# zombie-einstein/bourse

Measured on AMD Instinct MI355X. Metric: book-steps/sec, higher is better.
Workload: dtype u32

## Files before the change

bourse_amd/csrc/agent_table.hpp:

```cpp
#pragma once
#include <cmath>
#include <cstdint>
#include <cstring>
#include <string>
#include <vector>

#include "../../include/bourse_amd.h"
#include "host_math.hpp"

namespace bkd {

struct Group {
  uint32_t n;
  uint32_t thr;
  uint32_t tick_lo, tick_rng, tick_zone;
  uint32_t vol_lo, vol_rng, vol_zone;
  uint32_t tick_size;
  uint32_t asset;
  uint32_t pad[2];
};
static_assert(sizeof(Group) == 48, "Group: 48-byte records (the per-unit table is read as three 16-byte loads)");

inline uint64_t groups_hash(const Group* g, size_t n) {
  const unsigned char* c = reinterpret_cast<const unsigned char*>(g);
  uint64_t h = 1469598103934665603ull;
  for (size_t i = 0; i < n * sizeof(Group); ++i) h = (h ^ c[i]) * 1099511628211ull;
  return h;
}

inline int make_groups(const bk_random_agents* rows, uint32_t n_groups, const uint32_t* assets, uint32_t M,
                       const uint32_t* asset_tick, Group* out, uint64_t* total, std::string* msg,
                       const std::string& where = std::string()) {
  *total = 0;
  auto fail = [&](int code, uint32_t g, const char* m) {
    *msg = where.empty() ? std::string(m) : where + "group " + std::to_string(g) + ": " + m;
    return code;
  };
  for (uint32_t g = 0; g < n_groups; ++g) {
    const bk_random_agents& r = rows[g];
    if (r.tick_lo >= r.tick_hi || r.vol_lo >= r.vol_hi)
      return fail(BK_INVALID_ARGUMENT, g, "empty tick/vol range");
    const uint32_t asset = assets ? assets[g] : 0u;
    if (asset >= M) return fail(BK_INVALID_ARGUMENT, g, "group asset index out of range");
    if (r.tick_size % asset_tick[asset] != 0)
      return fail(BK_PRICE_NOT_TICK_MULTIPLE, g, "agent tick_size must be a multiple of the env tick_size");
    if (static_cast<uint64_t>(r.tick_hi - 1) * r.tick_size >= 0xFFFFFFFFull || r.tick_lo == 0)
      return fail(BK_INVALID_ARGUMENT, g, "limit prices must lie in (0, u32::MAX)");
    Group G{};
    G.n = r.n_agents;
    G.thr = activity_threshold(r.activity_rate);
    G.tick_lo = r.tick_lo;
    G.tick_rng = r.tick_hi - r.tick_lo;
    G.tick_zone = sample_zone(G.tick_rng);
    G.vol_lo = r.vol_lo;
    G.vol_rng = r.vol_hi - r.vol_lo;
    G.vol_zone = sample_zone(G.vol_rng);
    G.tick_size = r.tick_size;
    G.asset = asset;
    *total += r.n_agents;
    out[g] = G;
  }
  return BK_OK;
}

constexpr const char* CAPACITY_MSG = "sum of n_agents exceeds max_live_orders (one pool slot per agent)";

inline int make_group_table(const bk_random_agents* rows, uint32_t n_units, uint32_t n_groups, const uint32_t* assets,
                            uint32_t M, const uint32_t* asset_tick, uint32_t max_live_orders, std::vector<Group>& out,
                            uint64_t* total, std::string* msg) {
  std::vector<Group> t(static_cast<size_t>(n_units) * n_groups);
  *total = 0;
  for (uint32_t u = 0; u < n_units; ++u) {
    const std::string where = "unit " + std::to_string(u) + ", ";
    uint64_t tot = 0;
    const size_t row = static_cast<size_t>(u) * n_groups;
    if (int rc = make_groups(rows + row, n_groups, assets, M, asset_tick, t.data() + row, &tot, msg, where)) return rc;
    for (uint32_t g = 0; g < n_groups; ++g)
      if (t[row + g].n != t[g].n) {
        *msg = where + "group " + std::to_string(g) + ": n_agents differs from unit 0's (every unit shares the pool layout)";
        return BK_INVALID_ARGUMENT;
      }
    if (tot > max_live_orders) {
      *msg = where + CAPACITY_MSG;
      return BK_CAPACITY;
    }
    *total = tot;
  }
  out.swap(t);
  return BK_OK;
}

constexpr int MAX_MEMBERS = 4;
constexpr int MAX_ASSETS = 8;

struct MixedDesc {
  uint32_t type;
  uint32_t n;
  uint32_t thr, tick_lo, tick_rng, tick_zone, vol_lo, vol_rng, vol_zone, tick_size;
  uint32_t thr_limit, thr_market;
  int32_t keep_thr;
  uint32_t trade_vol;
  uint32_t slot_base;
  uint32_t pad;
  double mu, sigma, decay, demand, scale, order_ratio, n_f, tick_f;
};
static_assert(sizeof(MixedDesc) == 128, "MixedDesc layout");

inline uint64_t fnv1a_bytes(const void* p, size_t n, uint64_t h = 1469598103934665603ull) {
  const unsigned char* c = static_cast<const unsigned char*>(p);
  for (size_t i = 0; i < n; ++i) h = (h ^ c[i]) * 1099511628211ull;
  return h;
}
inline uint64_t mixed_hash(const uint32_t* member_asset, const MixedDesc* d, size_t n) {
  return fnv1a_bytes(member_asset, MAX_MEMBERS * sizeof(uint32_t), fnv1a_bytes(d, n * sizeof(MixedDesc)));
}

inline int make_mixed_descs(const bk_agent_desc* members, uint32_t n_members, const uint32_t* assets,
                            const uint32_t* asset_tick, MixedDesc* out, uint32_t* fixed_a, std::string* msg,
                            const std::string& where = std::string()) {
  for (int as = 0; as < MAX_ASSETS; ++as) fixed_a[as] = 0;
  auto fail = [&](int code, uint32_t i, const char* m) {
    *msg = where.empty() ? std::string(m) : where + "member " + std::to_string(i) + ": " + m;
    return code;
  };
  for (uint32_t i = 0; i < n_members; ++i) {
    const uint32_t as = assets ? assets[i] : 0u;
    uint32_t& fixed = fixed_a[as];
    const bk_agent_desc& m = members[i];
    MixedDesc D;
    std::memset(&D, 0, sizeof(D));
    D.type = m.type;
    D.n = m.n_agents;
    if (m.tick_size == 0 || m.tick_size % asset_tick[as] != 0)
      return fail(BK_PRICE_NOT_TICK_MULTIPLE, i, "member tick_size must be a non-zero multiple of the env tick_size");
    if (m.type == BK_AGENT_RANDOM) {
      if (m.tick_lo >= m.tick_hi || m.vol_lo >= m.vol_hi || m.tick_lo == 0 ||
          static_cast<uint64_t>(m.tick_hi - 1) * m.tick_size >= 0xFFFFFFFFull)
        return fail(BK_INVALID_ARGUMENT, i, "bad RandomAgents ranges");
      D.thr = activity_threshold(m.activity_rate);
      D.tick_lo = m.tick_lo;
      D.tick_rng = m.tick_hi - m.tick_lo;
      D.tick_zone = sample_zone(D.tick_rng);
      D.vol_lo = m.vol_lo;
      D.vol_rng = m.vol_hi - m.vol_lo;
      D.vol_zone = sample_zone(D.vol_rng);
      D.tick_size = m.tick_size;
      D.slot_base = fixed;
      fixed += m.n_agents;
    } else if (m.type == BK_AGENT_NOISE || m.type == BK_AGENT_MOMENTUM) {
      if (m.n_agents > 0xFFFFu) return fail(BK_INVALID_ARGUMENT, i, "n_agents is a u16 in the reference");
      if (!(m.price_dist_sigma >= 0.0) || !std::isfinite(m.price_dist_sigma) || !std::isfinite(m.price_dist_mu))
        return fail(BK_INVALID_ARGUMENT, i, "LogNormal::new(mu, sigma) needs finite mu and sigma >= 0");
      D.thr_limit = activity_threshold(m.p_limit);
      D.thr_market = activity_threshold(m.p_market);
      D.keep_thr = keep_threshold(m.p_cancel);
      D.trade_vol = m.trade_vol;
      D.mu = m.price_dist_mu;
      D.sigma = m.price_dist_sigma;
      D.decay = m.decay;
      D.demand = m.demand;
      D.scale = m.scale;
      D.order_ratio = m.order_ratio;
      D.n_f = static_cast<double>(m.n_agents);
      D.tick_f = static_cast<double>(m.tick_size);
    } else {
      return fail(BK_INVALID_ARGUMENT, i, "unknown agent type");
    }
    out[i] = D;
  }
  return BK_OK;
}

constexpr const char* MIXED_CAPACITY_MSG = "RandomAgents members leave no pool slots for the other members' orders";
inline bool mixed_capacity_ok(const uint32_t* fixed_a, uint32_t M, uint32_t max_live_orders) {
  for (uint32_t as = 0; as < M; ++as)
    if (fixed_a[as] >= max_live_orders) return false;
  return true;
}

inline int make_mixed_table(const bk_agent_desc* members, uint32_t n_units, uint32_t n_members, const uint32_t* assets,
                            uint32_t M, const uint32_t* asset_tick, uint32_t max_live_orders, std::vector<MixedDesc>& out,
                            uint32_t* fixed_a, std::string* msg) {
  std::vector<MixedDesc> t(static_cast<size_t>(n_units) * n_members);
  for (uint32_t u = 0; u < n_units; ++u) {
    const std::string where = "unit " + std::to_string(u) + ", ";
    const size_t row = static_cast<size_t>(u) * n_members;
    if (int rc = make_mixed_descs(members + row, n_members, assets, asset_tick, t.data() + row, fixed_a, msg, where))
      return rc;
    for (uint32_t i = 0; i < n_members; ++i) {
      const char* what = t[row + i].type != t[i].type ? "type differs from unit 0's"
                         : t[row + i].n != t[i].n   ? "n_agents differs from unit 0's"
                                                    : nullptr;
      if (what) {
        *msg = where + "member " + std::to_string(i) + ": " + what + " (every unit shares the members' kinds and pool layout)";
        return BK_INVALID_ARGUMENT;
      }
    }
  }
  if (!mixed_capacity_ok(fixed_a, M, max_live_orders)) {
    *msg = std::string("unit 0, ") + MIXED_CAPACITY_MSG;
    return BK_CAPACITY;
  }
  out.swap(t);
  return BK_OK;
}

}
```

bourse_amd/csrc/agents_fsm_body.inc:

```
  uint16_t* list = reinterpret_cast<uint16_t*>(fsm_lds);
  const int lane = threadIdx.x;
  __builtin_amdgcn_s_setprio(3);
#if BOURSE_AMD_FSM_TOP_VGPR > 0
  asm volatile("" ::: "v" BK_STR(BOURSE_AMD_FSM_TOP_VGPR));
#endif
  const uint32_t M = a.assets;
  const uint32_t b = a.book_begin + blockIdx.x * 64 + lane;
  if (b >= a.book_end) return;
  uint32_t* st = a.state + (size_t)b * M * a.state_stride;
  uint32_t* bt = a.batch + (size_t)b * M * a.batch_stride;
#if BK_PB
  const Group* row = table + (size_t)b * a.n_groups;
  LaneGroup nxt{};
  if (a.n_groups) nxt = load_lane_group(row);
#endif

  RngLane rng;
  {
    const uint2 x0 = *reinterpret_cast<const uint2*>(st + H_S0_LO);
    const uint2 x1 = *reinterpret_cast<const uint2*>(st + H_S1_LO);
    rng.a0 = x0.x, rng.a1 = x0.y, rng.b0 = x1.x, rng.b1 = x1.y;
  }
  uint64_t live[R];
#pragma unroll
  for (int r = 0; r < R; ++r) {
    uint2 x = *reinterpret_cast<const uint2*>(st + H_LIVE0 + 2 * r);
    for (uint32_t as = 1; as < M; ++as) {
      const uint2 y = *reinterpret_cast<const uint2*>(st + (size_t)as * a.state_stride + H_LIVE0 + 2 * r);
      x.x |= y.x;
      x.y |= y.y;
    }
    live[r] = mk64(x.x, x.y);
  }
  uint2* pv = reinterpret_cast<uint2*>(bt + BT_EV + 32 * R);

  const uint32_t five = RngLane::opaque5();
  uint32_t n = 0, n_ev = 0, gbase = 0;
  for (uint32_t g = 0; g < a.n_groups; ++g) {
    const Group G = a.groups[g];
    const uint32_t gend = gbase + G.n;
    gbase = gend;
#if BK_PB
    LaneGroup L{};
    L = nxt;
    if (g + 1 < a.n_groups) nxt = load_lane_group(row + g + 1);
#endif
    if (G.n == 0) continue;
#if BK_PB
    const uint32_t g_thr = L.a.y, g_tick_lo = L.a.z, g_vol_lo = L.b.y;
    uint32_t g_tick_size = L.tick_size;
    asm volatile("" : "+v"(g_tick_size));
    uint32_t v_trng = L.a.w, v_vrng = L.b.z, v_tzone = L.b.x, v_vzone = L.b.w;
#else
    asm volatile("" ::"s"(G.thr), "s"(G.tick_lo), "s"(G.tick_rng), "s"(G.tick_zone));
    asm volatile("" ::"s"(G.vol_lo), "s"(G.vol_rng), "s"(G.vol_zone), "s"(G.tick_size));
    const uint32_t g_thr = G.thr, g_tick_lo = G.tick_lo, g_vol_lo = G.vol_lo, g_tick_size = G.tick_size;
    uint32_t v_trng = G.tick_rng, v_vrng = G.vol_rng, v_tzone = G.tick_zone, v_vzone = G.vol_zone;
#endif
    asm volatile("" : "+v"(v_trng), "+v"(v_vrng), "+v"(v_tzone), "+v"(v_vzone));
    const uint64_t thr8 = (uint64_t)g_thr << 8;
    uint64_t price0 = (uint64_t)(g_tick_lo * g_tick_size);
    asm volatile("" : "+v"(price0));
    for (uint32_t sbeg = gend - G.n; sbeg < gend;) {
      const uint32_t send = gend < (sbeg | 63u) + 1u ? gend : (sbeg | 63u) + 1u;
      uint64_t w = live[0];
#pragma unroll
      for (int r = 1; r < R; ++r) w = ((sbeg >> 6) == (uint32_t)r) ? live[r] : w;
      uint32_t cur_side = 0, cur_price = 0;
      uint64_t P_ACT = ~0ull, P_SIDE = 0, P_TICK = 0, P_VOL = 0;
      while (n < send) {
        const uint32_t x = rng.output(five);
        const uint32_t range = sel(P_SIDE, 2u, sel(P_TICK, v_trng, v_vrng));
        const uint32_t zone = sel(P_SIDE, 0x7FFFFFFFu, sel(P_TICK, v_tzone, v_vzone));
        const uint64_t m = (uint64_t)x * range;
        const uint32_t val = (uint32_t)(m >> 32);
        uint64_t C_HIT = __builtin_amdgcn_ballot_w64((uint64_t)x < thr8);
        uint64_t C_ACC = __builtin_amdgcn_ballot_w64((uint32_t)m <= zone);
        uint64_t C_LIVE = __builtin_amdgcn_ballot_w64(((w >> (n & 63)) & 1ull) != 0);
        asm volatile("" : "+v"(rng.a0), "+v"(rng.a1), "+v"(rng.b0), "+v"(rng.b1)
                     : "s"(P_ACT), "s"(P_SIDE), "s"(P_TICK), "s"(P_VOL), "s"(C_HIT), "s"(C_ACC), "s"(C_LIVE));
        rng.advance();
        asm volatile("" : "+v"(rng.a0), "+v"(rng.a1), "+v"(rng.b0), "+v"(rng.b1), "+s"(P_ACT), "+s"(P_SIDE), "+s"(P_TICK),
                       "+s"(P_VOL), "+s"(C_HIT), "+s"(C_ACC), "+s"(C_LIVE));
        const uint64_t HIT = P_ACT & C_HIT, CANCEL = HIT & C_LIVE, TO_SIDE = HIT & ~C_LIVE;
        const uint64_t A_SIDE = C_ACC & P_SIDE, A_TICK = C_ACC & P_TICK, A_VOL = C_ACC & P_VOL;
        const uint64_t QUEUE = CANCEL | A_VOL, ADV = (P_ACT & ~C_HIT) | QUEUE;
        cur_side = sel(A_SIDE, val, cur_side);
        {
          uint64_t pr, cy;
#if BK_PB
          asm("v_mad_u64_u32 %0, %1, %2, %3, %4" : "=v"(pr), "=s"(cy) : "v"(val), "v"(g_tick_size), "v"(price0));
#else
          asm("v_mad_u64_u32 %0, %1, %2, %3, %4" : "=v"(pr), "=s"(cy) : "v"(val), "s"(g_tick_size), "v"(price0));
#endif
          cur_price = sel(A_TICK, (uint32_t)pr, cur_price);
        }
        if (lane_bit(QUEUE)) list[n_ev * 64 + lane] = (uint16_t)sel(A_VOL, n | EV_NEW | (cur_side << 14), n);
        asm("v_addc_co_u32_e64 %0, vcc, 0, %0, %1" : "+v"(n_ev) : "s"(QUEUE) : "vcc");
        if (lane_bit(A_VOL)) pv[n] = make_uint2(cur_price, g_vol_lo + val);
        P_SIDE = TO_SIDE | (P_SIDE & ~C_ACC);
        P_TICK = A_SIDE | (P_TICK & ~C_ACC);
        P_VOL = A_TICK | (P_VOL & ~C_ACC);
        P_ACT = ADV;
        asm("v_addc_co_u32_e64 %0, vcc, 0, %0, %1" : "+v"(n) : "s"(ADV) : "vcc");
      }
      sbeg = send;
    }
  }

  {
    uint32_t i = n_ev > 1 ? n_ev - 1 : 0;
    uint32_t rg = i + 1;
    uint32_t zn = (rg << __builtin_clz(rg)) - 1u;
    while (i != 0) {
      const uint32_t x = rng.output(five);
      const uint64_t m = (uint64_t)x * rg;
      uint64_t ACC = __builtin_amdgcn_ballot_w64((uint32_t)m <= zn);
      asm volatile("" : "+v"(rng.a0), "+v"(rng.a1), "+v"(rng.b0), "+v"(rng.b1) : "s"(ACC));
      rng.advance();
      asm volatile("" : "+v"(rng.a0), "+v"(rng.a1), "+v"(rng.b0), "+v"(rng.b1), "+s"(ACC));
      if (lane_bit(ACC)) {
        const uint32_t j = (uint32_t)(m >> 32);
        const uint16_t ai = list[i * 64 + lane], aj = list[j * 64 + lane];
        list[i * 64 + lane] = aj;
        list[j * 64 + lane] = ai;
        --i;
        rg = i + 1;
        zn = (rg << __builtin_clz(rg)) - 1u;
      }
    }
  }

  for (uint32_t as = 0; as < M; ++as) {
    *reinterpret_cast<uint2*>(st + (size_t)as * a.state_stride + H_S0_LO) = make_uint2(rng.a0, rng.a1);
    *reinterpret_cast<uint2*>(st + (size_t)as * a.state_stride + H_S1_LO) = make_uint2(rng.b0, rng.b1);
  }
  bt[BT_NEV] = n_ev;
  for (uint32_t k = 0; k < n_ev; k += 2) {
    const uint32_t lo = list[k * 64 + lane];
    const uint32_t hi = (k + 1 < n_ev) ? list[(k + 1) * 64 + lane] : 0u;
    bt[BT_EV + (k >> 1)] = lo | (hi << 16);
  }
```

bourse_amd/csrc/book_device.hpp:

```cpp
#pragma once
#include <hip/hip_runtime.h>
#include <utility>
#include <stdint.h>

#include "event_asm.hpp"
#include "event_asm_gen.hpp"
#include "agent_table.hpp"

#ifndef BOURSE_AMD_ASM_EVENTS
#define BOURSE_AMD_ASM_EVENTS 1
#endif
#ifndef BOURSE_AMD_ASM_R48
#define BOURSE_AMD_ASM_R48 1
#endif

namespace bkd {

constexpr int HDR_DW = 64;
enum Hdr : int {
  H_T_LO = 0, H_T_HI, H_S0_LO, H_S0_HI, H_S1_LO, H_S1_HI,
  H_NEXT_ID, H_SEQ, H_TRADES_LO, H_TRADES_HI, H_FLAGS, H_TRADING,
  H_STEPS_LO, H_STEPS_HI, H_EVENTS_LO, H_EVENTS_HI, H_TRADE_VOL,
  H_TRADE_BASE_LO, H_TRADE_BASE_HI, H_LAST_NTRADES, H_LAST_NEVENTS,
  H_EV_KEYED,
  H_LIVE0 = 32,
};
constexpr int HDR_SCALARS = 20;
constexpr int POOL_FIELDS = 5;
constexpr int MAX_GROUPS = 8;

constexpr uint32_t FLAG_POOL_OVERFLOW = 1u, FLAG_TRADE_OVERFLOW = 2u, FLAG_STEP_SIZE = 4u,
                   FLAG_ORDER_LOG_FULL = 8u, FLAG_UNKNOWN_ORDER = 16u, FLAG_HIST_OVERFLOW = 32u, FLAG_PRICE_TICK = 64u,
                   FLAG_EVENT_OVERFLOW = 128u;


struct UDiv {
  uint32_t m, sh1, sh2, d;
};
__device__ __forceinline__ uint32_t udiv(uint32_t n, const UDiv& dv) {
  const uint32_t t = __umulhi(dv.m, n);
  return (t + ((n - t) >> dv.sh1)) >> dv.sh2;
}

struct DevTrade {
  uint32_t t_lo, t_hi, price, vol, active, passive, side_is_bid, pad;
};

struct DevOrderLog {
  uint32_t status, vol, price;
  uint32_t key_price;
  uint32_t arr_lo, arr_hi, end_lo, end_hi;
  uint32_t key_lo, key_hi, pad[2];
};

struct DevArgs {
  uint32_t n_books, levels, tick_size, n_groups;
  uint32_t step_lo, step_hi;
  uint32_t state_stride;
  uint32_t l2_width;
  uint32_t trade_cap, hist_cap;
  uint32_t hist_slot0, step_prio;
  uint32_t n_agents_total, log_cap;
  uint32_t* state;
  uint32_t* l2_last;
  uint32_t* hist;
  DevTrade* trades;
  DevOrderLog* order_log;
  const uint32_t* ev_off;
  const uint4* ev;
  const uint32_t* ev_len;
  uint32_t ev_stride;
  uint32_t* batch;
  uint32_t batch_stride;
  uint32_t book_begin, book_end;
  uint32_t assets;
  uint32_t asset_tick[MAX_ASSETS];
  UDiv tick_div, asset_div[MAX_ASSETS];
  Group groups[MAX_GROUPS];
};
constexpr int BT_NEV = 0, BT_EV = 64;
constexpr uint32_t EV_NEW = 0x8000u, EV_BID = 0x4000u, EV_SLOT = 0x1FFu;
constexpr uint32_t EV_MOD = 0x800u, EV_MOD_P = 0x200u, EV_MOD_V = 0x400u;

__device__ __forceinline__ uint32_t rfl(uint32_t v) { return __builtin_amdgcn_readfirstlane(v); }

typedef uint32_t bk_u32x4 __attribute__((ext_vector_type(4)));
typedef uint32_t bk_u32x8 __attribute__((ext_vector_type(8)));
typedef uint32_t bk_u32x16 __attribute__((ext_vector_type(16)));
__device__ __forceinline__ void sload_x16_x4(const uint32_t* p, bk_u32x16& a, bk_u32x4& b) {
  asm volatile("s_load_dwordx16 %0, %2, 0x0\n\ts_load_dwordx4 %1, %2, 0x40\n\ts_waitcnt lgkmcnt(0)"
               : "=&s"(a), "=&s"(b) : "s"(p) : "memory");
}
__device__ __forceinline__ bk_u32x8 sload_x8(const uint32_t* p) {
  bk_u32x8 a;
  asm volatile("s_load_dwordx8 %0, %1, 0x0\n\ts_waitcnt lgkmcnt(0)" : "=&s"(a) : "s"(p) : "memory");
  return a;
}
__device__ __forceinline__ Group sload_group(const Group* p) {
  bk_u32x8 w;
  uint32_t ts;
  asm volatile("s_load_dwordx8 %0, %2, 0x0\n\ts_load_dword %1, %2, 0x20\n\ts_waitcnt lgkmcnt(0)" : "=&s"(w), "=&s"(ts) : "s"(p));
  Group G{};
  G.n = w[0], G.thr = w[1], G.tick_lo = w[2], G.tick_rng = w[3], G.tick_zone = w[4];
  G.vol_lo = w[5], G.vol_rng = w[6], G.vol_zone = w[7], G.tick_size = ts;
  return G;
}
__device__ __forceinline__ uint32_t rdl(uint32_t v, uint32_t lane) { return __builtin_amdgcn_readlane(v, lane); }
extern "C" __device__ uint32_t bk_llvm_writelane(uint32_t val, uint32_t lane, uint32_t old) __asm(
    "llvm.amdgcn.writelane.i32");
__device__ __forceinline__ uint32_t wrl(uint32_t val, uint32_t lane, uint32_t old) {
  return bk_llvm_writelane(val, lane, old);
}

__device__ __forceinline__ uint32_t sel(uint64_t mask, uint32_t if_set, uint32_t if_clear) {
  return __builtin_amdgcn_inverse_ballot_w64(mask) ? if_set : if_clear;
}
__device__ __forceinline__ bool lane_bit(uint64_t mask) { return __builtin_amdgcn_inverse_ballot_w64(mask); }

#define BK_DPP_REDUCE(OP)                                                                      \
  asm("s_nop 1\n\t" OP " %0, %0, %0 quad_perm:[1,0,3,2] row_mask:0xf bank_mask:0xf\n\t"        \
      "s_nop 1\n\t" OP " %0, %0, %0 quad_perm:[2,3,0,1] row_mask:0xf bank_mask:0xf\n\t"        \
      "s_nop 1\n\t" OP " %0, %0, %0 row_half_mirror row_mask:0xf bank_mask:0xf\n\t"            \
      "s_nop 1\n\t" OP " %0, %0, %0 row_mirror row_mask:0xf bank_mask:0xf\n\t"                 \
      "s_nop 1\n\t" OP " %0, %0, %0 row_bcast:15 row_mask:0xa bank_mask:0xf\n\t"               \
      "s_nop 1\n\t" OP " %0, %0, %0 row_bcast:31 row_mask:0xc bank_mask:0xf\n\t"               \
      "s_nop 1"                                                                                \
      : "+v"(x))
__device__ __forceinline__ uint32_t wave_umin(uint32_t x) {
  BK_DPP_REDUCE("v_min_u32_dpp");
  return rdl(x, 63);
}
__device__ __forceinline__ uint32_t wave_umax(uint32_t x) {
  BK_DPP_REDUCE("v_max_u32_dpp");
  return rdl(x, 63);
}
__device__ __forceinline__ int32_t wave_imin(int32_t x) {
  BK_DPP_REDUCE("v_min_i32_dpp");
  return (int32_t)rdl((uint32_t)x, 63);
}
__device__ __forceinline__ int32_t wave_imax(int32_t x) {
  BK_DPP_REDUCE("v_max_i32_dpp");
  return (int32_t)rdl((uint32_t)x, 63);
}
__device__ __forceinline__ uint32_t wave_add(uint32_t x) {
  BK_DPP_REDUCE("v_add_u32_dpp");
  return rdl(x, 63);
}

#define BK_DPP4(CTRL)                                                     \
  "v_max_u32_dpp %0, %0, %0 " CTRL "\n\tv_min_u32_dpp %1, %1, %1 " CTRL "\n\t" \
  "v_add_u32_dpp %2, %2, %2 " CTRL "\n\tv_add_u32_dpp %3, %3, %3 " CTRL "\n\t"
__device__ __forceinline__ void wave_reduce4(uint32_t& mx, uint32_t& mn, uint32_t& s1, uint32_t& s2) {
  asm("s_nop 1\n\t" BK_DPP4("quad_perm:[1,0,3,2] row_mask:0xf bank_mask:0xf") BK_DPP4("quad_perm:[2,3,0,1] row_mask:0xf bank_mask:0xf")
          BK_DPP4("row_half_mirror row_mask:0xf bank_mask:0xf") BK_DPP4("row_mirror row_mask:0xf bank_mask:0xf")
              BK_DPP4("row_bcast:15 row_mask:0xa bank_mask:0xf") BK_DPP4("row_bcast:31 row_mask:0xc bank_mask:0xf") "s_nop 1"
      : "+v"(mx), "+v"(mn), "+v"(s1), "+v"(s2));
  mx = rdl(mx, 63);
  mn = rdl(mn, 63);
  s1 = rdl(s1, 63);
  s2 = rdl(s2, 63);
}

#define BK_DPP3(CTRL) \
  "v_max_u32_dpp %0, %0, %0 " CTRL "\n\tv_min_u32_dpp %1, %1, %1 " CTRL "\n\tv_max_u32_dpp %2, %2, %2 " CTRL "\n\t"
__device__ __forceinline__ void wave_reduce3(uint32_t& mx, uint32_t& mn, uint32_t& m2) {
  asm("s_nop 1\n\t" BK_DPP3("quad_perm:[1,0,3,2] row_mask:0xf bank_mask:0xf") BK_DPP3("quad_perm:[2,3,0,1] row_mask:0xf bank_mask:0xf")
          BK_DPP3("row_half_mirror row_mask:0xf bank_mask:0xf") BK_DPP3("row_mirror row_mask:0xf bank_mask:0xf")
              BK_DPP3("row_bcast:15 row_mask:0xa bank_mask:0xf") BK_DPP3("row_bcast:31 row_mask:0xc bank_mask:0xf") "s_nop 1"
      : "+v"(mx), "+v"(mn), "+v"(m2));
  mx = rdl(mx, 63);
  mn = rdl(mn, 63);
  m2 = rdl(m2, 63);
}

__device__ __forceinline__ uint64_t mk64(uint32_t lo, uint32_t hi) { return ((uint64_t)hi << 32) | lo; }

struct Rng {
  uint64_t s0, s1;
  __device__ __forceinline__ uint32_t next_u32() {
    uint64_t r = s0 * 5ull;
    r = (r << 7) | (r >> 57);
    r *= 9ull;
    uint64_t t1 = s1 ^ s0;
    s0 = ((s0 << 24) | (s0 >> 40)) ^ t1 ^ (t1 << 16);
    s1 = (t1 << 37) | (t1 >> 27);
    return (uint32_t)r;
  }
  __device__ __forceinline__ uint32_t below(uint32_t range, uint32_t zone) {
    for (;;) {
      uint32_t v = next_u32();
      uint64_t m = (uint64_t)v * range;
      if ((uint32_t)m <= zone) return (uint32_t)(m >> 32);
    }
  }
  __device__ __forceinline__ uint32_t below(uint32_t range) {
    uint32_t zone = (range << __builtin_clz(range)) - 1u;
    return below(range, zone);
  }
};

__device__ __forceinline__ uint32_t xor3(uint32_t a, uint32_t b, uint32_t c) {
  return __builtin_amdgcn_bitop3_b32(a, b, c, 0x96);
}
struct RngLane {
  uint32_t a0, a1, b0, b1;
  static __device__ __forceinline__ uint32_t opaque5() {
    uint32_t five = 5u;
    asm("" : "+s"(five));
    return five;
  }
  static __device__ __forceinline__ uint32_t mul5_rotl7_lo(uint32_t a0, uint32_t a1, uint32_t five) {
    const uint64_t p = (uint64_t)a0 * five;
    const uint32_t hi5 = (a1 << 2) + (uint32_t)(p >> 32) + a1;
    return __builtin_amdgcn_alignbit((uint32_t)p, hi5, 25);
  }
  __device__ __forceinline__ uint32_t next_u32() {
    const uint32_t r = mul5_rotl7_lo(a0, a1, opaque5());
    const uint32_t t0 = b0 ^ a0, t1 = b1 ^ a1;
    const uint32_t n0 = xor3(__builtin_amdgcn_alignbit(a0, a1, 8), t0, t0 << 16);
    const uint32_t n1 = xor3(__builtin_amdgcn_alignbit(a1, a0, 8), t1, __builtin_amdgcn_alignbit(t1, t0, 16));
    a0 = n0;
    a1 = n1;
    b0 = __builtin_amdgcn_alignbit(t1, t0, 27);
    b1 = __builtin_amdgcn_alignbit(t0, t1, 27);
    return (r << 3) + r;
  }
  __device__ __forceinline__ uint32_t output(uint32_t five) const {
    const uint32_t r = mul5_rotl7_lo(a0, a1, five);
    return (r << 3) + r;
  }
  __device__ __forceinline__ void advance() {
    uint32_t t0 = b0 ^ a0, t1 = b1 ^ a1;
    uint32_t r0 = __builtin_amdgcn_alignbit(a0, a1, 8), r1 = __builtin_amdgcn_alignbit(a1, a0, 8);
    asm volatile("" : "+v"(t0), "+v"(t1), "+v"(r0), "+v"(r1));
    const uint32_t n0 = xor3(r0, t0, t0 << 16);
    const uint32_t n1 = xor3(r1, t1, __builtin_amdgcn_alignbit(t1, t0, 16));
    a0 = n0;
    a1 = n1;
    b0 = __builtin_amdgcn_alignbit(t1, t0, 27);
    b1 = __builtin_amdgcn_alignbit(t0, t1, 27);
  }
};

template <int R>
struct Book {
  uint32_t price[R], vol[R], id[R], seq[R];
  uint64_t live[R], bid[R], pend[R];
  uint64_t t;
  uint32_t next_id, seq_ctr, trade_vol, flags, trading;
  uint64_t n_trades, n_events, trade_base;
  uint32_t tr_k, tr_price, tr_vol, tr_act, tr_pas;
  uint32_t tr_n;
  uint32_t hdr0;
};

template <int R>
__device__ __forceinline__ uint32_t slot_read(const uint32_t (&v)[R], uint32_t n) {
  uint32_t out = rdl(v[0], n & 63);
#pragma unroll
  for (int r = 1; r < R; ++r) {
    uint32_t x = rdl(v[r], n & 63);
    out = ((n >> 6) == (uint32_t)r) ? x : out;
  }
  return out;
}
template <int R>
__device__ __forceinline__ void slot_write(uint32_t (&v)[R], uint32_t n, uint32_t val) {
#pragma unroll
  for (int r = 0; r < R; ++r)
    if ((n >> 6) == (uint32_t)r) v[r] = wrl(val, n & 63, v[r]);
}
template <int R>
__device__ __forceinline__ bool mask_test(const uint64_t (&m)[R], uint32_t n) {
  uint64_t w = 0;
#pragma unroll
  for (int r = 0; r < R; ++r) w |= m[r] & (((n >> 6) == (uint32_t)r) ? ~0ull : 0ull);
  return (w >> (n & 63)) & 1ull;
}
template <int R>
__device__ __forceinline__ void mask_set(uint64_t (&m)[R], uint32_t n, bool on) {
  const uint64_t bit = 1ull << (n & 63);
#pragma unroll
  for (int r = 0; r < R; ++r) {
    const uint64_t b = ((n >> 6) == (uint32_t)r) ? bit : 0ull;
    m[r] = on ? (m[r] | b) : (m[r] & ~b);
  }
}

template <int R>
__device__ __forceinline__ void flush_trades(Book<R>& B, const DevArgs& a, uint32_t book, uint64_t t0, int lane) {
  if (B.tr_n == 0) return;
  const uint64_t first = B.n_trades;
  B.n_trades += B.tr_n;
  const uint64_t pos0 = first - B.trade_base;
  if ((uint32_t)lane < B.tr_n) {
    const uint64_t pos = pos0 + (uint32_t)lane;
    if (pos < a.trade_cap) {
      const uint64_t t = t0 + (B.tr_k & 0x7FFFFFFFu);
      DevTrade rec;
      rec.t_lo = (uint32_t)t;
      rec.t_hi = (uint32_t)(t >> 32);
      rec.price = B.tr_price;
      rec.vol = B.tr_vol;
      rec.active = B.tr_act;
      rec.passive = B.tr_pas;
      rec.side_is_bid = B.tr_k >> 31;
      rec.pad = 0;
      uint4* dst = reinterpret_cast<uint4*>(a.trades + (size_t)book * a.trade_cap + pos);
      const uint4* src = reinterpret_cast<const uint4*>(&rec);
      dst[0] = src[0];
      dst[1] = src[1];
    }
  }
  if (pos0 + B.tr_n > a.trade_cap) B.flags |= FLAG_TRADE_OVERFLOW;
  B.tr_n = 0;
}

template <int R>
__device__ __forceinline__ void emit_trade(Book<R>& B, const DevArgs& a, uint32_t book, uint64_t t0, int lane,
                                           uint32_t k, bool passive_is_bid, uint32_t price, uint32_t vol,
                                           uint32_t active, uint32_t passive) {
  if (B.tr_n == 64) flush_trades(B, a, book, t0, lane);
  const uint32_t l = B.tr_n;
  B.tr_k = wrl(k | (passive_is_bid ? 0x80000000u : 0u), l, B.tr_k);
  B.tr_price = wrl(price, l, B.tr_price);
  B.tr_vol = wrl(vol, l, B.tr_vol);
  B.tr_act = wrl(active, l, B.tr_act);
  B.tr_pas = wrl(passive, l, B.tr_pas);
  B.tr_n = l + 1;
}

template <int R>
__device__ __forceinline__ uint32_t pool_gather(const uint32_t (&v)[R], uint32_t idx) {
  uint32_t out = (uint32_t)__builtin_amdgcn_ds_bpermute((int)((idx & 63u) << 2), (int)v[0]);
#pragma unroll
  for (int r = 1; r < R; ++r) {
    const uint32_t x = (uint32_t)__builtin_amdgcn_ds_bpermute((int)((idx & 63u) << 2), (int)v[r]);
    out = (idx >> 6) == (uint32_t)r ? x : out;
  }
  return out;
}
template <int R>
__device__ __forceinline__ void flush_trades_compact(Book<R>& B, const DevArgs& a, uint32_t book, uint64_t t0, int lane,
                                                     const uint32_t (&ev)[R]) {
  if (B.tr_n == 0) return;
  const uint32_t k = B.tr_k & 0x7FFFFFFFu, ps = B.tr_pas & (64u * R - 1u);
  const uint32_t as = pool_gather<R>(ev, k < 64u * R ? k : 0u) & EV_SLOT & (64u * R - 1u);
  B.tr_price = pool_gather<R>(B.price, ps);
  B.tr_pas = pool_gather<R>(B.id, ps);
  B.tr_act = pool_gather<R>(B.id, as);
  flush_trades<R>(B, a, book, t0, lane);
}

struct LogCtx {
  DevOrderLog* base;
  uint32_t cap;
};
__device__ __forceinline__ void log_write(const LogCtx& lg, uint32_t& flags, int lane, uint32_t id, uint32_t status,
                                          uint32_t vol, uint32_t price, uint64_t arr, uint64_t end,
                                          bool set_arr, bool set_key = false, uint64_t key_t = 0) {
  if (!lg.base) return;
  if (id >= lg.cap) {
    flags |= FLAG_ORDER_LOG_FULL;
    return;
  }
  if (lane == 0) {
    DevOrderLog* e = lg.base + id;
    e->status = status;
    e->vol = vol;
    e->price = price;
    if (set_arr) {
      e->arr_lo = (uint32_t)arr;
      e->arr_hi = (uint32_t)(arr >> 32);
    }
    e->end_lo = (uint32_t)end;
    e->end_hi = (uint32_t)(end >> 32);
    if (set_key) {
      e->key_price = price;
      e->key_lo = (uint32_t)key_t;
      e->key_hi = (uint32_t)(key_t >> 32);
    }
  }
}
__device__ __forceinline__ void log_fill(const LogCtx& lg, uint32_t& flags, int lane, uint32_t id, uint32_t vol,
                                         uint64_t t) {
  if (!lg.base) return;
  if (id >= lg.cap) {
    flags |= FLAG_ORDER_LOG_FULL;
    return;
  }
  if (lane == 0) {
    DevOrderLog* e = lg.base + id;
    e->vol = vol;
    if (vol == 0) {
      e->status = 2;
      e->end_lo = (uint32_t)t;
      e->end_hi = (uint32_t)(t >> 32);
    }
  }
}

template <int R, bool agg_bid>
__device__ __forceinline__ bool match_side(Book<R>& B, const DevArgs& a, uint32_t book, uint64_t t0, int lane,
                                           uint32_t k, uint32_t p, uint32_t& v, uint32_t agg_id, const LogCtx& lg) {
  const uint32_t v0 = v;
  while (v > 0) {
// ... 39 lines not shown
        pv -= tv;
        B.vol[r] = wrl(pv, l, B.vol[r]);
        if (pv == 0) B.live[r] &= ~eq[r];
      }
    }
    v -= tv;
    emit_trade(B, a, book, t0, lane, k, !agg_bid, best, tv, agg_id, pid);
    B.trade_vol += tv;
    log_fill(lg, B.flags, lane, pid, pv, t0 + k);
  }
  return v0 != 0 && v == 0;
}
template <int R>
__device__ __forceinline__ bool match(Book<R>& B, const DevArgs& a, uint32_t book, uint64_t t0, int lane, uint32_t k,
                                      bool agg_bid, uint32_t p, uint32_t& v, uint32_t agg_id, const LogCtx& lg) {
  return agg_bid ? match_side<R, true>(B, a, book, t0, lane, k, p, v, agg_id, lg)
                 : match_side<R, false>(B, a, book, t0, lane, k, p, v, agg_id, lg);
}

template <int R, int RS, bool CLS = false, bool LOG = false, class... Lg>
__device__ __forceinline__ void slot_event_at(Book<R>& B, const DevArgs& a, uint32_t book, uint64_t t0, int lane,
                                              uint32_t k, uint32_t sl, uint32_t ew = 0, const Lg&... lg) {
  const LogCtx nolog{nullptr, 0};
  const uint64_t bit = 1ull << sl;
  if (CLS ? !(ew & EV_NEW) : !(B.pend[RS] & bit)) {
    if constexpr (LOG) {
      if (B.live[RS] & bit)
        log_write(lg..., B.flags, lane, rdl(B.id[RS], sl), 3, rdl(B.vol[RS], sl), rdl(B.price[RS], sl), 0, t0 + k, false);
    }
    B.live[RS] &= ~bit;
    return;
  }
  if (!CLS) B.pend[RS] &= ~bit;
  const uint32_t p = rdl(B.price[RS], sl);
  uint32_t v = rdl(B.vol[RS], sl);
  const uint32_t id = rdl(B.id[RS], sl);
  bool filled = false, market;
  if (CLS ? (ew & EV_BID) != 0 : (B.bid[RS] & bit) != 0) {
    market = p == 0xFFFFFFFFu;
    if (B.trading) {
      if constexpr (LOG) filled = match_side<R, true>(B, a, book, t0, lane, k, p, v, id, lg...);
      else filled = match_side<R, true>(B, a, book, t0, lane, k, p, v, id, nolog);
    }
  } else {
    market = p == 0u;
    if (B.trading) {
      if constexpr (LOG) filled = match_side<R, false>(B, a, book, t0, lane, k, p, v, id, lg...);
      else filled = match_side<R, false>(B, a, book, t0, lane, k, p, v, id, nolog);
    }
  }
  if (!market && !filled) {
    B.vol[RS] = wrl(v, sl, B.vol[RS]);
    B.seq[RS] = wrl(B.seq_ctr, sl, B.seq[RS]);
    B.live[RS] |= bit;
    B.seq_ctr += 1;
  }
  if constexpr (LOG) {
    const uint64_t tk = t0 + k;
    uint32_t status = 1;
    uint64_t end = ~0ull;
    if (filled || market) {
      status = filled ? 2u : (B.trading ? 3u : 4u);
      end = tk;
    }
    log_write(lg..., B.flags, lane, id, status, v, p, tk, end, true, true, status == 1 ? tk : 0ull);
  }
}

template <int R, int RS = 0, bool CLS = false, bool LOG = false, class... Lg>
__device__ __forceinline__ void process_slot_event(Book<R>& B, const DevArgs& a, uint32_t book, uint64_t t0, int lane,
                                                   uint32_t k, uint32_t n, uint32_t ew = 0, const Lg&... lg) {
  if constexpr (RS + 1 < R) {
    if ((n >> 6) == (uint32_t)RS)
      slot_event_at<R, RS, CLS, LOG>(B, a, book, t0, lane, k, n & 63, ew, lg...);
    else
      process_slot_event<R, RS + 1, CLS, LOG>(B, a, book, t0, lane, k, n, ew, lg...);
  } else {
    slot_event_at<R, RS, CLS, LOG>(B, a, book, t0, lane, k, n & 63, ew, lg...);
  }
}

template <int R>
__device__ __forceinline__ void snapshot(const Book<R>& B, const DevArgs& a, uint32_t book, int lane,
                                         uint32_t* __restrict__ bins , uint32_t hist_slot,
                                         uint32_t& flags, bool write_last, const UDiv& tick) {
  const uint32_t L = a.levels;
  uint32_t mb = 0u, ma = 0xFFFFFFFFu, sb = 0u, sa = 0u;
#pragma unroll
  for (int r = 0; r < R; ++r) {
    const uint64_t lb = B.live[r] & B.bid[r], la = B.live[r] & ~B.bid[r];
    mb = max(mb, sel(lb, B.price[r], 0u));
    ma = min(ma, sel(la, B.price[r], 0xFFFFFFFFu));
    sb += sel(lb, B.vol[r], 0u);
    sa += sel(la, B.vol[r], 0u);
  }
  wave_reduce4(mb, ma, sb, sa);
  const uint32_t bid_best = mb;
  const uint32_t ask_best = ma;
  const uint32_t bid_vol = sb, ask_vol = sa;

  for (uint32_t j = lane; j < 4 * L; j += 64) bins[j] = 0;
  __builtin_amdgcn_fence(__ATOMIC_RELEASE, "wavefront");
  __builtin_amdgcn_wave_barrier();
#pragma unroll
  for (int r = 0; r < R; ++r) {
    const bool is_live = lane_bit(B.live[r]);
    const bool is_bid = lane_bit(B.bid[r]);
    if (is_live) {
      const uint32_t d = is_bid ? (bid_best - B.price[r]) : (B.price[r] - ask_best);
      const uint32_t q = udiv(d, tick);
      if (q * tick.d == d && q < L) {
        atomicAdd(&bins[4 * q + (is_bid ? 0 : 2)], B.vol[r]);
        atomicAdd(&bins[4 * q + (is_bid ? 1 : 3)], 1u);
      }
    }
  }
  __builtin_amdgcn_fence(__ATOMIC_ACQ_REL, "wavefront");
  __builtin_amdgcn_wave_barrier();
  if (__builtin_expect(__umulhi(L - 1u, tick.d) != 0u, 0)) {
    for (uint32_t i = 1; i < L; ++i) {
      const uint32_t m = i * tick.d, q = udiv(m, tick);
      if (q != i && q * tick.d == m && lane < 4) bins[4 * i + lane] = bins[4 * q + lane];
    }
    __builtin_amdgcn_fence(__ATOMIC_ACQ_REL, "wavefront");
    __builtin_amdgcn_wave_barrier();
  }

  const uint32_t W = a.l2_width;
  uint32_t* last = a.l2_last + (size_t)book * W;
  uint32_t* hist = nullptr;
  if (a.hist_cap) hist = a.hist + ((size_t)hist_slot * a.n_books + book) * W;
  (void)flags;
  uint32_t h = 0;
  h = lane == 0 ? B.trade_vol : h;
  h = lane == 1 ? bid_best : h;
  h = lane == 2 ? ask_best : h;
  h = lane == 3 ? ask_vol : h;
  h = lane == 4 ? bid_vol : h;
  if (lane < 5) {
    if (write_last) last[lane] = h;
    if (hist) hist[lane] = h;
  }
  for (uint32_t j = lane; j < 4 * L; j += 64) {
    const uint32_t x = bins[j];
    if (write_last) last[5 + j] = x;
    if (hist) hist[5 + j] = x;
  }
}

template <int R>
struct StepRaw {
  uint32_t hdr, f[R][POOL_FIELDS];
  uint32_t sh[HDR_SCALARS];
  uint32_t bh, ev[R];
  uint2 pv[R];
};
template <int R>
__device__ __forceinline__ void load_state_raw(StepRaw<R>& w, const uint32_t* __restrict__ st, int lane) {
  w.hdr = st[lane];
#pragma unroll
  for (int r = 0; r < R; ++r) {
    const uint32_t* p = st + HDR_DW + r * POOL_FIELDS * 64;
#pragma unroll
    for (int f = 0; f < POOL_FIELDS; ++f) w.f[r][f] = p[f * 64 + lane];
  }
}
template <int R>
__device__ __forceinline__ void load_state_scalars(StepRaw<R>& w, const uint32_t* __restrict__ st) {
  if constexpr (R <= 2) {
    bk_u32x16 a;
    bk_u32x4 b;
    sload_x16_x4(st, a, b);
#pragma unroll
    for (int i = 0; i < 16; ++i) w.sh[i] = a[i];
#pragma unroll
    for (int i = 16; i < HDR_SCALARS; ++i) w.sh[i] = b[i - 16];
  }
}
template <int R>
__device__ __forceinline__ void unpack_book(Book<R>& B, Rng& rng, const StepRaw<R>& w) {
  const uint32_t hdr = w.hdr;
#pragma unroll
  for (int r = 0; r < R; ++r) {
    B.price[r] = w.f[r][0];
    B.vol[r] = w.f[r][1];
    B.id[r] = w.f[r][2];
    B.seq[r] = w.f[r][3];
  }
  auto H = [&](int i) { return R <= 2 ? w.sh[i] : rdl(hdr, (uint32_t)i); };
  B.t = mk64(H(H_T_LO), H(H_T_HI));
  rng.s0 = mk64(H(H_S0_LO), H(H_S0_HI));
  rng.s1 = mk64(H(H_S1_LO), H(H_S1_HI));
  B.next_id = H(H_NEXT_ID);
  B.seq_ctr = H(H_SEQ);
  B.n_trades = mk64(H(H_TRADES_LO), H(H_TRADES_HI));
  B.flags = H(H_FLAGS);
  B.trading = H(H_TRADING);
  B.n_events = mk64(H(H_EVENTS_LO), H(H_EVENTS_HI));
  B.trade_vol = H(H_TRADE_VOL);
  B.trade_base = mk64(H(H_TRADE_BASE_LO), H(H_TRADE_BASE_HI));
#pragma unroll
  for (int r = 0; r < R; ++r) {
    const uint32_t meta = w.f[r][4];
    B.live[r] = __ballot((meta & 1u) != 0);
    B.bid[r] = __ballot((meta & 2u) != 0);
    B.pend[r] = __ballot((meta & 4u) != 0);
  }
  B.tr_k = B.tr_price = B.tr_vol = B.tr_act = B.tr_pas = 0;
  B.tr_n = 0;
  B.hdr0 = hdr;
}
template <int R>
__device__ __forceinline__ void load_book(Book<R>& B, Rng& rng, const uint32_t* __restrict__ st, int lane) {
  StepRaw<R> w;
  load_state_raw<R>(w, st, lane);
  load_state_scalars<R>(w, st);
  unpack_book<R>(B, rng, w);
}

template <int R, bool KEEP_HDR = false>
__device__ __forceinline__ void store_book(const Book<R>& B, const Rng& rng, uint32_t* __restrict__ st, int lane,
                                           uint64_t steps_done, uint32_t last_ntrades, uint32_t last_nevents,
                                           uint32_t ev_keyed = 0u) {
  uint32_t hdr = KEEP_HDR ? B.hdr0 : st[lane];
  if (!KEEP_HDR) hdr += lane == H_EV_KEYED ? ev_keyed : 0u;
  auto put = [&](int idx, uint32_t v) { hdr = wrl(rfl(v), (uint32_t)idx, hdr); };
  put(H_T_LO, (uint32_t)B.t);
  put(H_T_HI, (uint32_t)(B.t >> 32));
  put(H_S0_LO, (uint32_t)rng.s0);
  put(H_S0_HI, (uint32_t)(rng.s0 >> 32));
  put(H_S1_LO, (uint32_t)rng.s1);
  put(H_S1_HI, (uint32_t)(rng.s1 >> 32));
  put(H_NEXT_ID, B.next_id);
  put(H_SEQ, B.seq_ctr);
  put(H_TRADES_LO, (uint32_t)B.n_trades);
  put(H_TRADES_HI, (uint32_t)(B.n_trades >> 32));
  put(H_FLAGS, B.flags);
  put(H_STEPS_LO, (uint32_t)steps_done);
  put(H_STEPS_HI, (uint32_t)(steps_done >> 32));
  put(H_EVENTS_LO, (uint32_t)B.n_events);
  put(H_EVENTS_HI, (uint32_t)(B.n_events >> 32));
  put(H_TRADE_VOL, B.trade_vol);
  put(H_LAST_NTRADES, last_ntrades);
  put(H_LAST_NEVENTS, last_nevents);
#pragma unroll
  for (int r = 0; r < R; ++r) {
    put(H_LIVE0 + 2 * r, (uint32_t)B.live[r]);
    put(H_LIVE0 + 2 * r + 1, (uint32_t)(B.live[r] >> 32));
  }
  st[lane] = hdr;
#pragma unroll
  for (int r = 0; r < R; ++r) {
    uint32_t* p = st + HDR_DW + r * POOL_FIELDS * 64;
    p[0 * 64 + lane] = B.price[r];
    p[1 * 64 + lane] = B.vol[r];
    p[2 * 64 + lane] = B.id[r];
    p[3 * 64 + lane] = B.seq[r];
    p[4 * 64 + lane] = (lane_bit(B.live[r]) ? 1u : 0u) | (lane_bit(B.bid[r]) ? 2u : 0u) | (lane_bit(B.pend[r]) ? 4u : 0u);
  }
}

#ifndef BOURSE_AMD_KEYED_EVENTS
#define BOURSE_AMD_KEYED_EVENTS 1
#endif
#ifndef BOURSE_AMD_KEY_SEQ_BITS
#define BOURSE_AMD_KEY_SEQ_BITS 16
#endif
#ifndef BOURSE_AMD_KEYED_WIDE
#define BOURSE_AMD_KEYED_WIDE 1
#endif
constexpr uint32_t KEY_SB = BOURSE_AMD_KEY_SEQ_BITS;
constexpr uint32_t KEY_SMASK = (1u << (KEY_SB < 16u ? KEY_SB : 16u)) - 1u;
constexpr uint32_t KEY_PSPAN = (1u << (31u - (KEY_SB > 16u ? KEY_SB : 16u))) - 6u;
constexpr uint32_t KEY_ASK = 0x80000000u;
constexpr uint32_t KP_MKT_BID = 0xFFFFFFFFu, KP_MKT_ASK = 0x10000u;
template <int R>
__device__ __forceinline__ bool key_window(const Book<R>& B, const uint64_t (&newm)[R], uint32_t n_ev, uint32_t& pbase,
                                           uint32_t& sbase, uint32_t xmin = 0xFFFFFFFFu, uint32_t xmax = 0u) {
  uint32_t pmax = xmax, pmin = xmin, age = 0;
#pragma unroll
  for (int r = 0; r < R; ++r) {
    const bool lv = lane_bit(B.live[r]), in = lv | lane_bit(newm[r]);
    pmax = max(pmax, in ? B.price[r] : 0u);
    pmin = min(pmin, in ? B.price[r] : 0xFFFFFFFFu);
    age = max(age, lv ? B.seq_ctr - B.seq[r] : 0u);
  }
  wave_reduce3(pmax, pmin, age);
  pbase = pmin - 2u;
  sbase = B.seq_ctr - age - 1u;
  return pmin >= 2u && pmax != 0xFFFFFFFFu && pmax - pmin <= KEY_PSPAN && age + n_ev < KEY_SMASK - 1u;
}

template <int R>
struct KeyState {
  uint32_t key[R], pk[R];
  uint32_t sq, sbase, pbase;
  int32_t alo, bhi;
};
template <int R, bool MARKETS = false>
__device__ __forceinline__ bool keys_begin(const Book<R>& B, const uint64_t (&newm)[R], uint32_t n_ev, KeyState<R>& K,
                                           uint32_t xmin = 0xFFFFFFFFu, uint32_t xmax = 0u) {
  uint32_t pbase;
  uint64_t lim[R];
#pragma unroll
  for (int r = 0; r < R; ++r)
    lim[r] = MARKETS ? newm[r] & ~__ballot(B.price[r] == (lane_bit(B.bid[r]) ? 0xFFFFFFFFu : 0u)) : newm[r];
  if (!key_window<R>(B, lim, n_ev, pbase, K.sbase, xmin, xmax)) return false;
  K.pbase = pbase;
#pragma unroll
  for (int r = 0; r < R; ++r) {
    const bool bidl = lane_bit(B.bid[r]);
    const uint32_t pf = B.price[r] - pbase, sf = B.seq[r] - K.sbase;
    K.key[r] = lane_bit(B.live[r]) ? ((pf << 16) | (bidl ? 0xFFFFu - sf : KEY_ASK | sf)) : 0u;
    K.pk[r] = lane_bit(lim[r]) ? (bidl ? 0x8000u | pf : pf) : 0u;
    if (MARKETS) K.pk[r] = lane_bit(newm[r] & ~lim[r]) ? (bidl ? 0xFFFFu : 1u) : K.pk[r];
  }
  K.sq = KEY_ASK | (B.seq_ctr - K.sbase);
  K.alo = (int32_t)0x80000000u;
  K.bhi = 0x7FFFFFFF;
  return true;
}
template <int R, bool MARKETS>
__device__ __forceinline__ bool keys_begin_wide(const Book<R>& B, const uint64_t (&newm)[R], uint32_t n_ev, KeyState<R>& K,
                                                const uint32_t (&ev)[R], uint32_t* bins, int lane) {
  uint64_t lim[R];
#pragma unroll
  for (int r = 0; r < R; ++r)
    lim[r] = MARKETS ? newm[r] & ~__ballot(B.price[r] == (lane_bit(B.bid[r]) ? 0xFFFFFFFFu : 0u)) : newm[r];
  uint32_t pmax = 0, age = 0, vbig = 0;
#pragma unroll
  for (int r = 0; r < R; ++r) {
    const bool lv = lane_bit(B.live[r]), in = lv | lane_bit(lim[r]);
    pmax = max(pmax, in ? B.price[r] : 0u);
    age = max(age, lv ? B.seq_ctr - B.seq[r] : 0u);
    vbig = max(vbig, (lv | lane_bit(newm[r])) ? B.vol[r] : 0u);
  }
  uint32_t dummy = 0xFFFFFFFFu;
  wave_reduce3(pmax, dummy, age);
  vbig = wave_umax(vbig);
  if (pmax == 0xFFFFFFFFu || pmax < 2u || age + n_ev >= KEY_SMASK - 1u || vbig >= (1u << 22)) return false;
  const uint32_t pbase = pmax > KEY_PSPAN ? pmax - KEY_PSPAN : 0u, lowp = pbase + 2u;
  if (lane < 2 * R) bins[lane] = 0u;
  __builtin_amdgcn_fence(__ATOMIC_ACQ_REL, "wavefront");
  __builtin_amdgcn_wave_barrier();
#pragma unroll
  for (int re = 0; re < R; ++re) {
    const uint32_t slot = ev[re] & EV_SLOT & (64u * R - 1u);
    if ((uint32_t)(re * 64 + lane) < n_ev) atomicOr(&bins[slot >> 5], 1u << (slot & 31u));
  }
  __builtin_amdgcn_fence(__ATOMIC_ACQ_REL, "wavefront");
  __builtin_amdgcn_wave_barrier();
  uint32_t pbid = 0;
#pragma unroll
  for (int r = 0; r < R; ++r)
    pbid = max(pbid, ((lane_bit(B.live[r]) | lane_bit(lim[r])) && lane_bit(B.bid[r])) ? B.price[r] : 0u);
  pbid = wave_umax(pbid);
  uint32_t w_bid = 0, a_ask = 0;
  uint64_t bad = 0;
#pragma unroll
  for (int r = 0; r < R; ++r) {
    const bool lv = lane_bit(B.live[r]), bidl = lane_bit(B.bid[r]), nw = lane_bit(newm[r]);
    const bool below = (lv | lane_bit(lim[r])) && B.price[r] < lowp;
    const bool listed = ((bins[(uint32_t)(r * 64 + lane) >> 5] >> ((uint32_t)lane & 31u)) & 1u) != 0u;
    bad |= __ballot(below && !bidl);
    w_bid += (lv && bidl && !below && !listed) ? B.vol[r] : 0u;
    a_ask += (nw && !bidl && B.price[r] <= pbid) ? B.vol[r] : 0u;
  }
  if (bad) return false;
  w_bid = wave_add(w_bid);
  a_ask = wave_add(a_ask);
  if (a_ask > w_bid) return false;
  K.pbase = pbase;
  K.sbase = B.seq_ctr - age - 1u;
#pragma unroll
  for (int r = 0; r < R; ++r) {
    const bool bidl = lane_bit(B.bid[r]);
    const uint32_t pf = B.price[r] < lowp ? 1u : B.price[r] - pbase, sf = B.seq[r] - K.sbase;
    K.key[r] = lane_bit(B.live[r]) ? ((pf << 16) | (bidl ? 0xFFFFu - sf : KEY_ASK | sf)) : 0u;
    K.pk[r] = lane_bit(lim[r]) ? (bidl ? 0x8000u | pf : pf) : 0u;
    if (MARKETS) K.pk[r] = lane_bit(newm[r] & ~lim[r]) ? (bidl ? 0xFFFFu : 1u) : K.pk[r];
  }
  K.sq = KEY_ASK | (B.seq_ctr - K.sbase);
  K.alo = (int32_t)0x80000000u;
  K.bhi = 0x7FFFFFFF;
  return true;
}
template <int R, bool MARKETS>
__device__ __forceinline__ bool keys_begin_wide_high(const Book<R>& B, const uint64_t (&newm)[R], uint32_t n_ev, KeyState<R>& K,
                                                     const uint32_t (&ev)[R], uint32_t* bins, int lane) {
  uint64_t lim[R];
#pragma unroll
  for (int r = 0; r < R; ++r)
    lim[r] = MARKETS ? newm[r] & ~__ballot(B.price[r] == (lane_bit(B.bid[r]) ? 0xFFFFFFFFu : 0u)) : newm[r];
  uint32_t pmin = 0xFFFFFFFFu, age = 0, vbig = 0, pdummy = 0;
#pragma unroll
  for (int r = 0; r < R; ++r) {
    const bool lv = lane_bit(B.live[r]), in = lv | lane_bit(lim[r]);
    pmin = min(pmin, in ? B.price[r] : 0xFFFFFFFFu);
    age = max(age, lv ? B.seq_ctr - B.seq[r] : 0u);
    vbig = max(vbig, (lv | lane_bit(newm[r])) ? B.vol[r] : 0u);
  }
  wave_reduce3(pdummy, pmin, age);
  vbig = wave_umax(vbig);
  if (pmin < 2u || pmin > 0xFFFFFFFFu - KEY_PSPAN - 4u || age + n_ev >= KEY_SMASK - 1u || vbig >= (1u << 22)) return false;
  const uint32_t pbase = pmin - 2u, highp = pmin + KEY_PSPAN;
  if (lane < 2 * R) bins[lane] = 0u;
  __builtin_amdgcn_fence(__ATOMIC_ACQ_REL, "wavefront");
  __builtin_amdgcn_wave_barrier();
#pragma unroll
  for (int re = 0; re < R; ++re) {
    const uint32_t slot = ev[re] & EV_SLOT & (64u * R - 1u);
    if ((uint32_t)(re * 64 + lane) < n_ev) atomicOr(&bins[slot >> 5], 1u << (slot & 31u));
  }
  __builtin_amdgcn_fence(__ATOMIC_ACQ_REL, "wavefront");
  __builtin_amdgcn_wave_barrier();
  uint32_t pask = 0xFFFFFFFFu;
#pragma unroll
  for (int r = 0; r < R; ++r)
    pask = min(pask, ((lane_bit(B.live[r]) | lane_bit(lim[r])) && !lane_bit(B.bid[r])) ? B.price[r] : 0xFFFFFFFFu);
  pask = wave_umin(pask);
  uint32_t w_ask = 0, b_bid = 0;
  uint64_t bad = 0;
#pragma unroll
  for (int r = 0; r < R; ++r) {
    const bool lv = lane_bit(B.live[r]), bidl = lane_bit(B.bid[r]), nw = lane_bit(newm[r]);
    const bool above = (lv | lane_bit(lim[r])) && B.price[r] > highp;
    const bool listed = ((bins[(uint32_t)(r * 64 + lane) >> 5] >> ((uint32_t)lane & 31u)) & 1u) != 0u;
    bad |= __ballot(above && bidl);
    w_ask += (lv && !bidl && !above && !listed) ? B.vol[r] : 0u;
    b_bid += (nw && bidl && B.price[r] >= pask) ? B.vol[r] : 0u;
  }
  if (bad) return false;
  w_ask = wave_add(w_ask);
  b_bid = wave_add(b_bid);
  if (b_bid > w_ask) return false;
  K.pbase = pbase;
  K.sbase = B.seq_ctr - age - 1u;
#pragma unroll
  for (int r = 0; r < R; ++r) {
    const bool bidl = lane_bit(B.bid[r]);
    const uint32_t pf = B.price[r] > highp ? 0x7FFFu : B.price[r] - pbase, sf = B.seq[r] - K.sbase;
    K.key[r] = lane_bit(B.live[r]) ? ((pf << 16) | (bidl ? 0xFFFFu - sf : KEY_ASK | sf)) : 0u;
    K.pk[r] = lane_bit(lim[r]) ? (bidl ? 0x8000u | pf : pf) : 0u;
    if (MARKETS) K.pk[r] = lane_bit(newm[r] & ~lim[r]) ? (bidl ? 0xFFFFu : 1u) : K.pk[r];
  }
  K.sq = KEY_ASK | (B.seq_ctr - K.sbase);
  K.alo = (int32_t)0x80000000u;
  K.bhi = 0x7FFFFFFF;
  return true;
}
template <int R>
__device__ __forceinline__ void keys_end(Book<R>& B, const KeyState<R>& K) {
  B.seq_ctr = K.sbase + (K.sq & 0x7FFFFFFFu);
#pragma unroll
  for (int r = 0; r < R; ++r) {
    B.live[r] = __ballot(K.key[r] != 0u);
    const uint32_t f = K.key[r] & 0xFFFFu;
    B.seq[r] = K.key[r] != 0u ? K.sbase + ((int32_t)K.key[r] < 0 ? f : 0xFFFFu - f) : B.seq[r];
  }
}
template <int R>
__device__ __forceinline__ void key_event_words(const KeyState<R>& K, const uint32_t (&ev)[R], uint32_t n_ev, uint32_t (&evw)[R]) {
#pragma unroll
  for (int re = 0; re < R; ++re) {
    evw[re] = ev[re] & 0xFFFFu;
    if (n_ev > (uint32_t)re * 64u) evw[re] |= pool_gather<R>(K.pk, ev[re] & EV_SLOT & (64u * R - 1u)) << 16;
  }
}

template <int R, bool agg_bid, int... I>
__device__ __forceinline__ int32_t key_touch(const KeyState<R>& K, std::integer_sequence<int, I...>) {
  int32_t m = (int32_t)K.key[0];
  ((m = agg_bid ? min(m, (int32_t)K.key[I]) : max(m, (int32_t)K.key[I])), ...);
  return m;
}

template <int R>
__device__ __forceinline__ void flush_trades_compact(Book<R>& B, const DevArgs& a, uint32_t book, uint64_t t0, int lane,
                                                     const uint32_t (&ev)[R]);
template <int R, bool agg_bid>
__device__ __forceinline__ bool match_side_keyed(Book<R>& B, KeyState<R>& K, const DevArgs& a, uint32_t book, uint64_t t0,
                                                 int lane, uint32_t k, int32_t kp, uint32_t& v, const uint32_t (&ev)[R]) {
  const uint32_t v0 = v;
  while (v > 0) {
    const int32_t m = key_touch<R, agg_bid>(K, std::make_integer_sequence<int, R>());
    const int32_t best = agg_bid ? wave_imin(m) : wave_imax(m);
    (agg_bid ? K.alo : K.bhi) = best;
    if (agg_bid ? (best > kp) : (best < kp)) break;
    uint32_t pv = 0, tv = 0, slot = 0;
#pragma unroll
    for (int r = 0; r < R; ++r) {
      const uint64_t eq = __ballot(K.key[r] == (uint32_t)best);
      if (eq) {
        const uint32_t l = __builtin_ctzll(eq);
        pv = rdl(B.vol[r], l);
        tv = v < pv ? v : pv;
        pv -= tv;
        B.vol[r] = wrl(pv, l, B.vol[r]);
        if (pv == 0) K.key[r] = wrl(0u, l, K.key[r]);
        slot = (uint32_t)r * 64u + l;
      }
    }
    v -= tv;
    if (B.tr_n == 64) flush_trades_compact<R>(B, a, book, t0, lane, ev);
    const uint32_t tl = B.tr_n;
    B.tr_k = wrl(k | (agg_bid ? 0u : 0x80000000u), tl, B.tr_k);
    B.tr_vol = wrl(tv, tl, B.tr_vol);
    B.tr_pas = wrl(slot, tl, B.tr_pas);
    B.tr_n = tl + 1;
    B.trade_vol += tv;
  }
  return v0 != 0 && v == 0;
}
template <int R, int RS, bool CLS = true>
__device__ __forceinline__ void slot_event_keyed_at(Book<R>& B, KeyState<R>& K, const DevArgs& a, uint32_t book, uint64_t t0,
                                                    int lane, uint32_t k, uint32_t sl, uint32_t ew, const uint32_t (&ev)[R]) {
  const uint64_t bit = 1ull << sl;
  if (CLS ? !(ew & EV_NEW) : !(B.pend[RS] & bit)) {
    K.key[RS] = wrl(0u, sl, K.key[RS]);
    return;
  }
  if (!CLS) B.pend[RS] &= ~bit;
  const bool is_bid = CLS ? (ew & EV_BID) != 0 : (B.bid[RS] & bit) != 0;
  const uint32_t kpu = (rdl(K.pk[RS], sl) << 16) | (is_bid ? 0xFFFFu : 0u);
  const int32_t kp = (int32_t)kpu;
  uint32_t v = rdl(B.vol[RS], sl);
  const bool market = !CLS && kpu == (is_bid ? KP_MKT_BID : KP_MKT_ASK);
  bool filled = false;
  if (B.trading && !(is_bid ? kp < K.alo : kp > K.bhi))
    filled = is_bid ? match_side_keyed<R, true>(B, K, a, book, t0, lane, k, kp, v, ev)
                    : match_side_keyed<R, false>(B, K, a, book, t0, lane, k, kp, v, ev);
  if (!market && !filled) {
    B.vol[RS] = wrl(v, sl, B.vol[RS]);
    const uint32_t x = kpu ^ K.sq;
    if (is_bid)
      K.bhi = max(K.bhi, (int32_t)x);
    else
      K.alo = min(K.alo, (int32_t)x);
    K.key[RS] = wrl(x, sl, K.key[RS]);
    K.sq += 1;
  }
}
template <int R, int RS = 0, bool CLS = true>
__device__ __forceinline__ void slot_event_keyed(Book<R>& B, KeyState<R>& K, const DevArgs& a, uint32_t book, uint64_t t0,
                                                 int lane, uint32_t k, uint32_t n, uint32_t ew, const uint32_t (&ev)[R]) {
  if constexpr (RS + 1 < R) {
    if ((n >> 6) == (uint32_t)RS)
      slot_event_keyed_at<R, RS, CLS>(B, K, a, book, t0, lane, k, n & 63, ew, ev);
    else
      slot_event_keyed<R, RS + 1, CLS>(B, K, a, book, t0, lane, k, n, ew, ev);
  } else {
    slot_event_keyed_at<R, RS, CLS>(B, K, a, book, t0, lane, k, n & 63, ew, ev);
  }
}

template <int R, bool MKT = false, bool TAGGED = false, bool CLS = false, bool PENDKEY = false, bool LOG = false, class... Lg>
__device__ __forceinline__ uint32_t step_from_list(Book<R>& B, const DevArgs& a, uint32_t book, int lane,
                                                   const uint32_t (&ev)[R], uint32_t n_ev, uint32_t* bins,
                                                   uint32_t hist_slot, bool write_last, const UDiv& tick,
                                                   const uint64_t (&mine)[R], uint32_t& n_own, uint32_t asset = 0,
                                                   const Lg&... lg) {
  const uint64_t step_size = mk64(a.step_lo, a.step_hi);
  const uint64_t t0 = B.t;
  B.trade_vol = 0;
  const uint64_t trades_before = B.n_trades;
  if (step_size != 0 && (uint64_t)n_ev >= step_size) B.flags |= FLAG_STEP_SIZE;
  uint64_t newm[R];
#pragma unroll
  for (int r = 0; r < R; ++r) {
    newm[r] = (CLS || PENDKEY) ? B.pend[r] : 0ull;
    if (CLS) B.pend[r] = 0;
  }
  constexpr bool MKTK = MKT && CLS && !TAGGED;
  uint32_t evm[R], own_cnt = 0;
  bool listed = false;
#pragma unroll
  for (int re = 0; re < R; ++re) {
    evm[re] = ev[re];
    if constexpr (MKTK) {
      const uint32_t slot = ev[re] & EV_SLOT & (64u * R - 1u);
      bool own = false;
#pragma unroll
      for (int r = 0; r < R; ++r) own = (slot >> 6) == (uint32_t)r ? ((mine[r] >> (slot & 63u)) & 1ull) != 0ull : own;
      evm[re] = own ? ev[re] : (ev[re] & ~(EV_NEW | EV_BID));
      own_cnt += (uint32_t)__builtin_popcountll(__ballot(own && (uint32_t)(re * 64 + lane) < n_ev));
    }
  }
  if constexpr (!LOG && (R == 2 || R == 1) && (!MKT || MKTK) && CLS && BOURSE_AMD_ASM_EVENTS) {
    listed = true;
    uint32_t k = 0;
    const uint32_t nev = rfl(n_ev), tmask = B.trading ? 0xFFFFFFFFu : 0u;
    KeyState<R> K;
    if (BOURSE_AMD_KEYED_EVENTS && keys_begin<R>(B, newm, nev, K)) {
      uint32_t evw[R];
      key_event_words<R>(K, evm, nev, evw);
      uint64_t zero_vol = 0;
#pragma unroll
      for (int r = 0; r < R; ++r) zero_vol |= __ballot(lane_bit(newm[r]) && B.vol[r] == 0u);
      const uint32_t checked = (!B.trading || zero_vol != 0) ? 1u : 0u;
      for (;;) {
        uint32_t full;
        if constexpr (R == 2)
          full = events_key_r2(checked, k, nev, tmask, B.tr_n, K.sq, B.vol[0], B.vol[1], K.key[0], K.key[1], evw[0], evw[1],
                               B.tr_k, B.tr_vol, B.tr_pas);
        else
          full = events_key_r1(checked, k, nev, tmask, B.tr_n, K.sq, B.vol[0], K.key[0], evw[0], B.tr_k, B.tr_vol, B.tr_pas);
        if (B.tr_n) B.trade_vol += wave_add((uint32_t)lane < B.tr_n ? B.tr_vol : 0u);
        flush_trades_compact<R>(B, a, book, t0, lane, evw);
        if (!full) break;
      }
      keys_end<R>(B, K);
    } else if constexpr (R == 2) {
      while (events_asm_r2(k, nev, tmask, B.tr_n, B.seq_ctr, B.trade_vol, B.live[0], B.live[1], B.bid[0], B.bid[1],
                           B.price[0], B.price[1], B.vol[0], B.vol[1], B.id[0], B.id[1], B.seq[0], B.seq[1], evm[0], evm[1],
                           B.tr_k, B.tr_price, B.tr_vol, B.tr_act, B.tr_pas))
        flush_trades<R>(B, a, book, t0, lane);
    } else {
      while (events_asm_r1(k, nev, tmask, B.tr_n, B.seq_ctr, B.trade_vol, B.live[0], B.bid[0], B.price[0], B.vol[0], B.id[0],
                           B.seq[0], evm[0], B.tr_k, B.tr_price, B.tr_vol, B.tr_act, B.tr_pas))
        flush_trades<R>(B, a, book, t0, lane);
    }
  } else if (KeyState<R> K; !LOG && (CLS || PENDKEY) && (!MKT || MKTK) && BOURSE_AMD_KEYED_EVENTS &&
             (keys_begin<R, !CLS>(B, newm, rfl(n_ev), K) ||
              (BOURSE_AMD_KEYED_WIDE && !CLS && keys_begin_wide<R, true>(B, newm, rfl(n_ev), K, ev, bins, lane)))) {
   if constexpr ((R == 4 || R == 8) && BOURSE_AMD_ASM_EVENTS && BOURSE_AMD_ASM_R48) {
    listed = true;
    uint32_t evw[R];
    key_event_words<R>(K, evm, rfl(n_ev), evw);
    if (!CLS) {
#pragma unroll
      for (int re = 0; re < R; ++re) {
        const uint32_t pk = evw[re] >> 16;
        evw[re] = (evw[re] & (0xFFFF0000u | EV_SLOT)) | (pk != 0u ? EV_NEW | ((pk & 0x8000u) ? EV_BID : 0u) : 0u);
      }
#pragma unroll
      for (int r = 0; r < R; ++r) B.pend[r] = 0;
    }
    uint32_t evq[R];
#pragma unroll
    for (int re = 0; re < R; ++re)
      evq[re] = n_ev > (uint32_t)re * 64u ? pool_gather<R>(B.vol, evw[re] & EV_SLOT & (64u * R - 1u)) : 0u;
    uint32_t k = 0;
    const uint32_t nev = rfl(n_ev), tmask = B.trading ? 0xFFFFFFFFu : 0u;
    uint64_t zero_vol = 0;
#pragma unroll
    for (int r = 0; r < R; ++r) zero_vol |= __ballot(lane_bit(newm[r]) && B.vol[r] == 0u);
    const uint32_t checked = (!B.trading || zero_vol != 0) ? 1u : 0u;
    for (;;) {
      uint32_t full;
      if constexpr (R == 4 && CLS)
        full = events_key_r4(checked, k, nev, tmask, B.tr_n, K.sq, B.vol, K.key, evw, evq, B.tr_k, B.tr_vol, B.tr_pas);
      else if constexpr (R == 4)
        full = events_key_r4m(checked, k, nev, tmask, B.tr_n, K.sq, B.vol, K.key, evw, evq, B.tr_k, B.tr_vol, B.tr_pas);
      else if constexpr (CLS)
        full = events_key_r8(checked, k, nev, tmask, B.tr_n, K.sq, B.vol, K.key, evw, evq, B.tr_k, B.tr_vol, B.tr_pas);
      else
        full = events_key_r8m(checked, k, nev, tmask, B.tr_n, K.sq, B.vol, K.key, evw, evq, B.tr_k, B.tr_vol, B.tr_pas);
      if (B.tr_n) B.trade_vol += wave_add((uint32_t)lane < B.tr_n ? B.tr_vol : 0u);
      flush_trades_compact<R>(B, a, book, t0, lane, evw);
      if (!full) break;
    }
   } else {
#pragma unroll
    for (int re = 0; re < R; ++re) {
      const uint32_t kb = re * 64;
      if (n_ev > kb) {
        const uint32_t cnt = rfl((n_ev - kb) < 64u ? (n_ev - kb) : 64u);
        for (uint32_t l = 0; l < cnt; ++l) {
          const uint32_t ew = rdl(evm[re], l);
          slot_event_keyed<R, 0, CLS>(B, K, a, book, t0, lane, kb + l, CLS ? (ew & EV_SLOT) : ew, ew, evm);
        }
      }
    }
    listed = true;
    flush_trades_compact<R>(B, a, book, t0, lane, evm);
   }
    keys_end<R>(B, K);
  } else
#pragma unroll
  for (int re = 0; re < R; ++re) {
    const uint32_t kb = re * 64;
    if (n_ev > kb) {
      const uint32_t cnt = rfl((n_ev - kb) < 64u ? (n_ev - kb) : 64u);
      for (uint32_t l = 0; l < cnt; ++l) {
        uint32_t slot = rdl(ev[re], l);
        const uint32_t ew = slot;
        if (CLS) slot &= EV_SLOT;
        if (MKT && TAGGED) {
          if ((slot >> 12) != asset) continue;
          slot &= 0xFFFu;
          ++n_own;
        } else if (MKT) {
          if (!mask_test<R>(mine, slot)) continue;
          ++n_own;
        }
        process_slot_event<R, 0, CLS, LOG>(B, a, book, t0, lane, kb + l, slot, ew, lg...);
      }
    }
  }
  if (!MKT) n_own = n_ev;
  if (MKTK && listed) n_own = own_cnt;
  B.n_events += n_own;
  B.t = t0 + step_size;
  snapshot<R>(B, a, book, lane, bins, hist_slot, B.flags, write_last, tick);
  flush_trades<R>(B, a, book, t0, lane);
  return (uint32_t)(B.n_trades - trades_before);
}

constexpr int LDS_DW_PER_WAVE = 4 * 64;

template <int R>
__global__ __launch_bounds__(256) void k_run_random(DevArgs a, uint64_t first_step, uint32_t n_steps) {
  __shared__ uint32_t lds[4][LDS_DW_PER_WAVE];
  const int lane = threadIdx.x & 63;
  const int wv = threadIdx.x >> 6;
  const uint32_t book = rfl(blockIdx.x * 4 + wv);
  if (book >= a.n_books) return;
  uint32_t* st = a.state + (size_t)book * a.state_stride;
  uint32_t* bins = lds[wv];

  Book<R> B;
  Rng rng;
  load_book<R>(B, rng, st, lane);
  uint32_t last_ntr = 0, last_nev = 0;
  uint32_t ev[R];
#pragma unroll
  for (int r = 0; r < R; ++r) ev[r] = 0;

  for (uint32_t s = 0; s < n_steps; ++s) {
    uint32_t n_ev = 0;
    {
      uint32_t g = 0;
      Group G = a.groups[0];
      uint32_t gend = G.n;
      uint32_t n = 0;
#pragma unroll
      for (int r = 0; r < R; ++r) {
        for (uint32_t l = 0; l < 64; ++l, ++n) {
          if (n >= a.n_agents_total) break;
          while (n >= gend) {
            ++g;
            G = a.groups[g];
            gend += G.n;
          }
          const uint32_t x = rng.next_u32();
          if ((x >> 8) < G.thr) {
            slot_write<R>(ev, n_ev, n);
            n_ev += 1;
            const uint64_t bit = 1ull << l;
            if (!(B.live[r] & bit)) {
              const uint32_t side = rng.below(2u, 0x7FFFFFFFu);
              const uint32_t tick = G.tick_lo + rng.below(G.tick_rng, G.tick_zone);
              const uint32_t vol = G.vol_lo + rng.below(G.vol_rng, G.vol_zone);
              B.price[r] = wrl(tick * G.tick_size, l, B.price[r]);
              B.vol[r] = wrl(vol, l, B.vol[r]);
              B.id[r] = wrl(B.next_id, l, B.id[r]);
              B.next_id += 1;
              B.bid[r] = side ? (B.bid[r] | bit) : (B.bid[r] & ~bit);
              B.pend[r] |= bit;
            }
          }
        }
      }
    }
    for (uint32_t i = n_ev; i-- > 1;) {
      const uint32_t j = rng.below(i + 1);
      const uint32_t ai = slot_read<R>(ev, i), aj = slot_read<R>(ev, j);
      slot_write<R>(ev, i, aj);
      slot_write<R>(ev, j, ai);
    }
    last_ntr = step_from_list<R>(B, a, book, lane, ev, n_ev, bins, a.hist_cap ? (a.hist_slot0 + s) % a.hist_cap : 0u,
                                 s + 1 == n_steps || a.hist_cap == 0, a.tick_div, B.pend, last_nev);
  }
  store_book<R>(B, rng, st, lane, first_step + n_steps, last_ntr, last_nev);
}

enum Phase : uint32_t { PH_ACT = 0, PH_SIDE = 1, PH_TICK = 2, PH_VOL = 3, PH_SHUF = 4, PH_DONE = 5 };

#ifndef BOURSE_AMD_FSM_TOP_VGPR
#define BOURSE_AMD_FSM_TOP_VGPR 231
#endif
#define BK_STR2(x) #x
#define BK_STR(x) BK_STR2(x)

constexpr uint32_t fsm_lds_bytes(int R) { return 64u * R * 32u * 4u; }

struct LaneGroup {
  uint4 a, b;
  uint32_t tick_size;
};
__device__ __forceinline__ LaneGroup load_lane_group(const Group* g) {
  const uint4* q = reinterpret_cast<const uint4*>(g);
  return LaneGroup{q[0], q[1], g->tick_size};
}

template <int R>
__global__ __launch_bounds__(64) void k_agents_fsm(DevArgs a) {
  extern __shared__ uint32_t fsm_lds[];
#define BK_PB 0
#include "agents_fsm_body.inc"
#undef BK_PB
}

template <int R>
__device__ __forceinline__ void agents_fsm_pb(const DevArgs& a, const Group* table, uint32_t* fsm_lds) {
#define BK_PB 1
#include "agents_fsm_body.inc"
#undef BK_PB
}
template <int R, bool PB>
__global__ __launch_bounds__(64) void k_agents_fsm(DevArgs a, const Group* table) {
  static_assert(PB, "the uniform form is k_agents_fsm<R>(DevArgs)");
  extern __shared__ uint32_t fsm_lds[];
  agents_fsm_pb<R>(a, table, fsm_lds);
}

template <int R, bool MKT, bool POOLPEND, bool LOG = false>
__device__ __forceinline__ void step_batch_book(const DevArgs& a, uint32_t book, int lane, uint32_t* lds, uint64_t step_index,
                                                uint32_t write_last, Book<R>& B, Rng& rng, uint32_t hist_slot,
                                                uint4* dorders = nullptr);
template <int R, bool MKT, bool POOLPEND, bool LOG = false>
__device__ __forceinline__ void step_batch_raw(const DevArgs& a, uint32_t book, int lane, uint32_t* lds, uint64_t step_index,
                                               uint32_t write_last, const StepRaw<R>& w, Book<R>& B, Rng& rng, uint32_t hist_slot,
                                               uint4* dorders = nullptr);
template <int R, bool MKT, bool POOLPEND = false>
#ifndef BOURSE_AMD_SB8_TOP_VGPR
#define BOURSE_AMD_SB8_TOP_VGPR 95
#endif
__global__ __launch_bounds__(64, R >= 8 ? 5 : 1) void k_step_batch(DevArgs a, uint64_t step_index, uint32_t write_last) {
  __shared__ uint32_t lds[LDS_DW_PER_WAVE];
#if BOURSE_AMD_SB8_TOP_VGPR > 0
  if constexpr (R >= 8) asm volatile("" ::: "v" BK_STR(BOURSE_AMD_SB8_TOP_VGPR));
#endif
  if (a.step_prio) __builtin_amdgcn_s_setprio(1);
  const int lane = threadIdx.x;
  const uint32_t book = MKT ? a.book_begin * a.assets + blockIdx.x : a.book_begin + blockIdx.x;
  if (book >= (MKT ? a.book_end * a.assets : a.book_end)) return;
  Book<R> B;
  Rng rng;
  step_batch_book<R, MKT, POOLPEND>(a, book, lane, lds, step_index, write_last, B, rng, a.hist_slot0);
}

template <int R, bool MKT>
__global__ __launch_bounds__(64) void k_step_batch_log(DevArgs a, uint64_t step_index, uint32_t write_last, uint4* dorders) {
  __shared__ uint32_t lds[LDS_DW_PER_WAVE];
  if (a.step_prio) __builtin_amdgcn_s_setprio(1);
  const int lane = threadIdx.x;
  const uint32_t book = MKT ? a.book_begin * a.assets + blockIdx.x : a.book_begin + blockIdx.x;
  if (book >= (MKT ? a.book_end * a.assets : a.book_end)) return;
  Book<R> B;
  Rng rng;
  step_batch_book<R, MKT, false, true>(a, book, lane, lds, step_index, write_last, B, rng, a.hist_slot0, dorders);
}

template <int R, bool MKT, bool POOLPEND, bool LOG>
__device__ __forceinline__ void step_batch_book(const DevArgs& a, uint32_t book, int lane, uint32_t* lds, uint64_t step_index,
                                                uint32_t write_last, Book<R>& B, Rng& rng, uint32_t hist_slot, uint4* dorders) {
  StepRaw<R> w;
  const uint32_t mkt_book0 = MKT ? (book / a.assets) * a.assets : book;
  const uint32_t* st = a.state + (size_t)book * a.state_stride;
  const uint32_t* bt = a.batch + (size_t)mkt_book0 * a.batch_stride;
  load_state_raw<R>(w, st, lane);
  w.bh = bt[lane];
#pragma unroll
  for (int r = 0; r < R; ++r) {
    w.ev[r] = reinterpret_cast<const uint16_t*>(bt + BT_EV)[r * 64 + lane];
    w.pv[r] = POOLPEND ? make_uint2(0u, 0u) : reinterpret_cast<const uint2*>(bt + BT_EV + 32 * R)[r * 64 + lane];
  }
  load_state_scalars<R>(w, st);
  step_batch_raw<R, MKT, POOLPEND, LOG>(a, book, lane, lds, step_index, write_last, w, B, rng, hist_slot, dorders);
}
template <int R, bool MKT, bool POOLPEND, bool LOG>
__device__ __forceinline__ void step_batch_raw(const DevArgs& a, uint32_t book, int lane, uint32_t* lds, uint64_t step_index,
                                               uint32_t write_last, const StepRaw<R>& w, Book<R>& B, Rng& rng, uint32_t hist_slot,
                                               uint4* dorders) {
  const uint32_t mkt_book0 = MKT ? (book / a.assets) * a.assets : book;
  const uint32_t asset = book - mkt_book0;
  uint32_t* st = a.state + (size_t)book * a.state_stride;
  uint64_t mine[R];
#pragma unroll
  for (int r = 0; r < R; ++r) mine[r] = MKT ? 0ull : ~0ull;
  if (MKT) {
    uint32_t gb = 0;
    for (uint32_t g = 0; g < a.n_groups; ++g) {
      const uint32_t ge = gb + a.groups[g].n;
      if (a.groups[g].asset == asset) {
#pragma unroll
        for (int r = 0; r < R; ++r) {
          const uint32_t lo = gb > 64u * r ? gb : 64u * r, hi = ge < 64u * r + 64u ? ge : 64u * r + 64u;
          if (lo < hi) mine[r] |= ((hi - lo) == 64u ? ~0ull : ((1ull << (hi - lo)) - 1ull)) << (lo - 64u * r);
        }
      }
      gb = ge;
    }
  }

  unpack_book<R>(B, rng, w);
  const uint32_t n_ev = rdl(w.bh, BT_NEV);
  uint32_t ev[R];
  uint32_t owner[R];
  uint32_t base = B.next_id;
#pragma unroll
  for (int r = 0; r < R; ++r) ev[r] = w.ev[r];
  uint32_t mw = 0;
  if (!POOLPEND) {
    uint32_t* pm = lds;
    if (lane < 4 * R) pm[lane] = 0;
#pragma unroll
    for (int r = 0; r < R; ++r) {
      const uint32_t ew = ev[r], slot = ew & EV_SLOT, bit = 1u << (slot & 31);
      const bool is_new = (uint32_t)(r * 64 + lane) < n_ev && (ew & EV_NEW);
      atomicOr(&pm[slot >> 5], is_new ? bit : 0u);
      atomicOr(&pm[2 * R + (slot >> 5)], (is_new && (ew & EV_BID)) ? bit : 0u);
    }
    mw = pm[lane & (4 * R - 1)];
  }
#pragma unroll
  for (int r = 0; r < R; ++r) {
    if (POOLPEND) {
      owner[r] = w.f[r][4] & 0xFF00u;
      continue;
    }
    const uint64_t pend = mk64(rdl(mw, 2 * r), rdl(mw, 2 * r + 1)) & mine[r];
    const uint64_t side = mk64(rdl(mw, 2 * R + 2 * r), rdl(mw, 2 * R + 2 * r + 1));
    const uint2 pv = w.pv[r];
    B.price[r] = sel(pend, pv.x, B.price[r]);
    B.vol[r] = sel(pend, pv.y, B.vol[r]);
    const uint32_t rank = __builtin_amdgcn_mbcnt_hi((uint32_t)(pend >> 32), __builtin_amdgcn_mbcnt_lo((uint32_t)pend, 0u));
    B.id[r] = sel(pend, base + rank, B.id[r]);
    if constexpr (LOG) {
      const uint32_t slot = 64u * r + (uint32_t)lane, id = base + rank;
      uint32_t trader = 0, gb = 0;
      for (uint32_t g = 0; g < a.n_groups; ++g) {
        const uint32_t ge = gb + a.groups[g].n;
        trader = (slot >= gb && slot < ge) ? slot - gb : trader;
        gb = ge;
      }
      if (lane_bit(pend) && id < a.log_cap) {
        uint4* d = dorders + ((size_t)book * a.log_cap + id) * 2;
        d[0] = make_uint4(pv.y, trader, pv.x, (uint32_t)lane_bit(side));
        d[1] = make_uint4((uint32_t)B.t, (uint32_t)(B.t >> 32), 0u, 0u);
      }
    }
    base += __builtin_popcountll(pend);
    B.bid[r] = (B.bid[r] & ~pend) | (side & pend);
    B.pend[r] = pend;
  }
  B.next_id = base;
  uint32_t n_own = 0;
  uint32_t ntr;
  if constexpr (LOG)
    ntr = step_from_list<R, MKT, false, true, false, true>(B, a, book, lane, ev, n_ev, lds, hist_slot, write_last != 0,
                                                           MKT ? a.asset_div[asset] : a.tick_div, mine, n_own, asset,
                                                           LogCtx{a.order_log + (size_t)book * a.log_cap, a.log_cap});
  else
    ntr = step_from_list<R, MKT, MKT && POOLPEND, !POOLPEND, POOLPEND && !MKT>(B, a, book, lane, ev, n_ev, lds, hist_slot,
                                                                               write_last != 0, MKT ? a.asset_div[asset] : a.tick_div,
                                                                               mine, n_own, asset);
  store_book<R, !POOLPEND>(B, rng, st, lane, step_index + 1, ntr, n_own);
  if (POOLPEND) {
#pragma unroll
    for (int r = 0; r < R; ++r) {
      uint32_t* p = st + HDR_DW + r * POOL_FIELDS * 64 + 4 * 64;
      p[lane] = (lane_bit(B.live[r]) ? 1u : 0u) | (lane_bit(B.bid[r]) ? 2u : 0u) | owner[r];
    }
  }
}


#ifndef BOURSE_AMD_FSM_UNIT
__global__ void k_book_service(uint32_t* state, uint32_t stride, uint32_t n_books, int op, uint32_t value) {
  const uint32_t b = blockIdx.x * blockDim.x + threadIdx.x;
  if (b >= n_books) return;
  uint32_t* h = state + (size_t)b * stride;
  if (op == 0) {
    h[H_TRADE_BASE_LO] = h[H_TRADES_LO];
    h[H_TRADE_BASE_HI] = h[H_TRADES_HI];
  } else if (op == 1) {
    h[H_TRADING] = value;
  } else if (op == 2) {
    h[H_FLAGS] &= ~value;
  }
}

struct IngestArgs {
  const unsigned long long* off;
  const uint32_t* action;
  const uint8_t* side;
  const uint32_t* vol;
  const uint32_t* trader;
  const uint32_t* price;
  const unsigned long long* order_id;
  unsigned long long* out_ids;
  uint32_t* status;
  uint4* q;
  uint32_t* qlen;
  uint32_t qcap;
  uint4* dorders;
  uint32_t* mods_flag;
};
constexpr uint32_t ING_ACTION_MODIFY = 0x80000003u;
constexpr uint32_t ING_OK = 0u, ING_PRICE = 1u, ING_CAPACITY = 3u;

__global__ __launch_bounds__(64) void k_ingest(DevArgs a, IngestArgs g) {
  const int lane = threadIdx.x;
  const uint32_t mkt = blockIdx.x, M = a.assets;
  uint32_t qn = g.qlen[mkt];
  uint4* q = g.q + (size_t)mkt * g.qcap;
  for (uint32_t asset = 0; asset < M; ++asset) {
    const uint32_t book = mkt * M + asset;
    uint32_t* hdr = a.state + (size_t)book * a.state_stride;
    const uint32_t tick = a.asset_tick[asset];
    uint32_t next_id = rfl(hdr[H_NEXT_ID]);
    const uint32_t t_lo = rfl(hdr[H_T_LO]), t_hi = rfl(hdr[H_T_HI]);
    const unsigned long long lo = g.off[book], hi = g.off[book + 1];
    uint32_t code = ING_OK;
    unsigned long long applied = 0;
    for (unsigned long long base = lo; base < hi && code == ING_OK; base += 64) {
      const unsigned long long i = base + (uint32_t)lane;
      const bool in = i < hi;
      const uint32_t act = in ? g.action[i] : 0u, sd = in ? g.side[i] : 0u, vol = in ? g.vol[i] : 0u;
      const uint32_t price = in ? g.price[i] : 0u, trader = in ? g.trader[i] : 0u;
      const unsigned long long oid = in ? g.order_id[i] : 0ull;
      const bool is_new = act == 1u, is_ev = act == 1u || act == 2u || act == ING_ACTION_MODIFY;
      if (g.mods_flag && __ballot(in && act == ING_ACTION_MODIFY) && lane == 0) *g.mods_flag = 1u;
      const uint64_t badm = __ballot(is_new && price % tick != 0u);
      uint32_t cut = badm ? (uint32_t)__builtin_ctzll(badm) : 64u;
      if (badm) code = ING_PRICE;
      uint64_t evm = __ballot(in && is_ev && (uint32_t)lane < cut);
      const uint32_t room = g.qcap - qn;
      if ((uint32_t)__builtin_popcountll(evm) > room) {
        uint64_t m = evm;
        for (uint32_t r = 0; r < room; ++r) m &= m - 1ull;
        cut = (uint32_t)__builtin_ctzll(m);
        code = ING_CAPACITY;
        evm = __ballot(in && is_ev && (uint32_t)lane < cut);
      }
      if ((uint64_t)next_id + 64u >= 0xFFFFFFFFull) {
        cut = 0;
        code = ING_CAPACITY;
        evm = 0;
      }
      const bool valid = in && (uint32_t)lane < cut;
      const uint64_t newm = __ballot(valid && is_new);
      const uint32_t rank_ev = __builtin_amdgcn_mbcnt_hi((uint32_t)(evm >> 32), __builtin_amdgcn_mbcnt_lo((uint32_t)evm, 0u));
      const uint32_t rank_new = __builtin_amdgcn_mbcnt_hi((uint32_t)(newm >> 32), __builtin_amdgcn_mbcnt_lo((uint32_t)newm, 0u));
      const uint32_t id = next_id + rank_new;
      if (valid && is_ev) {
        uint4 e;
        const uint32_t idc = oid > 0xFFFFFFFFull ? 0xFFFFFFFFu : (uint32_t)oid;
        if (is_new) {
          e = make_uint4(0u | ((sd & 1u) << 8) | (asset << 16), id, price, vol);
        } else if (act == 2u) {
          e = make_uint4(1u | (asset << 16), idc, 0u, 0u);
        } else {
          e = make_uint4(2u | ((sd & 2u) ? 1u << 9 : 0u) | ((sd & 4u) ? 1u << 10 : 0u) | (asset << 16), idc, price, vol);
        }
        q[qn + rank_ev] = e;
      }
      if (valid && is_new && id < a.log_cap) {
        uint4* d = g.dorders + ((size_t)book * a.log_cap + id) * 2;
        d[0] = make_uint4(vol, trader, price, sd & 1u);
        d[1] = make_uint4(t_lo, t_hi, 0u, 0u);
        uint4* l = reinterpret_cast<uint4*>(a.order_log + (size_t)book * a.log_cap + id);
        l[0] = make_uint4(0u, vol, price, price);
        l[1] = make_uint4(t_lo, t_hi, 0xFFFFFFFFu, 0xFFFFFFFFu);
        l[2] = make_uint4(0u, 0u, 0u, 0u);
      }
      if (valid && g.out_ids) g.out_ids[i] = is_new ? (unsigned long long)id : ~0ull;
      next_id += (uint32_t)__builtin_popcountll(newm);
      qn += (uint32_t)__builtin_popcountll(evm);
      applied += cut < 64u ? cut : (hi - base < 64ull ? hi - base : 64ull);
    }
    if (lane == 0) {
      hdr[H_NEXT_ID] = next_id;
      if (g.status) {
        g.status[2 * book] = code;
        g.status[2 * book + 1] = applied > 0xFFFFFFFFull ? 0xFFFFFFFFu : (uint32_t)applied;
      }
    }
  }
  if (lane == 0) g.qlen[mkt] = qn;
}

__global__ void k_flags_summary(const uint32_t* state, uint32_t stride, uint32_t n_books, uint32_t* out ) {
  const uint32_t b = blockIdx.x * blockDim.x + threadIdx.x;
  uint32_t f = 0, r = 0;
  if (b < n_books) {
    const uint32_t* h = state + (size_t)b * stride;
    f = h[H_FLAGS];
    const uint64_t n = mk64(h[H_TRADES_LO], h[H_TRADES_HI]) - mk64(h[H_TRADE_BASE_LO], h[H_TRADE_BASE_HI]);
    r = n > 0xFFFFFFFFull ? 0xFFFFFFFFu : (uint32_t)n;
  }
  for (int o = 32; o > 0; o >>= 1) {
    f |= (uint32_t)__shfl_xor((int)f, o);
    r = max(r, (uint32_t)__shfl_xor((int)r, o));
  }
  if ((threadIdx.x & 63) == 0 && (f | r)) {
    if (f) atomicOr(&out[0], f);
    atomicMax(&out[1], r);
  }
}

__global__ void k_gather_header(const uint32_t* state, uint32_t stride, uint32_t word, uint32_t n_words, uint32_t n_books,
                                unsigned long long* out) {
  const uint32_t b = blockIdx.x * blockDim.x + threadIdx.x;
  if (b >= n_books) return;
  const uint32_t* h = state + (size_t)b * stride + word;
  out[b] = n_words == 2 ? mk64(h[0], h[1]) : (unsigned long long)h[0];
}

__global__ void k_delay(uint32_t ticks) {
// ... 134 lines not shown
```

bourse_amd/csrc/bourse_amd.hip:

```cpp
#include <hip/hip_runtime.h>

#include <algorithm>
#include <array>
#include <chrono>
#include <cmath>
#include <cstdio>
#include <cstdlib>
#include <atomic>
#include <condition_variable>
#include <cstring>
#include <functional>
#include <map>
#include <memory>
#include <mutex>
#include <string>
#include <thread>
#include <type_traits>
#include <vector>

#include "../../include/bourse_amd.h"
#include "book_device.hpp"
namespace bkd {
extern template __global__ void k_agents_fsm<1>(DevArgs);
extern template __global__ void k_agents_fsm<2>(DevArgs);
// ... 44 lines not shown
  g_err = msg;
  return code;
}

#define HIPCHK(expr)                                                                              \
  do {                                                                                            \
    hipError_t _e = (expr);                                                                       \
    if (_e != hipSuccess)                                                                         \
      return fail(BK_HIP_ERROR, std::string(#expr) + ": " + hipGetErrorString(_e));               \
  } while (0)

struct HostOrder {
  uint8_t bid;
  uint32_t start_vol, price, trader;
  uint64_t create_time;
};
struct HostEvent {
  uint32_t word, id, price, vol;
};
static_assert(sizeof(HostEvent) == 16, "HostEvent is uploaded as one uint4 per event");
struct BookHost {
  std::vector<HostOrder> orders;
  std::vector<HostEvent> queue;
  std::vector<DevOrderLog> log_cache;
  uint64_t n_uploaded = 0;
  uint64_t time_offset = 0;
  bool log_fresh = false;
  uint64_t mirror_epoch = ~0ull;
};

template <class T>
struct DevBuf {
  T* p = nullptr;
  size_t n = 0;
  ~DevBuf() {
    if (p) (void)hipFree(p);
  }
  hipError_t alloc(size_t count) {
    if (p) (void)hipFree(p);
    p = nullptr;
    n = count;
    if (count == 0) return hipSuccess;
    return hipMalloc(reinterpret_cast<void**>(&p), count * sizeof(T));
  }
};

}

struct bk_env {
  bk_config cfg{};
  int R = 1;
  uint32_t M = 1;
  uint32_t asset_tick[MAX_ASSETS] = {0, 0, 0, 0, 0, 0, 0, 0};
  uint32_t W = 0, stride = 0;
  hipStream_t stream = nullptr;
  DevBuf<uint32_t> state, l2_last, hist, ev_off, batch;
  DevBuf<uint4> ev;
  HostEvent* ev_stage = nullptr;
  uint32_t* off_stage = nullptr;
  uint32_t batch_stride = 0;
  int pipeline = 0;
  DevBuf<uint32_t> warm_snap;
  bool warming = false;
  struct Snapshot {
    DevBuf<uint32_t> buf;
    bool used = false;
    uint64_t shape[4] = {0, 0, 0, 0};
  } snaps[BK_MAX_SNAPSHOTS];
  DevBuf<uint8_t> reset_mask;
  DevBuf<uint64_t> reset_seeds;
  struct IngressSnapshot {
    DevBuf<uint32_t> buf;
    DevBuf<uint4> orders, log;
    uint32_t n_keep = 0, keep_cap = 0;
    DevBuf<uint32_t> held, lists, lens, mflags;
    DevBuf<uint64_t> mstate;
    bool held_saved = false, members_saved = false;
    bool used = false;
    uint64_t shape[4] = {0, 0, 0, 0};
    uint64_t installs = 0;
    uint64_t bytes = 0;
  } isnaps[BK_MAX_SNAPSHOTS];
  DevBuf<uint32_t> reset_list;
  int reset_blocks = 0;
  DevBuf<bk_u32x4> acct;
  DevBuf<unsigned long long> acct_seen;
  DevBuf<uint8_t> acct_mask;
  uint32_t acct_traders = 0;
  bool acct_consume = false;
  DevBuf<bk_u32x4> open_summary;
  DevBuf<bk_u32x4> open_entries;
  uint32_t open_traders = 0, open_depth = 0;
  uint64_t agent_installs = 0;
  DevBuf<uint4> jump_tabs;
  DevBuf<uint32_t> wcache;
  uint32_t wave_lookahead = 64;
  uint32_t stagger_us = ~0u;
  int wave_parts = 0;
  bool wl_valid = false;
  DevBuf<uint16_t> wl_list;
  DevBuf<uint32_t> wl_len;
  bool mw_attr_set = false;
  uint32_t fused_resident = 0;
  bool step_decode = false;
  int n_parts = 4;
  uint32_t min_part = 4096;
  static constexpr int MAX_PARTS = 8;
  hipStream_t part_stream[MAX_PARTS] = {};
  hipEvent_t ev_fork = nullptr, ev_first[MAX_PARTS] = {}, ev_join[MAX_PARTS] = {};
  DevBuf<DevTrade> trades;
  DevBuf<DevOrderLog> order_log;
  DevBuf<DevStats> stats;
  DevBuf<OutTrade> tr_dense;
  DevBuf<unsigned long long> tr_off;
  uint64_t tr_total = 0;
  DevBuf<MixedDesc> mixed_descs;
  std::vector<MixedDesc> mtable;
  DevBuf<MixedDesc> dmtable;
  uint32_t n_mixed = 0, n_fixed = 0;
  DevBuf<uint16_t> ml_list;
  DevBuf<uint32_t> ml_len, ml_inl;
  bool lds_attr_set = false;
  DevBuf<uint64_t> gather_buf;
  bool fsm_attr_set = false;
  bool ml_valid = false;
  uint32_t member_asset[MAX_MEMBERS] = {0, 0, 0, 0};
  uint32_t n_fixed_a[MAX_ASSETS] = {0, 0, 0, 0, 0, 0, 0, 0};
  MixedLists lists() const {
    return MixedLists{ml_list.p, ml_len.p, ml_inl.p, static_cast<uint32_t>(R) * 64u, cfg.n_books, cfg.n_books / M};
  }
  MixedArgs margs() const {
    MixedArgs ma{};
    ma.descs = mixed_descs.p;
    ma.n_desc = n_mixed;
    ma.n_fixed = n_fixed;
    for (int i = 0; i < MAX_MEMBERS; ++i) ma.asset[i] = member_asset[i];
    for (int i = 0; i < MAX_ASSETS; ++i) ma.n_fixed_a[i] = n_fixed_a[i];
    return ma;
  }
  std::vector<BookHost> books;
  std::unique_ptr<HostPool> pool;
  HostPool& host_pool() {
    if (!pool) {
      unsigned nt = std::min<unsigned>(std::max(1u, std::thread::hardware_concurrency()), 16u);
      if (const char* e = std::getenv("BOURSE_AMD_HOST_THREADS")) nt = static_cast<unsigned>(std::max(1, std::atoi(e)));
      pool.reset(new HostPool(nt - 1));
    }
    return *pool;
  }
  std::vector<Group> groups;
  std::vector<Group> table;
  DevBuf<Group> dtable;
  uint32_t n_agents_total = 0;
  uint64_t agents_hash = 0;
  bool device_ingress = false;
  uint32_t qcap = 0;
  DevBuf<uint4> dq, dorders;
  DevBuf<uint32_t> dqlen;
  uint64_t ingest_epoch = 0;
  DevBuf<uint32_t> agent_held;
  DevBuf<Group> agent_groups;
  bool agent_held_stale = true;
  DevBuf<uint32_t> member_lists, member_lens, member_flags, member_id0_dev;
  DevBuf<uint64_t> member_state;
  std::vector<uint32_t> member_id0;
  std::vector<uint32_t> member_type, member_n;
  uint32_t member_list_cap = 0;
  bool member_lists_stale = true;
  bool agent_log = false;
  struct HostIngress {
    static constexpr int SLOTS = 2;
    size_t cap = 0;
    char* pin[SLOTS] = {nullptr, nullptr};
    char* dev[SLOTS] = {nullptr, nullptr};
    hipStream_t in = nullptr, out = nullptr;
    hipEvent_t e_h2d[SLOTS] = {}, e_ing[SLOTS] = {}, e_done[SLOTS] = {};
    uint64_t ticket_of[SLOTS] = {~0ull, ~0ull};
    uint64_t n_elem[SLOTS] = {0, 0};
    uint64_t next_ticket = 0;
    struct Retired {
      char* pin;
      uint64_t free_from_ticket;
    };
    std::vector<Retired> retired;
    size_t o_off = 0, o_oid = 0, o_out = 0, o_st = 0, o_act = 0, o_vol = 0, o_trd = 0, o_prc = 0, o_side = 0, bytes = 0;
    void layout(size_t B, size_t c) {
      cap = c;
      o_off = 0;
      o_oid = o_off + (B + 1) * 8;
      o_out = o_oid + c * 8;
      o_st = o_out + c * 8;
      o_act = o_st + B * 8;
      o_vol = o_act + c * 4;
      o_trd = o_vol + c * 4;
      o_prc = o_trd + c * 4;
      o_side = o_prc + c * 4;
      bytes = (o_side + c + 63) & ~size_t(63);
    }
  } hi;
  bool ev_seq_shuffle = false;
  int ev_shuffle_min = -1;
  std::atomic<bool> ev_mods_seen{false};
  uint32_t* mods_flag_host = nullptr;
  uint32_t* mods_flag_dev = nullptr;
  bool device_flow = false;
  uint64_t steps_done = 0, hist_base = 0;
  uint32_t trading = 1;
  size_t ev_capacity = 0;
  int profile = 0;
  uint64_t prof_tick = 0;
  bool prof_now = false;
  struct ProfEv {
    hipEvent_t a, b;
    int kind;
  };
  std::vector<ProfEv> prof_events;
  double prof_bracket_ms = 0;
  std::vector<hipEvent_t> prof_pool;
  hipEvent_t prof_event() {
    hipEvent_t e = nullptr;
    if (!prof_pool.empty()) {
      e = prof_pool.back();
      prof_pool.pop_back();
    } else if (hipEventCreate(&e) != hipSuccess) {
      e = nullptr;
    }
    return e;
  }
  static constexpr int PROF_KINDS = 4;
  double prof_ms[PROF_KINDS] = {0, 0, 0, 0};
  uint64_t prof_launches[PROF_KINDS] = {0, 0, 0, 0};

  DevArgs args() const {
    DevArgs a{};
    a.n_books = cfg.n_books;
    a.levels = cfg.levels;
    a.tick_size = cfg.tick_size;
    a.n_groups = static_cast<uint32_t>(groups.size());
    a.step_lo = static_cast<uint32_t>(cfg.step_size);
    a.step_hi = static_cast<uint32_t>(cfg.step_size >> 32);
    a.state_stride = stride;
    a.l2_width = W;
    a.trade_cap = warming ? 0u : cfg.trade_capacity;
    a.hist_cap = warming ? 0u : cfg.history_capacity;
    a.hist_slot0 = a.hist_cap ? static_cast<uint32_t>(steps_done % cfg.history_capacity) : 0u;
    a.step_prio = 0;
    a.n_agents_total = n_agents_total;
    a.log_cap = cfg.max_orders;
    a.state = state.p;
    a.l2_last = l2_last.p;
    a.hist = hist.p;
    a.trades = trades.p;
    a.order_log = order_log.p;
    a.ev_off = ev_off.p;
    a.ev = device_ingress ? dq.p : ev.p;
    a.ev_len = device_ingress ? dqlen.p : nullptr;
    a.ev_stride = qcap;
    a.batch = batch.p;
    a.batch_stride = batch_stride;
    a.book_begin = 0;
    a.book_end = cfg.n_books / M;
    a.assets = M;
    for (int i = 0; i < MAX_ASSETS; ++i) a.asset_tick[i] = asset_tick[i];
    auto dv = [](uint32_t d) {
      const HostUDiv h = make_udiv(d ? d : 1u);
      return UDiv{h.m, h.sh1, h.sh2, h.d};
    };
    a.tick_div = dv(cfg.tick_size);
    for (int i = 0; i < MAX_ASSETS; ++i) a.asset_div[i] = dv(asset_tick[i]);
    for (size_t g = 0; g < groups.size(); ++g) a.groups[g] = groups[g];
    return a;
  }
};

namespace {

int use_device(bk_env* env) {
  HIPCHK(hipSetDevice(env->cfg.device));
  return BK_OK;
}

struct ProfScope {
  bk_env* env;
  int kind;
  hipStream_t st;
  hipEvent_t a = nullptr, b = nullptr;
  ProfScope(bk_env* e, int k, hipStream_t s = nullptr) : env(e), kind(k), st(s ? s : e->stream) {
    if (env->prof_now && hipEventCreate(&a) == hipSuccess && hipEventCreate(&b) == hipSuccess)
      (void)hipEventRecord(a, st);
  }
  ~ProfScope() {
    if (a && b) {
      (void)hipEventRecord(b, st);
      env->prof_events.push_back({a, b, kind});
    }
  }
};

template <typename K, typename... Args>
void launch_timed(bk_env* env, int kind, K kernel, dim3 grid, dim3 block, uint32_t lds, hipStream_t st, Args... args) {
  hipEvent_t a = nullptr, b = nullptr;
  const uint64_t every = env->profile == 1 ? 1u : 2u * static_cast<uint64_t>(env->profile) + 1u;
  const bool sample = env->profile > 0 && (env->prof_tick++ % every) == 0;
  if (sample && (a = env->prof_event()) && (b = env->prof_event())) {
    (void)hipEventRecord(a, st);
    hipLaunchKernelGGL(kernel, grid, block, lds, st, args...);
    (void)hipEventRecord(b, st);
    env->prof_events.push_back({a, b, kind});
  } else {
    hipLaunchKernelGGL(kernel, grid, block, lds, st, args...);
  }
}

template <typename F>
auto by_R(int R, F&& f) {
  switch (R) {
    case 1: return f(std::integral_constant<int, 1>{});
    case 2: return f(std::integral_constant<int, 2>{});
    case 4: return f(std::integral_constant<int, 4>{});
    default: return f(std::integral_constant<int, 8>{});
  }
}

int wave_args(bk_env* env, WaveArgs* wva);
template <int R>
int launch_events(bk_env* env, const DevArgs& a, uint64_t step_index, uint32_t max_queue) {
  env->prof_now = env->profile > 0;
  ProfScope ps(env, 3);
  uint32_t perm_bytes = ((max_queue + 63u) & ~63u) * 2u + 128u;
  if (perm_bytes < ev_lds_bytes(R)) perm_bytes = ev_lds_bytes(R);
  if (max_queue > 64u * R) perm_bytes = std::max(perm_bytes, ((max_queue + 63u) & ~63u) * 2u + ev_keyed_lds_bytes(R));
  const bool seq_shuffle = env->ev_seq_shuffle;
  const int min_env = env->ev_shuffle_min;
  const uint32_t shuffle_min = min_env >= 0 ? static_cast<uint32_t>(min_env) : (12u * R > 32u ? 12u * R : 32u);
  WaveArgs wva{};
  if (!seq_shuffle && max_queue >= shuffle_min && max_queue >= 2u)
    if (int rc = wave_args(env, &wva)) return rc;
  const bool chunks = max_queue > 64u * R;
  const dim3 grid(env->cfg.n_books), block(64);
  if (env->mods_flag_host && *static_cast<volatile uint32_t*>(env->mods_flag_host)) env->ev_mods_seen.store(true, std::memory_order_relaxed);
  if constexpr (R == 8) {
    if (!chunks && !env->ev_mods_seen.load(std::memory_order_relaxed)) {
      if (env->M == 1)
        hipLaunchKernelGGL((k_step_events<R, false, false, false>), grid, block, perm_bytes, env->stream, a, wva, step_index, shuffle_min, perm_bytes);
      else
        hipLaunchKernelGGL((k_step_events<R, true, false, false>), grid, block, perm_bytes, env->stream, a, wva, step_index, shuffle_min, perm_bytes);
      HIPCHK(hipGetLastError());
      return BK_OK;
    }
  }
  if (env->M == 1 && !chunks)
    hipLaunchKernelGGL((k_step_events<R, false, false>), grid, block, perm_bytes, env->stream, a, wva, step_index, shuffle_min, perm_bytes);
  else if (env->M == 1)
    hipLaunchKernelGGL((k_step_events<R, false, true>), grid, block, perm_bytes, env->stream, a, wva, step_index, shuffle_min, perm_bytes);
  else if (!chunks)
    hipLaunchKernelGGL((k_step_events<R, true, false>), grid, block, perm_bytes, env->stream, a, wva, step_index, shuffle_min, perm_bytes);
  else
    hipLaunchKernelGGL((k_step_events<R, true, true>), grid, block, perm_bytes, env->stream, a, wva, step_index, shuffle_min, perm_bytes);
  HIPCHK(hipGetLastError());
  return BK_OK;
}

int wave_args(bk_env* env, WaveArgs* wva) {
  if (!env->jump_tabs.p) {
    std::vector<uint32_t> all;
    for (int t = 0; t < 7; ++t) {
      const std::vector<uint32_t> tab = xoroshiro_jump_table(t == 0 ? WV_BLOCK : static_cast<uint64_t>(WV_K) << (t - 1));
      all.insert(all.end(), tab.begin(), tab.end());
    }
    HIPCHK(env->jump_tabs.alloc(all.size() / 4));
    HIPCHK(env->wcache.alloc(static_cast<size_t>(env->cfg.n_books) * WC_STRIDE));
    HIPCHK(hipMemcpyAsync(env->jump_tabs.p, all.data(), all.size() * 4, hipMemcpyHostToDevice, env->stream));
    HIPCHK(hipMemsetAsync(env->wcache.p, 0, static_cast<size_t>(env->cfg.n_books) * WC_STRIDE * 4, env->stream));
    HIPCHK(hipStreamSynchronize(env->stream));
  }
  wva->jt_block = env->jump_tabs.p;
  wva->jt_lane = env->jump_tabs.p + 512;
  wva->wcache = env->wcache.p;
  wva->lookahead = env->wave_lookahead;
  return BK_OK;
}

const std::vector<hipStream_t>& part_streams(int device) {
  static std::mutex mu;
  static std::map<int, std::vector<hipStream_t>> pool;
  std::lock_guard<std::mutex> lk(mu);
  auto it = pool.find(device);
  if (it != pool.end()) return it->second;
  std::vector<hipStream_t> cand, chosen;
  if (const char* e = std::getenv("BOURSE_AMD_PART_STREAMS")) {
    const int want = std::atoi(e);
    if (want >= 1 && want <= 8) {
      for (int k = 0; k < want; ++k) {
        hipStream_t st = nullptr;
        if (hipStreamCreateWithFlags(&st, hipStreamNonBlocking) != hipSuccess) break;
        chosen.push_back(st);
      }
      (void)hipGetLastError();
      if (getenv("BOURSE_AMD_VERBOSE"))
        fprintf(stderr, "bourse_amd: device %d: %zu part streams taken unprobed (BOURSE_AMD_PART_STREAMS)\n", device, chosen.size());
      return pool.emplace(device, std::move(chosen)).first->second;
    }
  }
  for (int k = 0; k < 8; ++k) {
    hipStream_t st = nullptr;
    if (hipStreamCreateWithFlags(&st, hipStreamNonBlocking) != hipSuccess) break;
    hipLaunchKernelGGL(k_delay, dim3(1), dim3(64), 0, st, 1u);
    cand.push_back(st);
  }
  (void)hipDeviceSynchronize();
  constexpr uint32_t SPIN_US = 300;
  auto concurrent = [&](hipStream_t x, hipStream_t y) {
    for (int attempt = 0; attempt < 2; ++attempt) {
      const auto t0 = std::chrono::steady_clock::now();
// ... 6 lines not shown
    }
    return false;
  };
  for (hipStream_t c : cand) {
    bool ok = chosen.size() < 4;
    for (size_t j = 0; ok && j < chosen.size(); ++j) ok = concurrent(c, chosen[j]);
    if (ok)
      chosen.push_back(c);
    else
      (void)hipStreamDestroy(c);
  }
  (void)hipGetLastError();
  if (getenv("BOURSE_AMD_VERBOSE"))
    fprintf(stderr, "bourse_amd: device %d: %zu of %zu candidate streams on hardware queues of their own\n", device,
            chosen.size(), cand.size());
  if (chosen.size() < 4 && !cand.empty())
    fprintf(stderr, "bourse_amd: warning: device %d: only %zu of %zu candidate streams run concurrently (busy GPU or serialised "
            "kernels?): multi-part launches will overlap less; BOURSE_AMD_PART_STREAMS=4 skips the probe\n", device,
            chosen.size(), cand.size());
  return pool.emplace(device, std::move(chosen)).first->second;
}

template <int R>
int prepare_launch(bk_env* env, const Plan& pl, const DevArgs& a0, WaveArgs* wva) {
  switch (pl.kind) {
    case PL_FUSED_RANDOM: break;
    case PL_SPLIT_LANES:
    case PL_SPLIT_WAVE:
      if (!env->fsm_attr_set) {
        HIPCHK(hipFuncSetAttribute(reinterpret_cast<const void*>(&k_agents_fsm<R>), hipFuncAttributeMaxDynamicSharedMemorySize,
                                   static_cast<int>(fsm_lds_bytes(R))));
        HIPCHK(hipFuncSetAttribute(reinterpret_cast<const void*>(&k_agents_fsm<R, true>),
                                   hipFuncAttributeMaxDynamicSharedMemorySize, static_cast<int>(fsm_lds_bytes(R))));
        env->fsm_attr_set = true;
      }
      if (pl.kind == PL_SPLIT_WAVE) return wave_args(env, wva);
      break;
    case PL_FUSED_WAVE: return wave_args(env, wva);
    case PL_MIXED_LANES: {
      const size_t NB = env->cfg.n_books, cap = static_cast<size_t>(R) * 64, NU = NB / env->M;
      if (!env->ml_list.p) {
        HIPCHK(env->ml_list.alloc(MAX_MEMBERS * cap * NU));
        HIPCHK(env->ml_len.alloc(MAX_MEMBERS * NU));
        HIPCHK(env->ml_inl.alloc(2 * static_cast<size_t>(R) * NB));
        env->ml_valid = false;
      }
      if (!env->lds_attr_set) {
        HIPCHK(hipFuncSetAttribute(reinterpret_cast<const void*>(&k_agents_mixed_lanes<R, true>),
                                   hipFuncAttributeMaxDynamicSharedMemorySize, static_cast<int>(mixed_lanes_lds_bytes(R, true))));
        HIPCHK(hipFuncSetAttribute(reinterpret_cast<const void*>(&k_agents_mixed_lanes<R, false>),
                                   hipFuncAttributeMaxDynamicSharedMemorySize, static_cast<int>(mixed_lanes_lds_bytes(R, false))));
        HIPCHK(hipFuncSetAttribute(reinterpret_cast<const void*>(&k_agents_mixed_lanes<R, true, true>),
                                   hipFuncAttributeMaxDynamicSharedMemorySize, static_cast<int>(mixed_lanes_pb_lds_bytes(R, true))));
        HIPCHK(hipFuncSetAttribute(reinterpret_cast<const void*>(&k_agents_mixed_lanes<R, false, true>),
                                   hipFuncAttributeMaxDynamicSharedMemorySize, static_cast<int>(mixed_lanes_pb_lds_bytes(R, false))));
        env->lds_attr_set = true;
      }
      if (!env->ml_valid) {
        hipLaunchKernelGGL(k_mixed_lists_rebuild<R>, dim3((env->cfg.n_books + 3) / 4), dim3(256), 0, env->stream, a0, env->margs(),
                           env->lists());
        HIPCHK(hipGetLastError());
        env->ml_valid = true;
      }
      env->wl_valid = false;
      break;
    }
    case PL_MIXED_WPB:
    case PL_MIXED_FUSED:
      env->ml_valid = false;
      env->wl_valid = false;
      break;
    case PL_MIXED_WAVE:
      if (int rc = wave_args(env, wva)) return rc;
      if (!env->mw_attr_set) {
        HIPCHK(hipFuncSetAttribute(reinterpret_cast<const void*>(&k_agents_mixed_wave<R>), hipFuncAttributeMaxDynamicSharedMemorySize,
                                   static_cast<int>(mixed_wave_lds_bytes(R))));
        HIPCHK(hipFuncSetAttribute(reinterpret_cast<const void*>(&k_agents_mixed_wave<R, true>),
                                   hipFuncAttributeMaxDynamicSharedMemorySize, static_cast<int>(mixed_wave_lds_bytes(R))));
        env->mw_attr_set = true;
      }
      if (!env->wl_list.p) {
        HIPCHK(env->wl_list.alloc(static_cast<size_t>(env->cfg.n_books) * MAX_MEMBERS * R * 64));
        HIPCHK(env->wl_len.alloc(static_cast<size_t>(env->cfg.n_books) * MAX_MEMBERS));
        env->wl_valid = false;
      }
      if (!env->wl_valid) {
        hipLaunchKernelGGL(k_wave_lists_rebuild<R>, dim3((env->cfg.n_books + 3) / 4), dim3(256), 0, env->stream, a0, env->margs(),
                           WaveLists{env->wl_list.p, env->wl_len.p, static_cast<uint32_t>(R) * 64u});
        HIPCHK(hipGetLastError());
        env->wl_valid = true;
      }
      env->ml_valid = false;
      break;
  }
  return BK_OK;
}

int prepare_parts(bk_env* env) {
  if (env->ev_fork) return BK_OK;
  const std::vector<hipStream_t>& ps = part_streams(env->cfg.device);
  if (ps.empty()) return fail(BK_HIP_ERROR, "could not create the parts' streams");
  for (int i = 0; i < bk_env::MAX_PARTS; ++i) {
    env->part_stream[i] = ps[static_cast<size_t>(i) % ps.size()];
    if (!env->ev_first[i]) HIPCHK(hipEventCreateWithFlags(&env->ev_first[i], hipEventDisableTiming));
    if (!env->ev_join[i]) HIPCHK(hipEventCreateWithFlags(&env->ev_join[i], hipEventDisableTiming));
  }
  HIPCHK(hipEventCreateWithFlags(&env->ev_fork, hipEventDisableTiming));
  return BK_OK;
}

template <int R>
int launch_fused(bk_env* env, const Plan& pl, const DevArgs& a, const WaveArgs& wva, uint64_t first_step, uint32_t n_steps) {
  const uint32_t nb = env->cfg.n_books;
  env->prof_now = env->profile > 0;
  ProfScope ps(env, 0);
  if (pl.kind == PL_MIXED_FUSED && pl.members_per_book)
    hipLaunchKernelGGL((k_run_mixed<R, true>), dim3((nb + 3) / 4), dim3(256), 0, env->stream, a, env->margs(), first_step, n_steps,
                       static_cast<const MixedDesc*>(env->dmtable.p));
  else if (pl.kind == PL_MIXED_FUSED)
    hipLaunchKernelGGL(k_run_mixed<R>, dim3((nb + 3) / 4), dim3(256), 0, env->stream, a, env->margs(), first_step, n_steps);
  else if (pl.kind == PL_FUSED_WAVE && pl.agents_per_book)
    hipLaunchKernelGGL((k_run_wave<R, true>), dim3((nb + 7) / 8), dim3(512), 0, env->stream, a, wva, first_step, n_steps,
                       static_cast<const Group*>(env->dtable.p));
  else if (pl.kind == PL_FUSED_WAVE)
    hipLaunchKernelGGL(k_run_wave<R>, dim3((nb + 7) / 8), dim3(512), 0, env->stream, a, wva, first_step, n_steps);
  else
    hipLaunchKernelGGL(k_run_random<R>, dim3((nb + 3) / 4), dim3(256), 0, env->stream, a, first_step, n_steps);
  HIPCHK(hipGetLastError());
  return BK_OK;
}

template <int R>
int launch_split(bk_env* env, const Plan& pl, const DevArgs& a0, const WaveArgs& wva, uint64_t first_step, uint32_t n_steps) {
  const MixedArgs ma = env->margs();
  const MixedLists ml = env->lists();
  const uint32_t M = env->M;
  const uint32_t B = env->cfg.n_books / M;
  const Group* table = env->dtable.p;
  const MixedDesc* mtable = env->dmtable.p;
  const int P = pl.parts;
  if (P > 1) {
    if (int rc = prepare_parts(env)) return rc;
    HIPCHK(hipEventRecord(env->ev_fork, env->stream));
    for (int i = 0; i < P; ++i) HIPCHK(hipStreamWaitEvent(env->part_stream[i], env->ev_fork, 0));
  }
  for (uint32_t s = 0; s < n_steps; ++s) {
    env->prof_now = false;
    for (int i = 0; i < P; ++i) {
      DevArgs a = a0;
      a.book_begin = static_cast<uint32_t>(static_cast<uint64_t>(B) * i / P) & ~3u;
      a.book_end = (i + 1 == P) ? B : (static_cast<uint32_t>(static_cast<uint64_t>(B) * (i + 1) / P) & ~3u);
      a.hist_slot0 = a.hist_cap ? static_cast<uint32_t>((first_step + s) % a.hist_cap) : 0u;
      a.step_prio = pl.step_prio ? 1u : 0u;
      const uint32_t nb = a.book_end - a.book_begin;
      hipStream_t st = P > 1 ? env->part_stream[i] : env->stream;
      if (P > 1 && s == 0 && i > 0) {
        if (pl.stagger_us > 0)
          hipLaunchKernelGGL(k_delay, dim3(1), dim3(64), 0, st, static_cast<uint32_t>(i) * pl.stagger_us * 100u);
        else
          HIPCHK(hipStreamWaitEvent(st, env->ev_first[i - 1], 0));
      }
      const uint64_t step_no = first_step + s;
      if (pl.agents == AG_MIXED_WAVE && pl.members_per_book)
        launch_timed(env, 1, &k_agents_mixed_wave<R, true>, dim3((nb + MW_WPB - 1) / MW_WPB), dim3(64 * MW_WPB),
                     static_cast<uint32_t>(mixed_wave_lds_bytes(R)), st, a, ma, wva,
                     WaveLists{env->wl_list.p, env->wl_len.p, static_cast<uint32_t>(R) * 64u}, mtable);
      else if (pl.agents == AG_MIXED_WAVE)
        launch_timed(env, 1, &k_agents_mixed_wave<R>, dim3((nb + MW_WPB - 1) / MW_WPB), dim3(64 * MW_WPB),
                     static_cast<uint32_t>(mixed_wave_lds_bytes(R)), st, a, ma, wva,
                     WaveLists{env->wl_list.p, env->wl_len.p, static_cast<uint32_t>(R) * 64u});
      else if (pl.agents == AG_MIXED_LANES_MKT && pl.members_per_book)
        launch_timed(env, 1, &k_agents_mixed_lanes<R, true, true>, dim3((nb + 63) / 64), dim3(64), mixed_lanes_pb_lds_bytes(R, true),
                     st, a, ma, ml, mtable);
      else if (pl.agents == AG_MIXED_LANES && pl.members_per_book)
        launch_timed(env, 1, &k_agents_mixed_lanes<R, false, true>, dim3((nb + 63) / 64), dim3(64),
                     mixed_lanes_pb_lds_bytes(R, false), st, a, ma, ml, mtable);
      else if (pl.agents == AG_MIXED_WPB && pl.members_per_book)
        launch_timed(env, 1, &k_agents_mixed<R, true>, dim3((nb + 3) / 4), dim3(256), 0u, st, a, ma, mtable);
      else if (pl.agents == AG_MIXED_LANES_MKT)
        launch_timed(env, 1, &k_agents_mixed_lanes<R, true>, dim3((nb + 63) / 64), dim3(64), mixed_lanes_lds_bytes(R, true), st, a,
                     ma, ml);
      else if (pl.agents == AG_MIXED_LANES)
        launch_timed(env, 1, &k_agents_mixed_lanes<R, false>, dim3((nb + 63) / 64), dim3(64), mixed_lanes_lds_bytes(R, false), st,
                     a, ma, ml);
      else if (pl.agents == AG_MIXED_WPB)
        launch_timed(env, 1, &k_agents_mixed<R>, dim3((nb + 3) / 4), dim3(256), 0u, st, a, ma);
      else if (pl.agents == AG_WAVE && pl.step_decode && s > 0)
        ;
      else if (pl.agents == AG_WAVE && pl.agents_per_book)
        launch_timed(env, 1, &k_agents_wave<R, true>, dim3((nb + 3) / 4), dim3(256), 0u, st, a, wva, table);
      else if (pl.agents == AG_WAVE)
        launch_timed(env, 1, &k_agents_wave<R>, dim3((nb + 3) / 4), dim3(256), 0u, st, a, wva);
      else if (pl.agents_per_book)
        launch_timed(env, 1, &k_agents_fsm<R, true>, dim3((nb + 63) / 64), dim3(64), fsm_lds_bytes(R), st, a, table);
      else
        launch_timed(env, 1, &k_agents_fsm<R>, dim3((nb + 63) / 64), dim3(64), fsm_lds_bytes(R), st, a);
      if (P > 1 && s == 0) HIPCHK(hipEventRecord(env->ev_first[i], st));
      const uint32_t write_last = (s + 1 == n_steps || a.hist_cap == 0 || pl.write_last) ? 1u : 0u;
      if (pl.step_log && pl.step_mkt)
        launch_timed(env, 2, &k_step_batch_log<R, true>, dim3(nb * M), dim3(64), 0u, st, a, step_no, write_last, env->dorders.p);
      else if (pl.step_log)
        launch_timed(env, 2, &k_step_batch_log<R, false>, dim3(nb), dim3(64), 0u, st, a, step_no, write_last, env->dorders.p);
      else if (pl.step_poolpend && pl.step_mkt)
        launch_timed(env, 2, &k_step_batch<R, true, true>, dim3(nb * M), dim3(64), 0u, st, a, step_no, write_last);
      else if (pl.step_poolpend)
        launch_timed(env, 2, &k_step_batch<R, false, true>, dim3(nb), dim3(64), 0u, st, a, step_no, write_last);
      else if (pl.step_mkt)
        launch_timed(env, 2, &k_step_batch<R, true>, dim3(nb * M), dim3(64), 0u, st, a, step_no, write_last);
      else if (pl.step_decode && s + 1 < n_steps)
        launch_timed(env, 2, &k_step_decode<R>, dim3((nb + 3) / 4), dim3(256), 0u, st, a, wva, step_no, write_last);
      else
        launch_timed(env, 2, &k_step_batch<R, false>, dim3(nb), dim3(64), 0u, st, a, step_no, write_last);
    }
  }
  HIPCHK(hipGetLastError());
  if (P > 1) {
    for (int i = 0; i < P; ++i) {
      HIPCHK(hipEventRecord(env->ev_join[i], env->part_stream[i]));
      HIPCHK(hipStreamWaitEvent(env->stream, env->ev_join[i], 0));
    }
  }
  return BK_OK;
}

int order_after(hipStream_t later, hipStream_t earlier) {
  hipEvent_t ev = nullptr;
  HIPCHK(hipEventCreateWithFlags(&ev, hipEventDisableTiming));
  hipError_t e = hipEventRecord(ev, earlier);
  if (e == hipSuccess) e = hipStreamWaitEvent(later, ev, 0);
  (void)hipEventDestroy(ev);
  if (e != hipSuccess) return fail(BK_HIP_ERROR, std::string("stream ordering: ") + hipGetErrorString(e));
  return BK_OK;
}

int host_flow_ok(bk_env* env) {
  if (env->device_ingress)
    return fail(BK_INVALID_ARGUMENT, "this env takes its instructions from device memory (bk_device_ingress_enable): "
                                     "per-order host calls would collide with the ids assigned on the device");
  if (env->device_flow)
    return fail(BK_INVALID_ARGUMENT, "host-driven orders cannot be mixed with bk_run's on-device agents on the same env");
  return BK_OK;
}

int check_book(bk_env* env, uint32_t book) {
  if (!env) return fail(BK_INVALID_ARGUMENT, "null env");
  if (book >= env->cfg.n_books) return fail(BK_INVALID_ARGUMENT, "book index out of range");
  return BK_OK;
}

int refresh_log(bk_env* env, uint32_t book) {
  BookHost& bh = env->books[book];
  if (bh.log_fresh) return BK_OK;
  const uint64_t n = std::min<uint64_t>(bh.n_uploaded, env->cfg.max_orders);
  bh.log_cache.resize(n);
  if (n) {
    HIPCHK(hipStreamSynchronize(env->stream));
    HIPCHK(hipMemcpy(bh.log_cache.data(), env->order_log.p + static_cast<size_t>(book) * env->cfg.max_orders,
                     n * sizeof(DevOrderLog), hipMemcpyDeviceToHost));
  }
  bh.log_fresh = true;
  return BK_OK;
}

int mirror_orders(bk_env* env, uint32_t book) {
  if (!env->device_ingress && !env->agent_log) return BK_OK;
  BookHost& bh = env->books[book];
  if (bh.mirror_epoch == env->ingest_epoch) return BK_OK;
  HIPCHK(hipSetDevice(env->cfg.device));
  HIPCHK(hipStreamSynchronize(env->stream));
  uint32_t count = 0;
  HIPCHK(hipMemcpy(&count, env->state.p + static_cast<size_t>(book) * env->stride + H_NEXT_ID, 4, hipMemcpyDeviceToHost));
  const uint64_t logged = std::min<uint64_t>(count, env->cfg.max_orders);
  std::vector<uint4> rows(logged * 2);
  if (logged)
    HIPCHK(hipMemcpy(rows.data(), env->dorders.p + static_cast<size_t>(book) * env->cfg.max_orders * 2, logged * 32,
                     hipMemcpyDeviceToHost));
  bh.orders.assign(count, HostOrder{0, 0, 0, 0, 0});
  for (uint64_t id = 0; id < logged; ++id) {
    const uint4 a = rows[2 * id], b = rows[2 * id + 1];
    bh.orders[id] = HostOrder{static_cast<uint8_t>(a.w & 1u), a.x, a.z, a.y, (static_cast<uint64_t>(b.y) << 32) | b.x};
  }
  bh.n_uploaded = count;
  bh.log_fresh = false;
  bh.mirror_epoch = env->ingest_epoch;
  return BK_OK;
}

int prof_collect(bk_env* env) {
  HIPCHK(hipStreamSynchronize(env->stream));
  for (auto& pr : env->prof_events) {
    float ms = 0.f;
    if (hipEventElapsedTime(&ms, pr.a, pr.b) == hipSuccess) {
      env->prof_ms[pr.kind] += std::max(0.0, static_cast<double>(ms) - env->prof_bracket_ms);
      env->prof_launches[pr.kind] += 1;
    }
    env->prof_pool.push_back(pr.a);
    env->prof_pool.push_back(pr.b);
  }
  env->prof_events.clear();
  return BK_OK;
}

void fill_order(const bk_env* env, const BookHost& bh, uint64_t id, bk_order* o) {
  const HostOrder& h = bh.orders[id];
  std::memset(o, 0, sizeof(*o));
  o->side_is_bid = h.bid;
// ... 775 lines not shown
  g.state = env->state.p;
  g.state_stride = env->stride;
  g.n_agents = NA;
  g.log_cap = env->cfg.max_orders;
  g.qcap = env->qcap;
  g.groups = env->table.empty() ? env->agent_groups.p : env->dtable.p;
  g.g_stride = env->table.empty() ? 0u : static_cast<uint32_t>(env->groups.size());
  g.held = env->agent_held.p;
  g.q = env->dq.p;
  g.qlen = env->dqlen.p;
  g.dorders = env->dorders.p;
  g.order_log = env->order_log.p;
  by_R(env->R, [&](auto r) {
    hipLaunchKernelGGL(k_update_agents<decltype(r)::value>, dim3(B), dim3(64), 0, env->stream, g);
    return 0;
  });
  HIPCHK(hipGetLastError());
  env->ingest_epoch += 1;
  return BK_OK;
}

int bk_update_members(bk_env* env) {
  if (!env) return fail(BK_INVALID_ARGUMENT, "null env");
  if (!env->device_ingress)
    return fail(BK_INVALID_ARGUMENT, "bk_update_members queues the members' orders in the device-resident queues: call "
                                     "bk_device_ingress_enable first");
  if (env->M > 1) return fail(BK_INVALID_ARGUMENT, "bk_update_members runs an AgentSet on independent books (assets == 1)");
  if (!env->n_mixed) {
    if (!env->groups.empty())
      return fail(BK_INVALID_ARGUMENT, "this env has RandomAgents groups only (bk_set_random_agents*): they are run by "
                                       "bk_update_agents");
    return fail(BK_INVALID_ARGUMENT, "no AgentSet installed (bk_set_agents / bk_set_agents_per_book)");
  }
  if (int rc = use_device(env)) return rc;
  const uint32_t B = env->cfg.n_books, NM = env->n_mixed;
  if (env->member_lists_stale) {
    HIPCHK(hipStreamSynchronize(env->stream));
    uint32_t max_n = 0;
    for (uint32_t n : env->member_n) max_n = std::max(max_n, n);
    env->member_list_cap = bkd::ingress::members_list_cap(static_cast<uint32_t>(env->R), max_n);
    const size_t rows = static_cast<size_t>(B) * NM;
    HIPCHK(env->member_lists.alloc(rows * env->member_list_cap));
    HIPCHK(env->member_lens.alloc(rows));
    HIPCHK(env->member_state.alloc(rows * 2));
    HIPCHK(env->member_flags.alloc(B));
    HIPCHK(env->member_id0_dev.alloc(env->member_id0.size()));
    HIPCHK(hipMemset(env->member_lists.p, 0xFF, rows * env->member_list_cap * 4));
    HIPCHK(hipMemset(env->member_lens.p, 0, rows * 4));
    HIPCHK(hipMemset(env->member_state.p, 0, rows * 16));
    HIPCHK(hipMemset(env->member_flags.p, 0, static_cast<size_t>(B) * 4));
    HIPCHK(hipMemcpy(env->member_id0_dev.p, env->member_id0.data(), env->member_id0.size() * 4, hipMemcpyHostToDevice));
    env->member_lists_stale = false;
  }
  bkd::ingress::MembersIngressArgs g{};
  g.state = env->state.p;
  g.state_stride = env->stride;
  g.n_members = NM;
  g.log_cap = env->cfg.max_orders;
  g.qcap = env->qcap;
  g.tick = env->cfg.tick_size;
  g.descs = env->mtable.empty() ? env->mixed_descs.p : env->dmtable.p;
  g.id_start = env->member_id0_dev.p;
  g.d_stride = env->mtable.empty() ? 0u : NM;
  g.list_cap = env->member_list_cap;
  g.lists = env->member_lists.p;
  g.lens = env->member_lens.p;
  g.mstate = env->member_state.p;
  g.mflags = env->member_flags.p;
  g.q = env->dq.p;
  g.qlen = env->dqlen.p;
  g.dorders = env->dorders.p;
  g.order_log = env->order_log.p;
  by_R(env->R, [&](auto r) {
    hipLaunchKernelGGL(bkd::ingress::k_update_members<decltype(r)::value>, dim3(B), dim3(64), 0, env->stream, g);
    return 0;
  });
  HIPCHK(hipGetLastError());
  env->ingest_epoch += 1;
  return BK_OK;
}

int bk_member_orders(bk_env* env, uint32_t book, uint32_t member, uint32_t cap, uint64_t* out_ids, uint32_t* n_out) {
  if (int rc = check_book(env, book)) return rc;
  if (!env->device_ingress || !env->n_mixed)
    return fail(BK_INVALID_ARGUMENT, "bk_member_orders reads the lists of bk_update_members: no AgentSet on a device-ingress env");
  if (member >= env->n_mixed) return fail(BK_INVALID_ARGUMENT, "member index out of range");
  if (cap && !out_ids) return fail(BK_INVALID_ARGUMENT, "null argument");
  if (int rc = use_device(env)) return rc;
  const bool random = env->member_type[member] == BK_AGENT_RANDOM;
  uint32_t n = random ? env->member_n[member] : 0u;
  std::vector<uint32_t> ids(n, AGENT_HELD_NONE);
  if (!env->member_lists_stale) {
    HIPCHK(hipStreamSynchronize(env->stream));
    const size_t row = static_cast<size_t>(book) * env->n_mixed + member;
    if (!random) HIPCHK(hipMemcpy(&n, env->member_lens.p + row, 4, hipMemcpyDeviceToHost));
    n = std::min(n, env->member_list_cap);
    ids.resize(n);
    if (n) HIPCHK(hipMemcpy(ids.data(), env->member_lists.p + row * env->member_list_cap, n * 4ull, hipMemcpyDeviceToHost));
  }
  for (uint32_t i = 0; i < n && i < cap; ++i) out_ids[i] = ids[i] == AGENT_HELD_NONE ? ~0ull : ids[i];
  if (n_out) *n_out = n;
  return BK_OK;
}

int bk_order_status(bk_env* env, uint32_t book, uint64_t order_id, uint8_t* out_status) {
  if (int rc = check_book(env, book)) return rc;
  if (int rc = mirror_orders(env, book)) return rc;
  BookHost& bh = env->books[book];
  if (order_id >= bh.orders.size())
    return fail(BK_UNKNOWN_ORDER_ID, "No order with id " + std::to_string(order_id) + " exists");
  if (env->cfg.max_orders == 0) return fail(BK_INVALID_ARGUMENT, "order log disabled (max_orders == 0)");
  if (order_id >= env->cfg.max_orders) return fail(BK_CAPACITY, "order id beyond the order-log capacity");
  if (int rc = use_device(env)) return rc;
  if (int rc = refresh_log(env, book)) return rc;
  bk_order o;
  fill_order(env, bh, order_id, &o);
  if (out_status) *out_status = o.status;
  return BK_OK;
}

int bk_order_count(bk_env* env, uint32_t book, uint64_t* out) {
  if (int rc = check_book(env, book)) return rc;
  if (int rc = mirror_orders(env, book)) return rc;
  if (out) *out = env->books[book].orders.size();
  return BK_OK;
}

int bk_get_orders(bk_env* env, uint32_t book, uint64_t first, uint64_t n, bk_order* out) {
  if (int rc = check_book(env, book)) return rc;
  if (int rc = mirror_orders(env, book)) return rc;
  BookHost& bh = env->books[book];
  if (first > bh.orders.size() || n > bh.orders.size() - first) return fail(BK_INVALID_ARGUMENT, "order range out of bounds");
  if (n && !out) return fail(BK_INVALID_ARGUMENT, "null argument");
  if (bh.orders.size() > env->cfg.max_orders && env->cfg.max_orders > 0 && bh.n_uploaded > env->cfg.max_orders)
    return fail(BK_CAPACITY, "order log capacity exceeded");
  if (int rc = use_device(env)) return rc;
  if (env->cfg.max_orders)
    if (int rc = refresh_log(env, book)) return rc;
  for (uint64_t i = 0; i < n; ++i) fill_order(env, bh, first + i, out + i);
  return BK_OK;
}

int bk_set_random_market_agents(bk_env* env, uint32_t n_groups, const bk_random_agents* groups,
                                const uint32_t* assets) {
  if (!env || (!groups && n_groups)) return fail(BK_INVALID_ARGUMENT, "null argument");
  if (n_groups > MAX_GROUPS) return fail(BK_INVALID_ARGUMENT, "at most 8 agent groups");
  std::vector<Group> gs(n_groups);
  uint64_t total = 0;
  std::string msg;
  if (int rc = make_groups(groups, n_groups, assets, env->M, env->asset_tick, gs.data(), &total, &msg))
    return fail(rc, msg);
  if (total > env->cfg.max_live_orders) return fail(BK_CAPACITY, CAPACITY_MSG);
  env->groups = gs;
  env->n_agents_total = static_cast<uint32_t>(total);
  env->n_mixed = 0;
  env->table.clear();
  (void)env->dtable.alloc(0);
  env->mtable.clear();
  (void)env->dmtable.alloc(0);
  env->agents_hash = gs.empty() ? 0 : groups_hash(gs.data(), gs.size());
  env->agent_held_stale = true;
  env->agent_installs += 1;
  return BK_OK;
}

int bk_set_random_agents_per_book(bk_env* env, uint32_t n_groups, const bk_random_agents* groups, const uint32_t* assets) {
  if (!env || (!groups && n_groups)) return fail(BK_INVALID_ARGUMENT, "null argument");
  if (n_groups == 0) return fail(BK_INVALID_ARGUMENT, "a per-unit table needs at least one group");
  if (n_groups > MAX_GROUPS) return fail(BK_INVALID_ARGUMENT, "at most 8 agent groups");
  const uint32_t n_units = env->cfg.n_books / env->M;
  std::vector<Group> t;
  uint64_t total = 0;
  std::string msg;
  if (int rc = make_group_table(groups, n_units, n_groups, assets, env->M, env->asset_tick, env->cfg.max_live_orders, t, &total, &msg))
    return fail(rc, msg);
  if (int rc = use_device(env)) return rc;
  DevBuf<Group> d;
  HIPCHK(d.alloc(t.size()));
  HIPCHK(hipMemcpy(d.p, t.data(), t.size() * sizeof(Group), hipMemcpyHostToDevice));
  std::swap(env->dtable.p, d.p);
  std::swap(env->dtable.n, d.n);
  env->groups.assign(t.begin(), t.begin() + n_groups);
  env->table.swap(t);
  env->n_agents_total = static_cast<uint32_t>(total);
  env->n_mixed = 0;
  env->mtable.clear();
  (void)env->dmtable.alloc(0);
  env->agents_hash = groups_hash(env->table.data(), env->table.size());
  env->agent_held_stale = true;
  env->agent_installs += 1;
  return BK_OK;
}

int bk_set_random_agents(bk_env* env, uint32_t n_groups, const bk_random_agents* groups) {
  return bk_set_random_market_agents(env, n_groups, groups, nullptr);
}

int bk_set_tick_sizes(bk_env* env, uint32_t n, const uint32_t* tick_sizes) {
  if (!env || !tick_sizes) return fail(BK_INVALID_ARGUMENT, "null argument");
  if (n != env->M) return fail(BK_INVALID_ARGUMENT, "one tick size per asset");
  if (env->steps_done || !env->groups.empty()) return fail(BK_INVALID_ARGUMENT, "set the tick sizes before anything else");
  for (const BookHost& bh : env->books)
    if (!bh.orders.empty()) return fail(BK_INVALID_ARGUMENT, "set the tick sizes before anything else");
  for (uint32_t i = 0; i < n; ++i)
    if (tick_sizes[i] == 0) return fail(BK_INVALID_ARGUMENT, "tick_size must be > 0");
  for (uint32_t i = 0; i < n; ++i) env->asset_tick[i] = tick_sizes[i];
  return BK_OK;
}

static int set_agents_impl(bk_env* env, uint32_t n_members, const bk_agent_desc* members, const uint32_t* assets);
static int install_members(bk_env* env, const std::vector<MixedDesc>& ds, uint32_t n_members, const uint32_t* assets,
                           const uint32_t* fixed_a, std::vector<MixedDesc> table);

int bk_set_agents(bk_env* env, uint32_t n_members, const bk_agent_desc* members) {
  if (!env || (!members && n_members)) return fail(BK_INVALID_ARGUMENT, "null argument");
  if (env->M > 1) return fail(BK_INVALID_ARGUMENT, "markets (assets > 1) take bk_set_market_agents");
  return set_agents_impl(env, n_members, members, nullptr);
}

int bk_set_market_agents(bk_env* env, uint32_t n_members, const bk_agent_desc* members, const uint32_t* assets) {
  if (!env || (!members && n_members) || (!assets && n_members)) return fail(BK_INVALID_ARGUMENT, "null argument");
  for (uint32_t i = 0; i < n_members; ++i)
    if (assets[i] >= env->M) return fail(BK_INVALID_ARGUMENT, "member asset index out of range");
  return set_agents_impl(env, n_members, members, assets);
}

static int set_agents_impl(bk_env* env, uint32_t n_members, const bk_agent_desc* members, const uint32_t* assets) {
  bool all_random = true;
  for (uint32_t i = 0; i < n_members; ++i) all_random = all_random && members[i].type == BK_AGENT_RANDOM;
  if (all_random) {
    std::vector<bk_random_agents> g(n_members);
    for (uint32_t i = 0; i < n_members; ++i)
      g[i] = bk_random_agents{members[i].n_agents, members[i].tick_lo, members[i].tick_hi, members[i].vol_lo,
                              members[i].vol_hi, members[i].tick_size, members[i].activity_rate};
    return bk_set_random_market_agents(env, n_members, g.data(), assets);
  }
  if (n_members > MAX_MEMBERS) return fail(BK_INVALID_ARGUMENT, "at most 4 members in a set with Noise/Momentum agents");
  if (env->agent_log)
    return fail(BK_INVALID_ARGUMENT, "the agents' order log (bk_set_agent_order_log) records RandomAgents only: "
                                     "a set with Noise / Momentum members cannot be installed on a logging env");
  if (int rc = use_device(env)) return rc;
  std::vector<MixedDesc> ds(n_members);
  uint32_t fixed_a[MAX_ASSETS];
  std::string msg;
  if (int rc = make_mixed_descs(members, n_members, assets, env->asset_tick, ds.data(), fixed_a, &msg))
    return fail(rc, msg);
  if (!mixed_capacity_ok(fixed_a, env->M, env->cfg.max_live_orders)) return fail(BK_CAPACITY, MIXED_CAPACITY_MSG);
  if (int rc = install_members(env, ds, n_members, assets, fixed_a, {})) return rc;
  env->member_id0.resize(n_members);
  for (uint32_t i = 0; i < n_members; ++i) env->member_id0[i] = members[i].agent_id_start;
  return BK_OK;
}

static int install_members(bk_env* env, const std::vector<MixedDesc>& ds, uint32_t n_members, const uint32_t* assets,
                           const uint32_t* fixed_a, std::vector<MixedDesc> table) {
  DevBuf<MixedDesc> dt;
  if (!table.empty()) {
    HIPCHK(dt.alloc(table.size()));
    HIPCHK(hipMemcpy(dt.p, table.data(), table.size() * sizeof(MixedDesc), hipMemcpyHostToDevice));
  }
  uint32_t fixed = fixed_a[0];
  HIPCHK(env->mixed_descs.alloc(n_members));
  HIPCHK(hipMemcpy(env->mixed_descs.p, ds.data(), ds.size() * sizeof(MixedDesc), hipMemcpyHostToDevice));
  env->n_mixed = n_members;
  env->n_fixed = fixed;
  env->member_type.resize(n_members);
  env->member_n.resize(n_members);
  for (uint32_t i = 0; i < n_members; ++i) env->member_type[i] = ds[i].type, env->member_n[i] = ds[i].n;
  env->member_lists_stale = true;
  env->agent_installs += 1;
  env->wl_valid = false;
  for (uint32_t i = 0; i < MAX_MEMBERS; ++i) env->member_asset[i] = (assets && i < n_members) ? assets[i] : 0u;
  for (uint32_t as = 0; as < MAX_ASSETS; ++as) env->n_fixed_a[as] = fixed_a[as];
  env->ml_valid = false;
  env->groups.clear();
  env->table.clear();
  (void)env->dtable.alloc(0);
  env->n_agents_total = 0;
  std::swap(env->dmtable.p, dt.p);
  std::swap(env->dmtable.n, dt.n);
  env->mtable.swap(table);
  env->agents_hash = env->mtable.empty() ? mixed_hash(env->member_asset, ds.data(), ds.size())
                                         : mixed_hash(env->member_asset, env->mtable.data(), env->mtable.size());
  return BK_OK;
}

int bk_set_agents_per_book(bk_env* env, uint32_t n_members, const bk_agent_desc* members, const uint32_t* assets) {
  if (!env || (!members && n_members)) return fail(BK_INVALID_ARGUMENT, "null argument");
  if (n_members == 0) return fail(BK_INVALID_ARGUMENT, "a per-unit table needs at least one member");
  if (env->M > 1 && !assets) return fail(BK_INVALID_ARGUMENT, "markets (assets > 1) need the members' assets");
  for (uint32_t i = 0; assets && i < n_members; ++i)
    if (assets[i] >= env->M) return fail(BK_INVALID_ARGUMENT, "member asset index out of range");
  const uint32_t n_units = env->cfg.n_books / env->M;
  const size_t n = static_cast<size_t>(n_units) * n_members;
  bool all_random = true;
  for (size_t k = 0; k < n; ++k) all_random = all_random && members[k].type == BK_AGENT_RANDOM;
  if (all_random) {
    std::vector<bk_random_agents> g(n);
    for (size_t k = 0; k < n; ++k)
      g[k] = bk_random_agents{members[k].n_agents, members[k].tick_lo, members[k].tick_hi, members[k].vol_lo,
                              members[k].vol_hi, members[k].tick_size, members[k].activity_rate};
    return bk_set_random_agents_per_book(env, n_members, g.data(), assets);
  }
  if (n_members > MAX_MEMBERS) return fail(BK_INVALID_ARGUMENT, "at most 4 members in a set with Noise/Momentum agents");
  if (env->agent_log)
    return fail(BK_INVALID_ARGUMENT, "the agents' order log (bk_set_agent_order_log) records RandomAgents only: "
                                     "a set with Noise / Momentum members cannot be installed on a logging env");
  std::vector<MixedDesc> t;
  uint32_t fixed_a[MAX_ASSETS];
  std::string msg;
  if (int rc = make_mixed_table(members, n_units, n_members, assets, env->M, env->asset_tick, env->cfg.max_live_orders, t,
                                fixed_a, &msg))
    return fail(rc, msg);
  if (int rc = use_device(env)) return rc;
  const std::vector<MixedDesc> row0(t.begin(), t.begin() + n_members);
  if (int rc = install_members(env, row0, n_members, assets, fixed_a, std::move(t))) return rc;
  env->member_id0.resize(n);
  for (size_t k = 0; k < n; ++k) env->member_id0[k] = members[k].agent_id_start;
  return BK_OK;
}

static void query_fused_resident(bk_env* env) {
  if (hipSetDevice(env->cfg.device) != hipSuccess) return;
  int blocks = 0, cus = 0;
  hipError_t e = by_R(env->R, [&](auto r) {
    return hipOccupancyMaxActiveBlocksPerMultiprocessor(&blocks, k_run_wave<decltype(r)::value>, 512, 0);
  });
  if (e == hipSuccess) e = hipDeviceGetAttribute(&cus, hipDeviceAttributeMultiprocessorCount, env->cfg.device);
  if (e == hipSuccess && blocks > 0 && cus > 0) env->fused_resident = static_cast<uint32_t>(blocks) * 8u * static_cast<uint32_t>(cus);
  (void)hipGetLastError();
  if (getenv("BOURSE_AMD_VERBOSE"))
    fprintf(stderr, "bourse_amd: k_run_wave<%d>: %d workgroups per CU x %d CUs -> one round holds %u books\n", env->R, blocks, cus,
            env->fused_resident);
}

static Plan env_plan(bk_env* env) {
  PlanInput in{env->R, env->cfg.n_books, env->M, !env->groups.empty(), env->n_mixed, env->pipeline, env->n_parts, env->wave_parts,
               env->min_part, env->fused_resident, env->stagger_us, env->warming, env->step_decode, env->agent_log,
               !env->table.empty(), !env->mtable.empty()};
  if (!in.fused_resident && random_books(in)) {
    query_fused_resident(env);
    in.fused_resident = env->fused_resident;
  }
  return make_plan(in);
}

int bk_run(bk_env* env, uint64_t n_steps) {
  if (!env) return fail(BK_INVALID_ARGUMENT, "null env");
  if (n_steps == 0) return BK_OK;
  const Plan pl = env_plan(env);
  if (n_steps > 0xFFFFFFFFull) return fail(BK_INVALID_ARGUMENT, "n_steps too large for one launch");
  if (int rc = use_device(env)) return rc;
  if (env->device_ingress) return fail(BK_INVALID_ARGUMENT, "bk_run cannot be mixed with submitted instructions on the same env");
  for (const BookHost& bh : env->books)
    if (!bh.queue.empty() || !bh.orders.empty())
      return fail(BK_INVALID_ARGUMENT, "bk_run cannot be mixed with host-driven orders on the same env");
  DevArgs a = env->args();
  if (a.n_groups == 0) {
    a.groups[0] = Group{};
    a.n_agents_total = 0;
  }
  const uint32_t ns = static_cast<uint32_t>(n_steps);
  if (env->n_mixed || a.n_groups) env->device_flow = true;
  const int rc = by_R(env->R, [&](auto r) -> int {
    constexpr int R = decltype(r)::value;
    WaveArgs wva{};
    if (int rc = prepare_launch<R>(env, pl, a, &wva)) return rc;
    return is_split(pl.kind) ? launch_split<R>(env, pl, a, wva, env->steps_done, ns)
                             : launch_fused<R>(env, pl, a, wva, env->steps_done, ns);
  });
  if (rc != BK_OK) return rc;
  env->steps_done += n_steps;
  if (env->agent_log) env->ingest_epoch += 1;
  return BK_OK;
}

int bk_set_agent_order_log(bk_env* env, int on) {
  if (!env) return fail(BK_INVALID_ARGUMENT, "null env");
  if (!on) {
    if (env->agent_log) return fail(BK_INVALID_ARGUMENT, "the agents' order log cannot be switched off once it is on");
    return BK_OK;
  }
  if (env->agent_log) return BK_OK;
  if (env->cfg.max_orders == 0)
    return fail(BK_INVALID_ARGUMENT, "the agents' order log needs max_orders > 0 (its capacity per book)");
  if (env->steps_done || env->device_flow)
    return fail(BK_INVALID_ARGUMENT, "switch the agents' order log on before the env's first bk_run: it could not hold "
                                     "the orders created before");
  if (env->device_ingress)
    return fail(BK_INVALID_ARGUMENT, "this env takes its instructions from device memory (bk_device_ingress_enable), which "
                                     "logs its orders already");
  if (env->n_mixed)
    return fail(BK_INVALID_ARGUMENT, "the agents' order log records RandomAgents only: this env has an AgentSet with "
                                     "Noise / Momentum members");
  for (const BookHost& bh : env->books)
    if (!bh.orders.empty() || !bh.queue.empty())
      return fail(BK_INVALID_ARGUMENT, "the agents' order log is for bk_run's on-device agents: this env holds host-driven orders");
  if (int rc = use_device(env)) return rc;
  HIPCHK(env->dorders.alloc(static_cast<size_t>(env->cfg.n_books) * env->cfg.max_orders * 2));
  env->agent_log = true;
  env->ingest_epoch += 1;
  return BK_OK;
}

int bk_warm(bk_env* env, uint64_t n_steps) {
  if (!env) return fail(BK_INVALID_ARGUMENT, "null env");
  if (n_steps == 0) return BK_OK;
  if (int rc = use_device(env)) return rc;
  const size_t sb = static_cast<size_t>(env->cfg.n_books) * env->stride, lb = static_cast<size_t>(env->cfg.n_books) * env->W;
  if (!env->warm_snap.p) HIPCHK(env->warm_snap.alloc(sb + lb));
  HIPCHK(hipMemcpyAsync(env->warm_snap.p, env->state.p, sb * 4, hipMemcpyDeviceToDevice, env->stream));
  HIPCHK(hipMemcpyAsync(env->warm_snap.p + sb, env->l2_last.p, lb * 4, hipMemcpyDeviceToDevice, env->stream));
  const uint64_t steps0 = env->steps_done;
  const bool flow0 = env->device_flow;
  env->warming = true;
  const int rc = bk_run(env, n_steps);
  env->warming = false;
  env->steps_done = steps0;
  env->device_flow = flow0;
  env->wl_valid = false;
  env->ml_valid = false;
  std::string run_err = rc != BK_OK ? g_err : std::string();
  if (rc != BK_OK)
    for (int i = 0; i < bk_env::MAX_PARTS; ++i)
      if (env->part_stream[i]) (void)hipStreamSynchronize(env->part_stream[i]);
  const hipError_t e1 = hipMemcpyAsync(env->state.p, env->warm_snap.p, sb * 4, hipMemcpyDeviceToDevice, env->stream);
  const hipError_t e2 = hipMemcpyAsync(env->l2_last.p, env->warm_snap.p + sb, lb * 4, hipMemcpyDeviceToDevice, env->stream);
  if (rc != BK_OK) return fail(rc, run_err);
// ... 126 lines not shown
  const uint32_t NB = env->cfg.n_books;
  if (!env->gather_buf.p) HIPCHK(env->gather_buf.alloc(NB));
  hipLaunchKernelGGL(k_gather_header, dim3((NB + 255) / 256), dim3(256), 0, env->stream, env->state.p, env->stride, word, n_words,
                     NB, reinterpret_cast<unsigned long long*>(env->gather_buf.p));
  HIPCHK(hipGetLastError());
  HIPCHK(hipMemcpyAsync(totals, env->gather_buf.p, static_cast<size_t>(NB) * 8, hipMemcpyDeviceToHost, env->stream));
  HIPCHK(hipStreamSynchronize(env->stream));
  return BK_OK;
}

int bk_trade_counts(bk_env* env, uint64_t* totals) {
  if (!env || !totals) return fail(BK_INVALID_ARGUMENT, "null argument");
  if (int rc = use_device(env)) return rc;
  return gather_header(env, H_TRADES_LO, 2, totals);
}

int bk_get_trades(bk_env* env, uint32_t book, uint64_t first, uint64_t n, bk_trade* out) {
  if (int rc = check_book(env, book)) return rc;
  uint64_t total = 0, base = 0;
  if (int rc = bk_trade_count(env, book, &total, &base)) return rc;
  if (first < base || first > total || n > total - first) return fail(BK_INVALID_ARGUMENT, "trade range not retained");
  if (n && !out) return fail(BK_INVALID_ARGUMENT, "null argument");
  if (first + n - base > env->cfg.trade_capacity)
    return fail(BK_CAPACITY, "trade records beyond trade_capacity were dropped");
  if (n == 0) return BK_OK;
  std::vector<DevTrade> tmp(n);
  HIPCHK(hipMemcpy(tmp.data(), env->trades.p + static_cast<size_t>(book) * env->cfg.trade_capacity + (first - base),
                   n * sizeof(DevTrade), hipMemcpyDeviceToHost));
  for (uint64_t i = 0; i < n; ++i) {
    const DevTrade& d = tmp[i];
    bk_trade& t = out[i];
    t.t = (static_cast<uint64_t>(d.t_hi) << 32) | d.t_lo;
    t.side_is_bid = d.side_is_bid;
    t.price = d.price;
    t.vol = d.vol;
    t.reserved = 0;
    t.active_order_id = d.active;
    t.passive_order_id = d.passive;
  }
  return BK_OK;
}

int bk_trades_compact(bk_env* env, uint64_t* out_total) {
  if (!env) return fail(BK_INVALID_ARGUMENT, "null env");
  if (int rc = use_device(env)) return rc;
  const uint32_t B = env->cfg.n_books;
  if (!env->tr_off.p) HIPCHK(env->tr_off.alloc(static_cast<size_t>(B) + 1));
  hipLaunchKernelGGL(k_trade_scan, dim3(1), dim3(1024), 0, env->stream, env->state.p, env->stride, B,
                     env->cfg.trade_capacity, env->tr_off.p);
  HIPCHK(hipGetLastError());
  unsigned long long total = 0;
  HIPCHK(hipMemcpyAsync(&total, env->tr_off.p + B, 8, hipMemcpyDeviceToHost, env->stream));
  HIPCHK(hipStreamSynchronize(env->stream));
  if (total > env->tr_dense.n) HIPCHK(env->tr_dense.alloc(std::max<size_t>(total + total / 4, 1024)));
  hipLaunchKernelGGL(k_trade_gather, dim3((B + 3) / 4), dim3(256), 0, env->stream, env->state.p, env->stride, B,
                     env->cfg.trade_capacity, env->trades.p, env->tr_off.p, env->tr_dense.p);
  HIPCHK(hipGetLastError());
  env->tr_total = total;
  if (out_total) *out_total = total;
  return BK_OK;
}

int bk_trades_compact_copy_async(bk_env* env, bk_trade* records, uint64_t* offsets, void* copy_stream) {
  if (!env || !offsets || (env->tr_total && !records)) return fail(BK_INVALID_ARGUMENT, "null argument");
  if (!env->tr_off.p) return fail(BK_INVALID_ARGUMENT, "call bk_trades_compact first");
  if (int rc = use_device(env)) return rc;
  hipStream_t cs = copy_stream ? static_cast<hipStream_t>(copy_stream) : env->stream;
  if (copy_stream)
    if (int rc = order_after(cs, env->stream)) return rc;
  HIPCHK(hipMemcpyAsync(offsets, env->tr_off.p, (static_cast<size_t>(env->cfg.n_books) + 1) * 8, hipMemcpyDeviceToHost, cs));
  if (env->tr_total)
    HIPCHK(hipMemcpyAsync(records, env->tr_dense.p, env->tr_total * sizeof(bk_trade), hipMemcpyDeviceToHost, cs));
  if (!copy_stream) HIPCHK(hipStreamSynchronize(cs));
  return BK_OK;
}

int bk_clear_trades(bk_env* env) {
  if (!env) return fail(BK_INVALID_ARGUMENT, "null env");
  if (int rc = use_device(env)) return rc;
  const uint32_t B = env->cfg.n_books;
  hipLaunchKernelGGL(k_book_service, dim3((B + 255) / 256), dim3(256), 0, env->stream, env->state.p, env->stride, B, 0,
                     0u);
  HIPCHK(hipGetLastError());
  return BK_OK;
}

int bk_get_order_keys(bk_env* env, uint32_t book, uint64_t first, uint64_t n, uint32_t* key_price,
                      uint64_t* key_time) {
  if (int rc = check_book(env, book)) return rc;
  if (int rc = mirror_orders(env, book)) return rc;
  BookHost& bh = env->books[book];
  if (first > bh.orders.size() || n > bh.orders.size() - first) return fail(BK_INVALID_ARGUMENT, "order range out of bounds");
  if (env->cfg.max_orders == 0) return fail(BK_INVALID_ARGUMENT, "order log disabled (max_orders == 0)");
  if (bh.n_uploaded > env->cfg.max_orders) return fail(BK_CAPACITY, "order log capacity exceeded");
  if (int rc = use_device(env)) return rc;
  if (int rc = refresh_log(env, book)) return rc;
  for (uint64_t i = 0; i < n; ++i) {
    const uint64_t id = first + i;
    if (id < bh.n_uploaded && id < bh.log_cache.size()) {
      const DevOrderLog& d = bh.log_cache[id];
      if (key_price) key_price[i] = d.key_price;
      if (key_time) key_time[i] = (static_cast<uint64_t>(d.key_hi) << 32) | d.key_lo;
    } else {
      if (key_price) key_price[i] = bh.orders[id].price;
      if (key_time) key_time[i] = 0;
    }
  }
  return BK_OK;
}

int bk_load_book(bk_env* env, uint32_t book, uint64_t t, uint32_t trade_vol, uint64_t n_orders, const bk_order* orders,
                 const uint32_t* key_price, const uint64_t* key_time, uint64_t n_trades, const bk_trade* trades) {
  if (int rc = check_book(env, book)) return rc;
  if (env->acct_traders)
    return fail(BK_INVALID_ARGUMENT, "loading a book into an env with trader accounts (bk_accounts_enable) is not supported: "
                                     "its trade records would have no order records to look the traders up in");
  if ((n_orders && (!orders || !key_price || !key_time)) || (n_trades && !trades))
    return fail(BK_INVALID_ARGUMENT, "null argument");
  if (env->agent_log)
    return fail(BK_INVALID_ARGUMENT, "loading a book into an env with the agents' order log (bk_set_agent_order_log) is not "
                                     "supported");
  BookHost& bh = env->books[book];
  if (!env->books[book - book % env->M].queue.empty())
    return fail(BK_INVALID_ARGUMENT, "events are queued for this book (market)");
  if (n_orders > env->cfg.max_orders) return fail(BK_CAPACITY, "snapshot holds more orders than max_orders");
  if (n_trades > env->cfg.trade_capacity) return fail(BK_CAPACITY, "snapshot holds more trades than trade_capacity");
  if (n_orders >= 0xFFFFFFFFull) return fail(BK_CAPACITY, "order id space exhausted");
  std::vector<uint64_t> act;
  for (uint64_t i = 0; i < n_orders; ++i) {
    if (orders[i].order_id != i) return fail(BK_INVALID_ARGUMENT, "orders must be listed by id");
    if (orders[i].status > 4) return fail(BK_INVALID_ARGUMENT, "bad order status");
    if (orders[i].status == 1) act.push_back(i);
  }
  const uint32_t pool = static_cast<uint32_t>(env->R) * 64u;
  if (act.size() > pool) return fail(BK_CAPACITY, "snapshot holds more Active orders than max_live_orders");
  if (int rc = use_device(env)) return rc;
  HIPCHK(hipStreamSynchronize(env->stream));
  std::stable_sort(act.begin(), act.end(), [&](uint64_t a, uint64_t b) { return key_time[a] < key_time[b]; });

  const uint32_t L = env->cfg.levels, W = env->W, tick = env->asset_tick[book % env->M];
  std::vector<uint32_t> st(env->stride, 0u), l2(W, 0u);
  uint32_t* hdr = st.data();
  HIPCHK(hipMemcpy(hdr, env->state.p + static_cast<size_t>(book) * env->stride, HDR_DW * 4, hipMemcpyDeviceToHost));
  hdr[H_T_LO] = static_cast<uint32_t>(t);
  hdr[H_T_HI] = static_cast<uint32_t>(t >> 32);
  hdr[H_NEXT_ID] = static_cast<uint32_t>(n_orders);
  hdr[H_SEQ] = static_cast<uint32_t>(act.size());
  hdr[H_TRADES_LO] = static_cast<uint32_t>(n_trades);
  hdr[H_TRADES_HI] = static_cast<uint32_t>(n_trades >> 32);
  hdr[H_TRADE_BASE_LO] = hdr[H_TRADE_BASE_HI] = 0;
  hdr[H_FLAGS] = 0;
  hdr[H_TRADE_VOL] = trade_vol;
  hdr[H_LAST_NTRADES] = hdr[H_LAST_NEVENTS] = 0;
  for (int r = 0; r < 8; ++r) hdr[H_LIVE0 + 2 * r] = hdr[H_LIVE0 + 2 * r + 1] = 0;
  uint32_t bid_best = 0, ask_best = 0xFFFFFFFFu, bid_vol = 0, ask_vol = 0;
  for (size_t k = 0; k < act.size(); ++k) {
    const bk_order& o = orders[act[k]];
    const uint32_t r = static_cast<uint32_t>(k) / 64u, lane = static_cast<uint32_t>(k) % 64u;
    uint32_t* p = st.data() + HDR_DW + r * POOL_FIELDS * 64;
    p[0 * 64 + lane] = o.price;
    p[1 * 64 + lane] = o.vol;
    p[2 * 64 + lane] = static_cast<uint32_t>(o.order_id);
    p[3 * 64 + lane] = static_cast<uint32_t>(k);
    p[4 * 64 + lane] = 1u | (o.side_is_bid ? 2u : 0u);
    hdr[H_LIVE0 + 2 * r + (lane >> 5)] |= 1u << (lane & 31);
    if (o.side_is_bid) {
      bid_best = std::max(bid_best, o.price);
      bid_vol += o.vol;
    } else {
      ask_best = std::min(ask_best, o.price);
      ask_vol += o.vol;
    }
  }
  l2[0] = trade_vol;
  l2[1] = bid_best;
  l2[2] = ask_best;
  l2[3] = ask_vol;
  l2[4] = bid_vol;
  for (uint64_t i : act) {
    const bk_order& o = orders[i];
    const uint32_t d = o.side_is_bid ? bid_best - o.price : o.price - ask_best;
    for (uint32_t q = 0; q < L; ++q) {
      if (q * tick == d) {
        l2[5 + 4 * q + (o.side_is_bid ? 0 : 2)] += o.vol;
        l2[5 + 4 * q + (o.side_is_bid ? 1 : 3)] += 1;
      }
    }
  }
  std::vector<DevOrderLog> log(n_orders);
  bh.orders.clear();
  for (uint64_t i = 0; i < n_orders; ++i) {
    const bk_order& o = orders[i];
    bh.orders.push_back(HostOrder{static_cast<uint8_t>(o.side_is_bid ? 1 : 0), o.start_vol, o.price, o.trader_id,
                                  o.arr_time});
    DevOrderLog& d = log[i];
    std::memset(&d, 0, sizeof(d));
    d.status = o.status;
    d.vol = o.vol;
    d.price = o.price;
    d.key_price = key_price[i];
    d.arr_lo = static_cast<uint32_t>(o.arr_time);
    d.arr_hi = static_cast<uint32_t>(o.arr_time >> 32);
    d.end_lo = static_cast<uint32_t>(o.end_time);
    d.end_hi = static_cast<uint32_t>(o.end_time >> 32);
    d.key_lo = static_cast<uint32_t>(key_time[i]);
    d.key_hi = static_cast<uint32_t>(key_time[i] >> 32);
  }
  std::vector<DevTrade> tr(n_trades);
  for (uint64_t i = 0; i < n_trades; ++i) {
    const bk_trade& x = trades[i];
    tr[i] = DevTrade{static_cast<uint32_t>(x.t), static_cast<uint32_t>(x.t >> 32), x.price, x.vol,
                     static_cast<uint32_t>(x.active_order_id), static_cast<uint32_t>(x.passive_order_id),
                     x.side_is_bid ? 1u : 0u, 0u};
  }
  HIPCHK(hipMemcpy(env->state.p + static_cast<size_t>(book) * env->stride, st.data(), st.size() * 4,
                   hipMemcpyHostToDevice));
  HIPCHK(hipMemcpy(env->l2_last.p + static_cast<size_t>(book) * W, l2.data(), W * 4, hipMemcpyHostToDevice));
  if (n_orders)
    HIPCHK(hipMemcpy(env->order_log.p + static_cast<size_t>(book) * env->cfg.max_orders, log.data(),
                     n_orders * sizeof(DevOrderLog), hipMemcpyHostToDevice));
  if (n_trades)
    HIPCHK(hipMemcpy(env->trades.p + static_cast<size_t>(book) * env->cfg.trade_capacity, tr.data(),
                     n_trades * sizeof(DevTrade), hipMemcpyHostToDevice));
  env->ml_valid = false;
  env->wl_valid = false;
  bh.n_uploaded = n_orders;
  bh.log_fresh = false;
  bh.time_offset = t - (env->cfg.start_time + env->steps_done * env->cfg.step_size);
  return BK_OK;
}

int bk_set_time(bk_env* env, uint32_t book, uint64_t t) {
  if (int rc = check_book(env, book)) return rc;
  if (int rc = use_device(env)) return rc;
  HIPCHK(hipStreamSynchronize(env->stream));
  const uint32_t w[2] = {static_cast<uint32_t>(t), static_cast<uint32_t>(t >> 32)};
  HIPCHK(hipMemcpy(env->state.p + static_cast<size_t>(book) * env->stride + H_T_LO, w, 8, hipMemcpyHostToDevice));
  env->books[book].time_offset = t - (env->cfg.start_time + env->steps_done * env->cfg.step_size);
  return BK_OK;
}

int bk_time(bk_env* env, uint32_t book, uint64_t* out) {
  if (int rc = check_book(env, book)) return rc;
  uint32_t h[2];
  if (int rc = read_hdr(env, book, H_T_LO, 2, h)) return rc;
  if (out) *out = (static_cast<uint64_t>(h[1]) << 32) | h[0];
  return BK_OK;
}

int bk_trade_vol(bk_env* env, uint32_t book, uint32_t* out) {
  if (int rc = check_book(env, book)) return rc;
  if (!out) return fail(BK_INVALID_ARGUMENT, "null argument");
  return read_hdr(env, book, H_TRADE_VOL, 1, out);
}

int bk_steps_done(bk_env* env, uint64_t* out) {
  if (!env) return fail(BK_INVALID_ARGUMENT, "null env");
  if (out) *out = env->steps_done;
  return BK_OK;
}

int bk_book_flags(bk_env* env, uint32_t* out) {
  if (!env || !out) return fail(BK_INVALID_ARGUMENT, "null argument");
  if (int rc = use_device(env)) return rc;
  std::vector<uint64_t> v(env->cfg.n_books);
  if (int rc = gather_header(env, H_FLAGS, 1, v.data())) return rc;
  for (size_t b = 0; b < v.size(); ++b) out[b] = static_cast<uint32_t>(v[b]);
  return BK_OK;
}

int bk_clear_flags(bk_env* env, uint32_t mask) {
  if (!env) return fail(BK_INVALID_ARGUMENT, "null env");
  if (int rc = use_device(env)) return rc;
  const uint32_t B = env->cfg.n_books;
  hipLaunchKernelGGL(k_book_service, dim3((B + 255) / 256), dim3(256), 0, env->stream, env->state.p, env->stride, B, 2, mask);
  HIPCHK(hipGetLastError());
  return BK_OK;
}

int bk_flags_summary(bk_env* env, uint32_t* flags_or, uint64_t* max_retained_trades) {
  if (!env) return fail(BK_INVALID_ARGUMENT, "null env");
  if (int rc = use_device(env)) return rc;
  const uint32_t B = env->cfg.n_books;
  if (!env->gather_buf.p) HIPCHK(env->gather_buf.alloc(B));
  uint32_t* out = reinterpret_cast<uint32_t*>(env->gather_buf.p);
  HIPCHK(hipMemsetAsync(out, 0, 8, env->stream));
  hipLaunchKernelGGL(k_flags_summary, dim3((B + 255) / 256), dim3(256), 0, env->stream, env->state.p, env->stride, B, out);
  HIPCHK(hipGetLastError());
  uint32_t res[2] = {0, 0};
  HIPCHK(hipMemcpyAsync(res, out, 8, hipMemcpyDeviceToHost, env->stream));
  HIPCHK(hipStreamSynchronize(env->stream));
  if (flags_or) *flags_or = res[0];
  if (max_retained_trades) *max_retained_trades = res[1];
  return BK_OK;
}

int bk_rng_state(bk_env* env, uint32_t book, uint64_t out_state[2]) {
  if (int rc = check_book(env, book)) return rc;
  if (!out_state) return fail(BK_INVALID_ARGUMENT, "null argument");
  uint32_t h[4];
  if (int rc = read_hdr(env, book, H_S0_LO, 4, h)) return rc;
  out_state[0] = (static_cast<uint64_t>(h[1]) << 32) | h[0];
  out_state[1] = (static_cast<uint64_t>(h[3]) << 32) | h[2];
  return BK_OK;
}

// ... 751 lines not shown
```

Measured before the change: 308.7 million.

## Carry key window across steps, precompute FSM event masks, skip redundant checks

Stores the keyed-event price/sequence window in spare header words so later steps can reuse it instead of recomputing it with a reduction over all live orders. The bound is widened with agent limit-price bounds precomputed on the host. The FSM agent kernel now builds pending/side bitmasks into the batch buffer, so the step kernel no longer rebuilds them with LDS atomics. Host-known non-zero volumes let it skip the zero-volume ballot, and RNG header words are no longer rewritten when the header is kept. The cost is extra header state, more LDS in the FSM kernel, and a carried window that must be invalidated correctly.

```diff
diff --git a/bourse_amd/csrc/agent_table.hpp b/bourse_amd/csrc/agent_table.hpp
--- a/bourse_amd/csrc/agent_table.hpp
+++ b/bourse_amd/csrc/agent_table.hpp
@@ -1,4 +1,5 @@
 #pragma once
+#include <algorithm>
 #include <cmath>
 #include <cstdint>
 #include <cstring>
@@ -61,6 +62,20 @@
     out[g] = G;
   }
   return BK_OK;
+}
+
+struct GroupBounds {
+  uint32_t pmin = 0xFFFFFFFFu, pmax = 0u, vol_nonzero = 1u;
+};
+inline GroupBounds group_bounds(const Group* g, size_t n) {
+  GroupBounds b;
+  for (size_t i = 0; i < n; ++i) {
+    if (g[i].n == 0) continue;
+    b.pmin = std::min(b.pmin, g[i].tick_lo * g[i].tick_size);
+    b.pmax = std::max(b.pmax, (g[i].tick_lo + g[i].tick_rng - 1u) * g[i].tick_size);
+    if (g[i].vol_lo == 0) b.vol_nonzero = 0u;
+  }
+  return b;
 }
 
 constexpr const char* CAPACITY_MSG = "sum of n_agents exceeds max_live_orders (one pool slot per agent)";
diff --git a/bourse_amd/csrc/agents_fsm_body.inc b/bourse_amd/csrc/agents_fsm_body.inc
--- a/bourse_amd/csrc/agents_fsm_body.inc
+++ b/bourse_amd/csrc/agents_fsm_body.inc
@@ -136,8 +136,42 @@
     *reinterpret_cast<uint2*>(st + (size_t)as * a.state_stride + H_S1_LO) = make_uint2(rng.b0, rng.b1);
   }
   bt[BT_NEV] = n_ev;
+#if BOURSE_AMD_FSM_MASKS
+  uint64_t* masks = reinterpret_cast<uint64_t*>(fsm_lds + fsm_list_dwords(R));
+#pragma unroll
+  for (int w = 0; w < 2 * R; ++w) masks[w * 64 + lane] = 0ull;
+  auto mark = [&](uint32_t e) {
+    const uint32_t bit = (e & EV_NEW) ? 1u << (e & 31u) : 0u;
+    __hip_atomic_fetch_or(&masks[((e & EV_SLOT) >> 5) * 64 + lane], mk64(bit, (e & EV_BID) ? bit : 0u), __ATOMIC_RELAXED,
+                          __HIP_MEMORY_SCOPE_WAVEFRONT);
+  };
+#endif
   for (uint32_t k = 0; k < n_ev; k += 2) {
     const uint32_t lo = list[k * 64 + lane];
     const uint32_t hi = (k + 1 < n_ev) ? list[(k + 1) * 64 + lane] : 0u;
     bt[BT_EV + (k >> 1)] = lo | (hi << 16);
+#if BOURSE_AMD_FSM_MASKS
+    mark(lo);
+    mark(hi);
+#endif
   }
+#if BOURSE_AMD_FSM_MASKS
+  {
+    uint32_t mp[2 * R], mb[2 * R];
+#pragma unroll
+    for (int w = 0; w < 2 * R; ++w) {
+      const uint64_t m = masks[w * 64 + lane];
+      mp[w] = (uint32_t)m, mb[w] = (uint32_t)(m >> 32);
+    }
+    if constexpr (R == 1) {
+      *reinterpret_cast<uint2*>(bt + BT_MASKS) = make_uint2(mp[0], mp[1]);
+      *reinterpret_cast<uint2*>(bt + BT_MASKS + 2) = make_uint2(mb[0], mb[1]);
+    } else {
+#pragma unroll
+      for (int q = 0; q < R / 2; ++q) {
+        reinterpret_cast<uint4*>(bt + BT_MASKS)[q] = make_uint4(mp[4 * q], mp[4 * q + 1], mp[4 * q + 2], mp[4 * q + 3]);
+        reinterpret_cast<uint4*>(bt + BT_MASKS + 2 * R)[q] = make_uint4(mb[4 * q], mb[4 * q + 1], mb[4 * q + 2], mb[4 * q + 3]);
+      }
+    }
+  }
+#endif
diff --git a/bourse_amd/csrc/book_device.hpp b/bourse_amd/csrc/book_device.hpp
--- a/bourse_amd/csrc/book_device.hpp
+++ b/bourse_amd/csrc/book_device.hpp
@@ -1,5 +1,6 @@
 #pragma once
 #include <hip/hip_runtime.h>
+#include <type_traits>
 #include <utility>
 #include <stdint.h>
 
@@ -12,6 +13,16 @@
 #endif
 #ifndef BOURSE_AMD_ASM_R48
 #define BOURSE_AMD_ASM_R48 1
+#endif
+
+#ifndef BOURSE_AMD_KEY_CARRY
+#define BOURSE_AMD_KEY_CARRY 1
+#endif
+#ifndef BOURSE_AMD_FSM_MASKS
+#define BOURSE_AMD_FSM_MASKS 1
+#endif
+#ifndef BOURSE_AMD_STEP_HINTS
+#define BOURSE_AMD_STEP_HINTS 1
 #endif
 
 namespace bkd {
@@ -23,6 +34,7 @@
   H_STEPS_LO, H_STEPS_HI, H_EVENTS_LO, H_EVENTS_HI, H_TRADE_VOL,
   H_TRADE_BASE_LO, H_TRADE_BASE_HI, H_LAST_NTRADES, H_LAST_NEVENTS,
   H_EV_KEYED,
+  H_KW_VALID = 24, H_KW_PMIN, H_KW_PMAX, H_KW_SFLOOR,
   H_LIVE0 = 32,
 };
 constexpr int HDR_SCALARS = 20;
@@ -73,12 +85,14 @@
   uint32_t* batch;
   uint32_t batch_stride;
   uint32_t book_begin, book_end;
+  uint32_t new_pmin, new_pmax, vol_nonzero;
+  uint32_t batch_masks;
   uint32_t assets;
   uint32_t asset_tick[MAX_ASSETS];
   UDiv tick_div, asset_div[MAX_ASSETS];
   Group groups[MAX_GROUPS];
 };
-constexpr int BT_NEV = 0, BT_EV = 64;
+constexpr int BT_NEV = 0, BT_MASKS = 8, BT_EV = 64;
 constexpr uint32_t EV_NEW = 0x8000u, EV_BID = 0x4000u, EV_SLOT = 0x1FFu;
 constexpr uint32_t EV_MOD = 0x800u, EV_MOD_P = 0x200u, EV_MOD_V = 0x400u;
 
@@ -90,6 +104,10 @@
 __device__ __forceinline__ void sload_x16_x4(const uint32_t* p, bk_u32x16& a, bk_u32x4& b) {
   asm volatile("s_load_dwordx16 %0, %2, 0x0\n\ts_load_dwordx4 %1, %2, 0x40\n\ts_waitcnt lgkmcnt(0)"
                : "=&s"(a), "=&s"(b) : "s"(p) : "memory");
+}
+__device__ __forceinline__ void sload_x16_x4_x4(const uint32_t* p, bk_u32x16& a, bk_u32x4& b, bk_u32x4& c) {
+  asm volatile("s_load_dwordx16 %0, %3, 0x0\n\ts_load_dwordx4 %1, %3, 0x40\n\ts_load_dwordx4 %2, %3, 0x60\n\ts_waitcnt lgkmcnt(0)"
+               : "=&s"(a), "=&s"(b), "=&s"(c) : "s"(p) : "memory");
 }
 __device__ __forceinline__ bk_u32x8 sload_x8(const uint32_t* p) {
   bk_u32x8 a;
@@ -252,6 +270,7 @@
   uint32_t tr_k, tr_price, tr_vol, tr_act, tr_pas;
   uint32_t tr_n;
   uint32_t hdr0;
+  uint32_t kw_valid, kw_pmin, kw_pmax, kw_sfloor;
 };
 
 template <int R>
@@ -597,6 +616,7 @@
 struct StepRaw {
   uint32_t hdr, f[R][POOL_FIELDS];
   uint32_t sh[HDR_SCALARS];
+  uint32_t kw[4];
   uint32_t bh, ev[R];
   uint2 pv[R];
 };
@@ -610,19 +630,26 @@
     for (int f = 0; f < POOL_FIELDS; ++f) w.f[r][f] = p[f * 64 + lane];
   }
 }
-template <int R>
+template <int R, bool KW = false>
 __device__ __forceinline__ void load_state_scalars(StepRaw<R>& w, const uint32_t* __restrict__ st) {
   if constexpr (R <= 2) {
     bk_u32x16 a;
     bk_u32x4 b;
-    sload_x16_x4(st, a, b);
+    if constexpr (KW) {
+      bk_u32x4 c;
+      sload_x16_x4_x4(st, a, b, c);
+#pragma unroll
+      for (int i = 0; i < 4; ++i) w.kw[i] = c[i];
+    } else {
+      sload_x16_x4(st, a, b);
+    }
 #pragma unroll
     for (int i = 0; i < 16; ++i) w.sh[i] = a[i];
 #pragma unroll
     for (int i = 16; i < HDR_SCALARS; ++i) w.sh[i] = b[i - 16];
   }
 }
-template <int R>
+template <int R, bool KW = false>
 __device__ __forceinline__ void unpack_book(Book<R>& B, Rng& rng, const StepRaw<R>& w) {
   const uint32_t hdr = w.hdr;
 #pragma unroll
@@ -654,6 +681,11 @@
   B.tr_k = B.tr_price = B.tr_vol = B.tr_act = B.tr_pas = 0;
   B.tr_n = 0;
   B.hdr0 = hdr;
+  auto W = [&](int i) { return !KW ? 0u : R <= 2 ? w.kw[i - H_KW_VALID] : rdl(hdr, (uint32_t)i); };
+  B.kw_valid = W(H_KW_VALID);
+  B.kw_pmin = W(H_KW_PMIN);
+  B.kw_pmax = W(H_KW_PMAX);
+  B.kw_sfloor = W(H_KW_SFLOOR);
 }
 template <int R>
 __device__ __forceinline__ void load_book(Book<R>& B, Rng& rng, const uint32_t* __restrict__ st, int lane) {
@@ -663,7 +695,7 @@
   unpack_book<R>(B, rng, w);
 }
 
-template <int R, bool KEEP_HDR = false>
+template <int R, bool KEEP_HDR = false, bool KEEP_KW = false>
 __device__ __forceinline__ void store_book(const Book<R>& B, const Rng& rng, uint32_t* __restrict__ st, int lane,
                                            uint64_t steps_done, uint32_t last_ntrades, uint32_t last_nevents,
                                            uint32_t ev_keyed = 0u) {
@@ -672,10 +704,12 @@
   auto put = [&](int idx, uint32_t v) { hdr = wrl(rfl(v), (uint32_t)idx, hdr); };
   put(H_T_LO, (uint32_t)B.t);
   put(H_T_HI, (uint32_t)(B.t >> 32));
-  put(H_S0_LO, (uint32_t)rng.s0);
-  put(H_S0_HI, (uint32_t)(rng.s0 >> 32));
-  put(H_S1_LO, (uint32_t)rng.s1);
-  put(H_S1_HI, (uint32_t)(rng.s1 >> 32));
+  if (!(KEEP_HDR && BOURSE_AMD_STEP_HINTS)) {
+    put(H_S0_LO, (uint32_t)rng.s0);
+    put(H_S0_HI, (uint32_t)(rng.s0 >> 32));
+    put(H_S1_LO, (uint32_t)rng.s1);
+    put(H_S1_HI, (uint32_t)(rng.s1 >> 32));
+  }
   put(H_NEXT_ID, B.next_id);
   put(H_SEQ, B.seq_ctr);
   put(H_TRADES_LO, (uint32_t)B.n_trades);
@@ -693,6 +727,8 @@
     put(H_LIVE0 + 2 * r, (uint32_t)B.live[r]);
     put(H_LIVE0 + 2 * r + 1, (uint32_t)(B.live[r] >> 32));
   }
+  static_assert(KEEP_HDR || !KEEP_KW, "the carried key window is kept in the loaded header copy");
+  if (!KEEP_KW) put(H_KW_VALID, 0u);
   st[lane] = hdr;
 #pragma unroll
   for (int r = 0; r < R; ++r) {
@@ -720,9 +756,10 @@
 constexpr uint32_t KEY_ASK = 0x80000000u;
 constexpr uint32_t KP_MKT_BID = 0xFFFFFFFFu, KP_MKT_ASK = 0x10000u;
 template <int R>
-__device__ __forceinline__ bool key_window(const Book<R>& B, const uint64_t (&newm)[R], uint32_t n_ev, uint32_t& pbase,
-                                           uint32_t& sbase, uint32_t xmin = 0xFFFFFFFFu, uint32_t xmax = 0u) {
-  uint32_t pmax = xmax, pmin = xmin, age = 0;
+__device__ __forceinline__ bool key_window(const Book<R>& B, const uint64_t (&newm)[R], uint32_t n_ev, uint32_t& pmin,
+                                           uint32_t& pmax, uint32_t& pbase, uint32_t& sbase, uint32_t xmin, uint32_t xmax) {
+  pmax = xmax, pmin = xmin;
+  uint32_t age = 0;
 #pragma unroll
   for (int r = 0; r < R; ++r) {
     const bool lv = lane_bit(B.live[r]), in = lv | lane_bit(newm[r]);
@@ -734,6 +771,12 @@
   pbase = pmin - 2u;
   sbase = B.seq_ctr - age - 1u;
   return pmin >= 2u && pmax != 0xFFFFFFFFu && pmax - pmin <= KEY_PSPAN && age + n_ev < KEY_SMASK - 1u;
+}
+template <int R>
+__device__ __forceinline__ bool key_window(const Book<R>& B, const uint64_t (&newm)[R], uint32_t n_ev, uint32_t& pbase,
+                                           uint32_t& sbase, uint32_t xmin = 0xFFFFFFFFu, uint32_t xmax = 0u) {
+  uint32_t pmin, pmax;
+  return key_window<R>(B, newm, n_ev, pmin, pmax, pbase, sbase, xmin, xmax);
 }
 
 template <int R>
@@ -742,15 +785,38 @@
   uint32_t sq, sbase, pbase;
   int32_t alo, bhi;
 };
-template <int R, bool MARKETS = false>
-__device__ __forceinline__ bool keys_begin(const Book<R>& B, const uint64_t (&newm)[R], uint32_t n_ev, KeyState<R>& K,
-                                           uint32_t xmin = 0xFFFFFFFFu, uint32_t xmax = 0u) {
+template <int R, bool MARKETS = false, bool CARRY = false>
+__device__ __forceinline__ bool keys_begin(std::conditional_t<CARRY, Book<R>, const Book<R>>& B, const uint64_t (&newm)[R],
+                                           uint32_t n_ev, KeyState<R>& K, uint32_t xmin = 0xFFFFFFFFu, uint32_t xmax = 0u,
+                                           uint32_t new_pmin = 0u, uint32_t new_pmax = 0xFFFFFFFFu) {
+  static_assert(!(CARRY && MARKETS), "the carried window knows the agents' limit prices only");
   uint32_t pbase;
   uint64_t lim[R];
 #pragma unroll
   for (int r = 0; r < R; ++r)
     lim[r] = MARKETS ? newm[r] & ~__ballot(B.price[r] == (lane_bit(B.bid[r]) ? 0xFFFFFFFFu : 0u)) : newm[r];
-  if (!key_window<R>(B, lim, n_ev, pbase, K.sbase, xmin, xmax)) return false;
+  if constexpr (CARRY) {
+    auto keep = [&](int idx, uint32_t v) { B.hdr0 = wrl(rfl(v), (uint32_t)idx, B.hdr0); };
+    const uint32_t lo = min(B.kw_pmin, new_pmin), hi = max(B.kw_pmax, new_pmax);
+    const uint32_t age = B.seq_ctr - B.kw_sfloor - 1u;
+    if (B.kw_valid != 0u && lo >= 2u && hi != 0xFFFFFFFFu && hi - lo <= KEY_PSPAN && age < KEY_SMASK - 1u &&
+        age + n_ev < KEY_SMASK - 1u) {
+      keep(H_KW_PMIN, lo);
+      keep(H_KW_PMAX, hi);
+      pbase = lo - 2u;
+      K.sbase = B.kw_sfloor;
+    } else {
+      uint32_t pmin, pmax;
+      const bool ok = key_window<R>(B, lim, n_ev, pmin, pmax, pbase, K.sbase, xmin, xmax);
+      keep(H_KW_VALID, 1u);
+      keep(H_KW_PMIN, pmin);
+      keep(H_KW_PMAX, pmax);
+      keep(H_KW_SFLOOR, K.sbase);
+      if (!ok) return false;
+    }
+  } else if (!key_window<R>(B, lim, n_ev, pbase, K.sbase, xmin, xmax)) {
+    return false;
+  }
   K.pbase = pbase;
 #pragma unroll
   for (int r = 0; r < R; ++r) {
@@ -999,7 +1065,8 @@
   }
 }
 
-template <int R, bool MKT = false, bool TAGGED = false, bool CLS = false, bool PENDKEY = false, bool LOG = false, class... Lg>
+template <int R, bool MKT = false, bool TAGGED = false, bool CLS = false, bool PENDKEY = false, bool LOG = false,
+          bool CARRY = false, class... Lg>
 __device__ __forceinline__ uint32_t step_from_list(Book<R>& B, const DevArgs& a, uint32_t book, int lane,
                                                    const uint32_t (&ev)[R], uint32_t n_ev, uint32_t* bins,
                                                    uint32_t hist_slot, bool write_last, const UDiv& tick,
@@ -1036,12 +1103,13 @@
     uint32_t k = 0;
     const uint32_t nev = rfl(n_ev), tmask = B.trading ? 0xFFFFFFFFu : 0u;
     KeyState<R> K;
-    if (BOURSE_AMD_KEYED_EVENTS && keys_begin<R>(B, newm, nev, K)) {
+    if (BOURSE_AMD_KEYED_EVENTS && keys_begin<R, false, CARRY>(B, newm, nev, K, 0xFFFFFFFFu, 0u, a.new_pmin, a.new_pmax)) {
       uint32_t evw[R];
       key_event_words<R>(K, evm, nev, evw);
       uint64_t zero_vol = 0;
-#pragma unroll
-      for (int r = 0; r < R; ++r) zero_vol |= __ballot(lane_bit(newm[r]) && B.vol[r] == 0u);
+      if (!(BOURSE_AMD_STEP_HINTS && a.vol_nonzero))
+#pragma unroll
+        for (int r = 0; r < R; ++r) zero_vol |= __ballot(lane_bit(newm[r]) && B.vol[r] == 0u);
       const uint32_t checked = (!B.trading || zero_vol != 0) ? 1u : 0u;
       for (;;) {
         uint32_t full;
@@ -1066,7 +1134,7 @@
         flush_trades<R>(B, a, book, t0, lane);
     }
   } else if (KeyState<R> K; !LOG && (CLS || PENDKEY) && (!MKT || MKTK) && BOURSE_AMD_KEYED_EVENTS &&
-             (keys_begin<R, !CLS>(B, newm, rfl(n_ev), K) ||
+             (keys_begin<R, !CLS, CARRY>(B, newm, rfl(n_ev), K, 0xFFFFFFFFu, 0u, a.new_pmin, a.new_pmax) ||
               (BOURSE_AMD_KEYED_WIDE && !CLS && keys_begin_wide<R, true>(B, newm, rfl(n_ev), K, ev, bins, lane)))) {
    if constexpr ((R == 4 || R == 8) && BOURSE_AMD_ASM_EVENTS && BOURSE_AMD_ASM_R48) {
     listed = true;
@@ -1088,8 +1156,9 @@
     uint32_t k = 0;
     const uint32_t nev = rfl(n_ev), tmask = B.trading ? 0xFFFFFFFFu : 0u;
     uint64_t zero_vol = 0;
-#pragma unroll
-    for (int r = 0; r < R; ++r) zero_vol |= __ballot(lane_bit(newm[r]) && B.vol[r] == 0u);
+    if (!(BOURSE_AMD_STEP_HINTS && CLS && a.vol_nonzero))
+#pragma unroll
+      for (int r = 0; r < R; ++r) zero_vol |= __ballot(lane_bit(newm[r]) && B.vol[r] == 0u);
     const uint32_t checked = (!B.trading || zero_vol != 0) ? 1u : 0u;
     for (;;) {
       uint32_t full;
@@ -1228,7 +1297,8 @@
 #define BK_STR2(x) #x
 #define BK_STR(x) BK_STR2(x)
 
-constexpr uint32_t fsm_lds_bytes(int R) { return 64u * R * 32u * 4u; }
+constexpr uint32_t fsm_list_dwords(int R) { return 64u * R * 32u; }
+constexpr uint32_t fsm_lds_bytes(int R) { return fsm_list_dwords(R) * 4u + 64u * 2u * R * 8u; }
 
 struct LaneGroup {
   uint4 a, b;
@@ -1312,7 +1382,7 @@
     w.ev[r] = reinterpret_cast<const uint16_t*>(bt + BT_EV)[r * 64 + lane];
     w.pv[r] = POOLPEND ? make_uint2(0u, 0u) : reinterpret_cast<const uint2*>(bt + BT_EV + 32 * R)[r * 64 + lane];
   }
-  load_state_scalars<R>(w, st);
+  load_state_scalars<R, BOURSE_AMD_KEY_CARRY && !POOLPEND && !LOG>(w, st);
   step_batch_raw<R, MKT, POOLPEND, LOG>(a, book, lane, lds, step_index, write_last, w, B, rng, hist_slot, dorders);
 }
 template <int R, bool MKT, bool POOLPEND, bool LOG>
@@ -1340,7 +1410,8 @@
     }
   }
 
-  unpack_book<R>(B, rng, w);
+  constexpr bool CARRY = BOURSE_AMD_KEY_CARRY && !POOLPEND && !LOG;
+  unpack_book<R, CARRY>(B, rng, w);
   const uint32_t n_ev = rdl(w.bh, BT_NEV);
   uint32_t ev[R];
   uint32_t owner[R];
@@ -1348,7 +1419,14 @@
 #pragma unroll
   for (int r = 0; r < R; ++r) ev[r] = w.ev[r];
   uint32_t mw = 0;
-  if (!POOLPEND) {
+  uint64_t pendm[R], sidem[R];
+  if (BOURSE_AMD_FSM_MASKS && !POOLPEND && a.batch_masks) {
+#pragma unroll
+    for (int r = 0; r < R; ++r) {
+      pendm[r] = mk64(rdl(w.bh, BT_MASKS + 2 * r), rdl(w.bh, BT_MASKS + 2 * r + 1));
+      sidem[r] = mk64(rdl(w.bh, BT_MASKS + 2 * R + 2 * r), rdl(w.bh, BT_MASKS + 2 * R + 2 * r + 1));
+    }
+  } else if (!POOLPEND) {
     uint32_t* pm = lds;
     if (lane < 4 * R) pm[lane] = 0;
 #pragma unroll
@@ -1359,6 +1437,11 @@
       atomicOr(&pm[2 * R + (slot >> 5)], (is_new && (ew & EV_BID)) ? bit : 0u);
     }
     mw = pm[lane & (4 * R - 1)];
+#pragma unroll
+    for (int r = 0; r < R; ++r) {
+      pendm[r] = mk64(rdl(mw, 2 * r), rdl(mw, 2 * r + 1));
+      sidem[r] = mk64(rdl(mw, 2 * R + 2 * r), rdl(mw, 2 * R + 2 * r + 1));
+    }
   }
 #pragma unroll
   for (int r = 0; r < R; ++r) {
@@ -1366,8 +1449,8 @@
       owner[r] = w.f[r][4] & 0xFF00u;
       continue;
     }
-    const uint64_t pend = mk64(rdl(mw, 2 * r), rdl(mw, 2 * r + 1)) & mine[r];
-    const uint64_t side = mk64(rdl(mw, 2 * R + 2 * r), rdl(mw, 2 * R + 2 * r + 1));
+    const uint64_t pend = pendm[r] & mine[r];
+    const uint64_t side = sidem[r];
     const uint2 pv = w.pv[r];
     B.price[r] = sel(pend, pv.x, B.price[r]);
     B.vol[r] = sel(pend, pv.y, B.vol[r]);
@@ -1399,10 +1482,9 @@
                                                            MKT ? a.asset_div[asset] : a.tick_div, mine, n_own, asset,
                                                            LogCtx{a.order_log + (size_t)book * a.log_cap, a.log_cap});
   else
-    ntr = step_from_list<R, MKT, MKT && POOLPEND, !POOLPEND, POOLPEND && !MKT>(B, a, book, lane, ev, n_ev, lds, hist_slot,
-                                                                               write_last != 0, MKT ? a.asset_div[asset] : a.tick_div,
-                                                                               mine, n_own, asset);
-  store_book<R, !POOLPEND>(B, rng, st, lane, step_index + 1, ntr, n_own);
+    ntr = step_from_list<R, MKT, MKT && POOLPEND, !POOLPEND, POOLPEND && !MKT, false, CARRY>(
+        B, a, book, lane, ev, n_ev, lds, hist_slot, write_last != 0, MKT ? a.asset_div[asset] : a.tick_div, mine, n_own, asset);
+  store_book<R, !POOLPEND, CARRY>(B, rng, st, lane, step_index + 1, ntr, n_own);
   if (POOLPEND) {
 #pragma unroll
     for (int r = 0; r < R; ++r) {
diff --git a/bourse_amd/csrc/bourse_amd.hip b/bourse_amd/csrc/bourse_amd.hip
--- a/bourse_amd/csrc/bourse_amd.hip
+++ b/bourse_amd/csrc/bourse_amd.hip
@@ -220,6 +220,7 @@
   std::vector<Group> table;
   DevBuf<Group> dtable;
   uint32_t n_agents_total = 0;
+  GroupBounds agent_bounds;
   uint64_t agents_hash = 0;
   bool device_ingress = false;
   uint32_t qcap = 0;
@@ -328,6 +329,10 @@
     a.batch_stride = batch_stride;
     a.book_begin = 0;
     a.book_end = cfg.n_books / M;
+    a.new_pmin = agent_bounds.pmin;
+    a.new_pmax = agent_bounds.pmax;
+    a.vol_nonzero = agent_bounds.vol_nonzero;
+    a.batch_masks = 0;
     a.assets = M;
     for (int i = 0; i < MAX_ASSETS; ++i) a.asset_tick[i] = asset_tick[i];
     auto dv = [](uint32_t d) {
@@ -640,6 +645,7 @@
       a.book_end = (i + 1 == P) ? B : (static_cast<uint32_t>(static_cast<uint64_t>(B) * (i + 1) / P) & ~3u);
       a.hist_slot0 = a.hist_cap ? static_cast<uint32_t>((first_step + s) % a.hist_cap) : 0u;
       a.step_prio = pl.step_prio ? 1u : 0u;
+      a.batch_masks = (BOURSE_AMD_FSM_MASKS && pl.agents == AG_FSM) ? 1u : 0u;
       const uint32_t nb = a.book_end - a.book_begin;
       hipStream_t st = P > 1 ? env->part_stream[i] : env->stream;
       if (P > 1 && s == 0 && i > 0) {
@@ -1721,6 +1727,7 @@
     return fail(rc, msg);
   if (total > env->cfg.max_live_orders) return fail(BK_CAPACITY, CAPACITY_MSG);
   env->groups = gs;
+  env->agent_bounds = group_bounds(gs.data(), gs.size());
   env->n_agents_total = static_cast<uint32_t>(total);
   env->n_mixed = 0;
   env->table.clear();
@@ -1751,6 +1758,7 @@
   std::swap(env->dtable.n, d.n);
   env->groups.assign(t.begin(), t.begin() + n_groups);
   env->table.swap(t);
+  env->agent_bounds = group_bounds(env->table.data(), env->table.size());
   env->n_agents_total = static_cast<uint32_t>(total);
   env->n_mixed = 0;
   env->mtable.clear();
@@ -1843,6 +1851,7 @@
   for (uint32_t as = 0; as < MAX_ASSETS; ++as) env->n_fixed_a[as] = fixed_a[as];
   env->ml_valid = false;
   env->groups.clear();
+  env->agent_bounds = GroupBounds{};
   env->table.clear();
   (void)env->dtable.alloc(0);
   env->n_agents_total = 0;
@@ -2275,6 +2284,7 @@
   hdr[H_FLAGS] = 0;
   hdr[H_TRADE_VOL] = trade_vol;
   hdr[H_LAST_NTRADES] = hdr[H_LAST_NEVENTS] = 0;
+  hdr[H_KW_VALID] = 0;
   for (int r = 0; r < 8; ++r) hdr[H_LIVE0 + 2 * r] = hdr[H_LIVE0 + 2 * r + 1] = 0;
   uint32_t bid_best = 0, ask_best = 0xFFFFFFFFu, bid_vol = 0, ask_vol = 0;
   for (size_t k = 0; k < act.size(); ++k) {
```

Result: slower. 304.7 million (-1.3%).
